# zju3dv/PVO

Measured on AMD Instinct MI355X. Metric: VO keyframe updates/sec (8-keyframe window, 512x384, 36 edges; 6 graph updates + edge rebuild per keyframe), higher is better.
Workload: dtype f16 (volume, lookup, update operator) / f32 (BA assembly) / f64 (pose solve); 1 GPU; S-B: BASELINE.json configs[1] window (8 keyframes, 48x64 maps, E=36, itrs=2), synthetic; edges=36, parallelism=independent window per GPU

## Files before the change

include/pvo_hip.h:

```cpp
#ifndef PVO_HIP_H
#define PVO_HIP_H

#include <stddef.h>
#include <stdint.h>

#ifdef __cplusplus
extern "C" {
#endif

enum { PVO_F32 = 0, PVO_F16 = 1, PVO_BF16 = 2, PVO_F64 = 3 };

enum {
  PVO_OK = 0,
  PVO_EINVAL = 1,
  PVO_ELAUNCH = 2,
  PVO_EWORKSPACE = 3,
  PVO_EUNSUPPORTED = 4
};

const char* pvo_strerror(int code);
const char* pvo_last_hip_error(void);
#define PVO_ABI_VERSION 105
int pvo_version(void);
size_t pvo_graph_update_args_size(void);

enum {
  PVO_KNOB_BA_SOLVER = 0,
  PVO_KNOB_HEADS_GATHER_FLAT = 1,
  PVO_KNOB_NO_RIDERS = 2,
  PVO_KNOB_POST_SEPARATE = 3,
  PVO_KNOB_COUNT = 4
};
int pvo_debug_config(int knob, int value);
int pvo_knob(int knob);


int pvo_corr_index_forward(const void* volume, const float* coords, void* corr,
                           int N, int h1, int w1, int h2, int w2,
                           int radius, int dtype, void* stream);

int pvo_corr_index_backward(const float* coords, const void* corr_grad, void* volume_grad,
                            int N, int h1, int w1, int h2, int w2,
                            int radius, int dtype, void* stream);

int pvo_corr_pyramid_lookup(const void* const* volumes_host, const float* coords, void* out,
                            int N, int h1, int w1, int h2, int w2,
                            int num_levels, int radius, int dtype, int out_channels_last,
                            const int* slots, int num_slots, void* stream);

int pvo_altcorr_forward(const void* fmap1, const void* fmap2, const float* coords, void* corr,
                        int B, int S, int H1, int W1, int H2, int W2, int C,
                        int radius, int dtype, void* stream);

int pvo_altcorr_backward(const void* fmap1, const void* fmap2, const float* coords,
                         const void* corr_grad, void* fmap1_grad, void* fmap2_grad,
                         int B, int S, int H1, int W1, int H2, int W2, int C,
                         int radius, int dtype, void* stream);


int pvo_corr_build(const void* fmap1, const void* fmap2, void* const* levels_host,
                   int N, int C, int H, int W, int num_levels, int dtype, int channels_last,
                   const int* out_slots, void* stream);

int pvo_corr_build_tiled(const void* fmap1, const void* fmap2, void* const* levels_host,
                         int N, int C, int H, int W, int dtype, const int* out_slots, void* stream);
int pvo_corr_pyramid_lookup_tiled(const void* const* volumes_host, const float* coords, void* out,
                                  int N, int h1, int w1, int h2, int w2, int num_levels, int dtype,
                                  int out_channels_last, const int* slots, int num_slots, void* stream);

int pvo_corr_lookup_encode_tiled(const void* const* volumes_host, const float* coords,
                                 const void* enc_weight, const float* enc_bias, void* out,
                                 int N, int h1, int w1, int dtype,
                                 const int* slots, int num_slots, void* stream);



int pvo_gru_glo_chunks(int HW);
int pvo_gru_glo_fused(const void* net, const void* w_weight, const float* w_bias, float* glo_part,
                      int E, int HW, int dtype, void* stream);
int pvo_gate_context(const float* glo_part, const float* wg_t, const float* g_bias, float* g,
                     int E, int chunks, void* stream);
int pvo_conv3x3_c128(const void* x, const void* w_taps, const float* bias, void* y,
                     int E, int H, int W, int Cout, int relu, int ystride, int yoff, int dtype, void* stream);
int pvo_conv3x3(const void* x, const void* w_taps, const float* bias, void* y,
                int E, int H, int W, int Cin, int Cout, int relu, int ystride, int yoff, int dtype, void* stream);
int pvo_gru_conv_gates(const void* net, const void* cf, int cf_channels, const void* w_taps, const float* g,
                       const void* P_zr, const int* p_slots, void* Z, void* RN, int E, int H, int W, int dtype, void* stream);
int pvo_gru_conv_candidate(const void* RN, const void* cf, int cf_channels, const void* w_taps, const float* g,
                           const void* P_q, const int* p_slots, const void* Z, const void* net, void* net_out,
                           int E, int H, int W, int dtype, void* stream);
int pvo_conv3x3_heads(const void* x, const void* w1_taps, const float* bias1, const void* w2_frags, float* z,
                      int E, int H, int W, int dtype, void* stream);
int pvo_heads_gather(const float* z, const float* bias2, void* y, int E, int H, int W, int dtype, void* stream);
int pvo_heads_out(const void* h1, const float* bias1, const void* w2, const float* bias2, void* y,
                  int E, int H, int W, int dtype, void* stream);
int pvo_conv7x7_c8(const void* x, const void* w_taps, const float* bias, void* y,
                   int E, int H, int W, int dtype, void* stream);
int pvo_flow_encoder(const void* x, const void* w7_taps, const float* bias7, const void* w3_taps, const float* bias3,
                     void* y, int E, int H, int W, int ystride, int yoff, int dtype, void* stream);
int pvo_corr_encode(const void* corr, const void* enc_weight, const float* enc_bias, void* y, long long rows,
                    int dtype, void* stream);
int pvo_segment_mean(const void* x, const int* seg_ptr, const int* seg_idx, const float* in_bias, void* out,
                     int K, int HW, int C, int dtype, void* stream);
int pvo_eta_head(const void* x, const void* w_taps, const float* bias, const int64_t* frame, const int* pos,
                 float* damping, float* eta, int R, int H, int W, float EP, float eta_scale, int dtype, void* stream);
int pvo_conv1x1_c128(const void* x, const void* w, const float* bias, void* y, long long rows, int Cout, int relu,
                     int dtype, void* stream);

int pvo_bias_norm_act(const void* x, const void* bias, const void* residual, void* y, long long planes, int C, int HW,
                      int norm, float eps, int relu_inner, int relu_outer, int dtype, void* stream);
int pvo_bias_norm_act_slices(int HW);
int pvo_bias_norm_act_split(const void* x, const void* bias, const void* residual, void* y, long long planes, int C, int HW,
                            int norm, float eps, int relu_inner, int relu_outer, int dtype, float* ws, size_t ws_floats, void* stream);
int pvo_conv1x1_planes(const void* x, const void* w, const void* bias, void* y, int N, int Cin, int Cout, int Hin, int Win, int stride,
                       int dtype, void* stream);
int pvo_frame_normalise(const void* img, void* out, int H, int W, const float* mean3, const float* std3, int in_kind, int dtype, void* stream);

int pvo_graph_motion(const float* target, const float* coords1, const float* delta_dy, const float* raw_mask,
                     void* motn, int E, int H, int W, int dtype, void* stream);
int pvo_segment_hist(const int* segm, const float* raw_mask, const void* heads, int* tot, int* dyn,
                     int E, int HW, int max_segments, float dy_thresh, int dtype, void* stream);
int pvo_graph_post(const float* coords1, const void* heads, float* raw_mask, float* target, float* delta_dy,
                   float* weight, float* target_ba, float* weight_ba, float* full_flow,
                   int E, int H, int W, float dy_thresh, const int* segm, const int* vote_tot, const int* vote_dyn,
                   int max_segments, float vote_thresh, int dtype, void* stream);


enum {
  PVO_OP_CONV128_WIDE = 1,
  PVO_OP_SINGLE_STREAM = 2,
  PVO_OP_ENC_SIDE_STREAM = 4
};

typedef struct pvo_update_weights {
  int dtype;
  int flags;
  const void* enc0_w;   const float* enc0_b;
  const void* cenc2_w;  const float* cenc2_b;
  const void* fenc0_w;  const float* fenc0_b;
  const void* fenc2_w;  const float* fenc2_b;
  const void* glo_w;    const float* glo_b;
  const float* gate_wt; const float* gate_b;
  const void* zr_w;     const void* q_w;
  const void* zr_inp_w; const void* q_inp_w;
  const void* heads1_w; const float* heads1_b;
  const void* heads2_w; const float* heads2_b;
  const void* agg1_w;   const float* agg1_b;
  const void* agg2_w;   const float* agg2_b;
  const void* eta_w;    const float* eta_b;
  const void* up_w;     const float* up_b;
} pvo_update_weights;

typedef struct pvo_operator_args {
  int E, H, W;
  const void* levels[4]; const int* slots; int num_slots;
  const float* coords;
  const void* corr;
  const void* motion;
  const void* net;
  void* net_out;
  const void* inp;
  const void* P_zr; const void* P_q;
  int static_by_slot;
  const int* seg_ptr; const int* seg_idx; int K;
  void* heads;
  const int64_t* eta_frame; const int* eta_pos; int R; float* damping; float EP; float eta_scale;
  float* eta;
  void* upmask;
} pvo_operator_args;

size_t pvo_operator_workspace_bytes(int E, int K, int H, int W);
int pvo_update_operator(const pvo_update_weights* weights, const pvo_operator_args* args,
                        void* workspace, size_t workspace_bytes, void* stream);

typedef struct pvo_graph_update_args {
  pvo_operator_args op;
  int nframes;
  float* poses; float* disps; const float* intrinsics;
  const int64_t* ii; const int64_t* jj;
  float* target; float* delta_dy; float* raw_mask;
  float* weight; float* full_flow;
  const int* segm; int max_segments; float vote_thresh;
  float dy_thresh;
  int n_in;
  float* target_ba; float* weight_ba;
  const int64_t* ii_ba; const int64_t* jj_ba;
  int t0, t1, itrs, motion_only; float lm, ep;
  void* sys; void* ba_ws; size_t ba_ws_bytes;
  int clamp_frames; float disp_min;
  int want_upmask;
  int context_ahead, context_ready;
} pvo_graph_update_args;

size_t pvo_graph_update_workspace_bytes(int E, int K, int R, int H, int W, int max_segments);
int pvo_side_stream(void** stream_out);

int pvo_proximity_select(const float* dist, int ni, int nj, int t0, int t1, int rad, int nms, double thresh,
                         const long long* have_i, const long long* have_j, int n_have,
                         long long* out_i, long long* out_j, int max_out, int* n_out);
enum { PVO_STAGE_LOOKUP = 0, PVO_STAGE_GATES = 1, PVO_STAGE_CANDIDATE = 2, PVO_STAGE_BA = 3, PVO_STAGE_UPDATE = 4,
       PVO_STAGE_EMPTY = 5  };
int pvo_probe_arm(int stage, int capacity);
int pvo_probe_arm_every(int stage, int capacity, int every);
int pvo_probe_read(float* ms_host, int max_n);
int pvo_graph_update(const pvo_update_weights* weights, const pvo_graph_update_args* args,
                     void* workspace, size_t workspace_bytes, void* stream);


int pvo_frame_distance(const float* poses, const float* disps, const float* intrinsics,
                       const int64_t* ii, const int64_t* jj, float* dist,
                       int M, int ht, int wd, float beta, void* stream);
int pvo_frame_distance_bidirectional(const float* poses, const float* disps, const float* intrinsics,
                                     const int64_t* ii, const int64_t* jj, float* dist,
                                     int M, int ht, int wd, float beta, void* stream);

int pvo_projmap(const float* poses, const float* disps, const float* intrinsics,
                const int64_t* ii, const int64_t* jj, float* coords, float* valid,
                int E, int ht, int wd, void* stream);

int pvo_iproj(const float* poses, const float* disps, const float* intrinsics,
              float* points, int N, int ht, int wd, void* stream);

int pvo_depth_filter(const float* poses, const float* disps, const float* intrinsics,
                     const int64_t* ix, const float* thresh, float* counter,
                     int N, int nframes, int ht, int wd, void* stream);

int pvo_reproject(const float* poses, const float* disps, const float* intrinsics,
                  const int64_t* ii, const int64_t* jj, float* coords, float* valid,
                  int E, int ht, int wd, void* stream);
int pvo_reproject_motion(const float* poses, const float* disps, const float* intrinsics,
                         const int64_t* ii, const int64_t* jj, float* coords, float* valid,
                         const float* target, const float* delta_dy, const float* raw_mask, void* motn,
                         int E, int ht, int wd, int dtype, void* stream);


int pvo_se3_unary(int op, const void* x, void* y, long long n, int dtype, void* stream);
int pvo_se3_binary(int op, const void* a, long long rep_a, const void* b, long long rep_b, void* y, long long n,
                   int dtype, void* stream);
int pvo_se3_unary_vjp(int op, const void* x, const void* gy, void* gx, long long n, int dtype, void* stream);
int pvo_se3_binary_vjp(int op, const void* a, long long rep_a, const void* b, long long rep_b, const void* gy,
                       void* ga, void* gb, long long n, int dtype, void* stream);

int pvo_proj_transform(const void* poses, const void* depths, const void* intr, const int64_t* ii, const int64_t* jj,
                       int B, int P, int N, int ht, int wd, int nx, void* x1, void* valid, void* Ji, void* Jj, void* Jz,
                       int dtype, void* stream);
int pvo_proj_transform_vjp(const void* poses, const void* depths, const void* intr, const int64_t* ii, const int64_t* jj,
                           int B, int P, int N, int ht, int wd, int nx, const void* g_x1, const void* g_Ji, const void* g_Jj, const void* g_Jz,
                           void* gposes, void* gdepths, int dtype, void* stream);


size_t pvo_ba_workspace_bytes(int E, int P, int nframes, int HW);

int pvo_ba(float* poses, float* disps, const float* intrinsics,
           const float* targets, const float* weights, const float* eta,
           const int64_t* ii, const int64_t* jj,
           int E, int nframes, int ht, int wd, int K_eta,
           int t0, int t1, int iterations, float lm, float ep, int motion_only,
           float* dx_out, float* dz_out, int dz_rows, int* status_out,
           void* workspace, size_t workspace_bytes, void* stream);

int pvo_ba_plan(const int64_t* ii, const int64_t* jj, int E, int nframes, int HW,
                int K_eta, int t0, int t1, void* workspace, size_t workspace_bytes,
                void* stream);
int pvo_ba_last_partition(void* workspace, size_t workspace_bytes, int E, int P, int nframes, int HW, int* out, void* stream);
int pvo_ba_local(const float* poses, const float* disps, const float* intrinsics,
                 const float* targets, const float* weights, const float* eta,
                 const int64_t* ii, const int64_t* jj,
                 int E, int nframes, int ht, int wd, int K_eta, int t0, int t1,
                 int motion_only, void* sys,
                 void* workspace, size_t workspace_bytes, void* stream);
int pvo_ba_finish(float* poses, float* disps, void* sys,
                  const int64_t* ii, const int64_t* jj,
                  int E, int nframes, int ht, int wd, int t0, int t1,
                  float lm, float ep, int motion_only, int clamp_frames, float disp_min,
                  float* dx_out, float* dz_out, int dz_rows, int* status_out,
                  void* workspace, size_t workspace_bytes, void* stream);
size_t pvo_ba_packed_elems(const int* first_host, int P);
int pvo_ba_pack(void* sys, const int* first_s, void* msg, int P, void* stream);
int pvo_ba_finish_packed(float* poses, float* disps, const void* msg, const int* first_s,
                         const int64_t* ii, const int64_t* jj,
                         int E, int nframes, int ht, int wd, int t0, int t1,
                         float lm, float ep, int motion_only, int clamp_frames, float disp_min,
                         float* dx_out, float* dz_out, int dz_rows, int* status_out,
                         void* workspace, size_t workspace_bytes, void* stream);

typedef struct pvo_ba_riders {
  const void* cx; const void* cw; const float* cbias; void* cy; long long crows; int cCout; int cdtype;
  const void* gnet; const void* gw; const float* gbias; float* gpart; int gE; int gHW; int gdtype;
  const float* xpart; const float* xwt; const float* xbias; float* xg; int xE; int xchunks;
} pvo_ba_riders;
int pvo_ba_finish_riders(float* poses, float* disps, void* sys,
                         const int64_t* ii, const int64_t* jj,
                         int E, int nframes, int ht, int wd, int t0, int t1,
                         float lm, float ep, int motion_only, int clamp_frames, float disp_min,
                         float* dx_out, float* dz_out, int dz_rows, int* status_out,
                         void* workspace, size_t workspace_bytes,
                         const pvo_ba_riders* riders, void* stream);
int pvo_ba_finish_conv1x1(float* poses, float* disps, void* sys,
                          const int64_t* ii, const int64_t* jj,
                          int E, int nframes, int ht, int wd, int t0, int t1,
                          float lm, float ep, int motion_only, int clamp_frames, float disp_min,
                          float* dx_out, float* dz_out, int dz_rows, int* status_out,
                          void* workspace, size_t workspace_bytes,
                          const void* cx, const void* cw, const float* cbias, void* cy, long long crows, int cCout, int cdtype,
                          void* stream);


size_t pvo_ba_train_workspace_bytes(int B, int P, int N, int M, int HW, int dtype);
size_t pvo_ba_train_vjp_scratch_bytes(int B, int P, int N, int M, int HW, int dtype);
int pvo_ba_train(const void* poses, const void* disps, const void* intr, const void* target, const void* weight, const void* eta,
                 const int64_t* ii, const int64_t* jj, const int* kx, const int* kk, const int* kptr, const int* kedge,
                 int B, int P, int N, int M, int ht, int wd, int fixedp, void* poses_out, void* disps_out, void* dx_out,
                 void* workspace, size_t workspace_bytes, int dtype, void* stream);
int pvo_ba_train_vjp(const void* poses, const void* disps, const void* intr, const void* target, const void* weight,
                     const int64_t* ii, const int64_t* jj, const int* kx, const int* kk, const int* kptr, const int* kedge,
                     int B, int P, int N, int M, int ht, int wd, int fixedp, const void* g_poses_out, const void* g_disps_out,
                     void* g_target, void* g_weight, void* g_eta, void* g_poses, void* g_disps,
                     const void* workspace, size_t workspace_bytes, void* scratch, size_t scratch_bytes, int dtype, void* stream);

#ifdef __cplusplus
}
#endif
#endif
```

pvo_amd/_lib.py:

```python
import ctypes
import os

_HERE = os.path.dirname(os.path.abspath(__file__))
LIB_PATH = os.path.join(_HERE, "libpvo_hip.so")

PVO_F32, PVO_F16, PVO_BF16, PVO_F64 = 0, 1, 2, 3
PVO_ABI_VERSION = 105

_c = ctypes
_vp, _i, _f, _sz = _c.c_void_p, _c.c_int, _c.c_float, _c.c_size_t

SIGNATURES = {
    "pvo_strerror": (_c.c_char_p, [_i]),
    "pvo_version": (_i, []),
    "pvo_graph_update_args_size": (_sz, []),
    "pvo_last_hip_error": (_c.c_char_p, []),
    "pvo_debug_config": (_i, [_i, _i]),
    "pvo_knob": (_i, [_i]),
    "pvo_corr_index_forward": (_i, [_vp, _vp, _vp, _i, _i, _i, _i, _i, _i, _i, _vp]),
    "pvo_corr_index_backward": (_i, [_vp, _vp, _vp, _i, _i, _i, _i, _i, _i, _i, _vp]),
    "pvo_corr_pyramid_lookup": (_i, [_vp, _vp, _vp, _i, _i, _i, _i, _i, _i, _i, _i, _i, _vp, _i, _vp]),
    "pvo_altcorr_forward": (_i, [_vp, _vp, _vp, _vp, _i, _i, _i, _i, _i, _i, _i, _i, _i, _vp]),
    "pvo_altcorr_backward": (_i, [_vp, _vp, _vp, _vp, _vp, _vp, _i, _i, _i, _i, _i, _i, _i, _i, _i, _vp]),
    "pvo_corr_build": (_i, [_vp, _vp, _vp, _i, _i, _i, _i, _i, _i, _i, _vp, _vp]),
    "pvo_gru_glo_chunks": (_i, [_i]),
    "pvo_gru_glo_fused": (_i, [_vp, _vp, _vp, _vp, _i, _i, _i, _vp]),
    "pvo_gate_context": (_i, [_vp, _vp, _vp, _vp, _i, _i, _vp]),
    "pvo_gru_conv_gates": (_i, [_vp, _vp, _i, _vp, _vp, _vp, _vp, _vp, _vp, _i, _i, _i, _i, _vp]),
    "pvo_gru_conv_candidate": (_i, [_vp, _vp, _i, _vp, _vp, _vp, _vp, _vp, _vp, _vp, _i, _i, _i, _i, _vp]),
    "pvo_conv3x3": (_i, [_vp, _vp, _vp, _vp, _i, _i, _i, _i, _i, _i, _i, _i, _i, _vp]),
    "pvo_conv3x3_c128": (_i, [_vp, _vp, _vp, _vp, _i, _i, _i, _i, _i, _i, _i, _i, _vp]),
    "pvo_conv7x7_c8": (_i, [_vp, _vp, _vp, _vp, _i, _i, _i, _i, _vp]),
    "pvo_flow_encoder": (_i, [_vp, _vp, _vp, _vp, _vp, _vp, _i, _i, _i, _i, _i, _i, _vp]),
    "pvo_corr_encode": (_i, [_vp, _vp, _vp, _vp, _c.c_longlong, _i, _vp]),
    "pvo_eta_head": (_i, [_vp, _vp, _vp, _vp, _vp, _vp, _vp, _i, _i, _i, _f, _f, _i, _vp]),
    "pvo_conv1x1_c128": (_i, [_vp, _vp, _vp, _vp, _c.c_longlong, _i, _i, _i, _vp]),
    "pvo_corr_build_tiled": (_i, [_vp, _vp, _vp, _i, _i, _i, _i, _i, _vp, _vp]),
    "pvo_corr_lookup_encode_tiled": (_i, [_vp, _vp, _vp, _vp, _vp, _i, _i, _i, _i, _vp, _i, _vp]),
    "pvo_corr_pyramid_lookup_tiled": (_i, [_vp, _vp, _vp, _i, _i, _i, _i, _i, _i, _i, _i, _vp, _i, _vp]),
    "pvo_heads_out": (_i, [_vp, _vp, _vp, _vp, _vp, _i, _i, _i, _i, _vp]),
    "pvo_conv3x3_heads": (_i, [_vp, _vp, _vp, _vp, _vp, _i, _i, _i, _i, _vp]),
    "pvo_heads_gather": (_i, [_vp, _vp, _vp, _i, _i, _i, _i, _vp]),
    "pvo_segment_mean": (_i, [_vp, _vp, _vp, _vp, _vp, _i, _i, _i, _i, _vp]),
    "pvo_graph_motion": (_i, [_vp, _vp, _vp, _vp, _vp, _i, _i, _i, _i, _vp]),
    "pvo_reproject_motion": (_i, [_vp, _vp, _vp, _vp, _vp, _vp, _vp, _vp, _vp, _vp, _vp, _i, _i, _i, _i, _vp]),
    "pvo_bias_norm_act": (_i, [_vp, _vp, _vp, _vp, _c.c_longlong, _i, _i, _i, _f, _i, _i, _i, _vp]),
    "pvo_bias_norm_act_slices": (_i, [_i]),
    "pvo_bias_norm_act_split": (_i, [_vp, _vp, _vp, _vp, _c.c_longlong, _i, _i, _i, _f, _i, _i, _i, _vp, _sz, _vp]),
    "pvo_conv1x1_planes": (_i, [_vp, _vp, _vp, _vp, _i, _i, _i, _i, _i, _i, _i, _vp]),
    "pvo_frame_normalise": (_i, [_vp, _vp, _i, _i, _c.POINTER(_f), _c.POINTER(_f), _i, _i, _vp]),
    "pvo_segment_hist": (_i, [_vp, _vp, _vp, _vp, _vp, _i, _i, _i, _f, _i, _vp]),
    "pvo_graph_post": (_i, [_vp, _vp, _vp, _vp, _vp, _vp, _vp, _vp, _vp, _i, _i, _i, _f, _vp, _vp, _vp, _i, _f, _i, _vp]),
    "pvo_operator_workspace_bytes": (_sz, [_i, _i, _i, _i]),
    "pvo_update_operator": (_i, [_vp, _vp, _vp, _sz, _vp]),
    "pvo_graph_update_workspace_bytes": (_sz, [_i, _i, _i, _i, _i, _i]),
    "pvo_graph_update": (_i, [_vp, _vp, _vp, _sz, _vp]),
    "pvo_se3_unary": (_i, [_i, _vp, _vp, _c.c_longlong, _i, _vp]),
    "pvo_se3_binary": (_i, [_i, _vp, _c.c_longlong, _vp, _c.c_longlong, _vp, _c.c_longlong, _i, _vp]),
    "pvo_se3_unary_vjp": (_i, [_i, _vp, _vp, _vp, _c.c_longlong, _i, _vp]),
    "pvo_se3_binary_vjp": (_i, [_i, _vp, _c.c_longlong, _vp, _c.c_longlong, _vp, _vp, _vp, _c.c_longlong, _i, _vp]),
    "pvo_proj_transform": (_i, [_vp, _vp, _vp, _vp, _vp, _i, _i, _i, _i, _i, _i, _vp, _vp, _vp, _vp, _vp, _i, _vp]),
    "pvo_proj_transform_vjp": (_i, [_vp, _vp, _vp, _vp, _vp, _i, _i, _i, _i, _i, _i, _vp, _vp, _vp, _vp, _vp, _vp, _i, _vp]),
    "pvo_side_stream": (_i, [_c.POINTER(_vp)]),
    "pvo_proximity_select": (_i, [_vp, _i, _i, _i, _i, _i, _i, _c.c_double, _vp, _vp, _i, _vp, _vp, _i, _c.POINTER(_i)]),
    "pvo_probe_arm": (_i, [_i, _i]),
    "pvo_probe_arm_every": (_i, [_i, _i, _i]),
    "pvo_probe_read": (_i, [_vp, _i]),
    "pvo_frame_distance": (_i, [_vp, _vp, _vp, _vp, _vp, _vp, _i, _i, _i, _f, _vp]),
    "pvo_frame_distance_bidirectional": (_i, [_vp, _vp, _vp, _vp, _vp, _vp, _i, _i, _i, _f, _vp]),
    "pvo_projmap": (_i, [_vp, _vp, _vp, _vp, _vp, _vp, _vp, _i, _i, _i, _vp]),
    "pvo_iproj": (_i, [_vp, _vp, _vp, _vp, _i, _i, _i, _vp]),
    "pvo_depth_filter": (_i, [_vp, _vp, _vp, _vp, _vp, _vp, _i, _i, _i, _i, _vp]),
    "pvo_reproject": (_i, [_vp, _vp, _vp, _vp, _vp, _vp, _vp, _i, _i, _i, _vp]),
    "pvo_ba_workspace_bytes": (_sz, [_i, _i, _i, _i]),
    "pvo_ba": (_i, [_vp, _vp, _vp, _vp, _vp, _vp, _vp, _vp, _i, _i, _i, _i, _i, _i, _i, _i,
                    _f, _f, _i, _vp, _vp, _i, _vp, _vp, _sz, _vp]),
    "pvo_ba_plan": (_i, [_vp, _vp, _i, _i, _i, _i, _i, _i, _vp, _sz, _vp]),
    "pvo_ba_last_partition": (_i, [_vp, _sz, _i, _i, _i, _i, ctypes.POINTER(ctypes.c_int), _vp]),
    "pvo_ba_packed_elems": (_sz, [ctypes.POINTER(ctypes.c_int), _i]),
    "pvo_ba_pack": (_i, [_vp, _vp, _vp, _i, _vp]),
    "pvo_ba_finish_packed": (_i, [_vp, _vp, _vp, _vp, _vp, _vp, _i, _i, _i, _i, _i, _i, _f, _f, _i, _i, _f,
                                  _vp, _vp, _i, _vp, _vp, _sz, _vp]),
    "pvo_ba_local": (_i, [_vp, _vp, _vp, _vp, _vp, _vp, _vp, _vp, _i, _i, _i, _i, _i, _i, _i,
                          _i, _vp, _vp, _sz, _vp]),
    "pvo_ba_finish": (_i, [_vp, _vp, _vp, _vp, _vp, _i, _i, _i, _i, _i, _i, _f, _f, _i, _i, _f,
                           _vp, _vp, _i, _vp, _vp, _sz, _vp]),
    "pvo_ba_finish_riders": (_i, [_vp, _vp, _vp, _vp, _vp, _i, _i, _i, _i, _i, _i, _f, _f, _i, _i, _f,
                                  _vp, _vp, _i, _vp, _vp, _sz, _vp, _vp]),
    "pvo_ba_finish_conv1x1": (_i, [_vp, _vp, _vp, _vp, _vp, _i, _i, _i, _i, _i, _i, _f, _f, _i, _i, _f,
                                   _vp, _vp, _i, _vp, _vp, _sz, _vp, _vp, _vp, _vp, _c.c_longlong, _i, _i, _vp]),
    "pvo_ba_train_workspace_bytes": (_sz, [_i, _i, _i, _i, _i, _i]),
    "pvo_ba_train_vjp_scratch_bytes": (_sz, [_i, _i, _i, _i, _i, _i]),
    "pvo_ba_train": (_i, [_vp, _vp, _vp, _vp, _vp, _vp, _vp, _vp, _vp, _vp, _vp, _vp, _i, _i, _i, _i, _i, _i, _i,
                          _vp, _vp, _vp, _vp, _sz, _i, _vp]),
    "pvo_ba_train_vjp": (_i, [_vp, _vp, _vp, _vp, _vp, _vp, _vp, _vp, _vp, _vp, _vp, _i, _i, _i, _i, _i, _i, _i,
                              _vp, _vp, _vp, _vp, _vp, _vp, _vp, _vp, _sz, _vp, _sz, _i, _vp]),
}



class UpdateWeights(_c.Structure):
    _fields_ = [("dtype", _i), ("flags", _i)] + [(n, _vp) for n in (
        "enc0_w", "enc0_b", "cenc2_w", "cenc2_b", "fenc0_w", "fenc0_b", "fenc2_w", "fenc2_b", "glo_w", "glo_b",
        "gate_wt", "gate_b", "zr_w", "q_w", "zr_inp_w", "q_inp_w", "heads1_w", "heads1_b", "heads2_w", "heads2_b",
        "agg1_w", "agg1_b", "agg2_w", "agg2_b", "eta_w", "eta_b", "up_w", "up_b")]


class OperatorArgs(_c.Structure):
    _fields_ = [("E", _i), ("H", _i), ("W", _i), ("levels", _vp * 4), ("slots", _vp), ("num_slots", _i),
                ("coords", _vp), ("corr", _vp), ("motion", _vp), ("net", _vp), ("net_out", _vp), ("inp", _vp),
                ("P_zr", _vp), ("P_q", _vp), ("static_by_slot", _i), ("seg_ptr", _vp), ("seg_idx", _vp), ("K", _i), ("heads", _vp),
                ("eta_frame", _vp), ("eta_pos", _vp), ("R", _i), ("damping", _vp), ("EP", _f), ("eta_scale", _f), ("eta", _vp),
                ("upmask", _vp)]


class GraphUpdateArgs(_c.Structure):
    _fields_ = [("op", OperatorArgs), ("nframes", _i), ("poses", _vp), ("disps", _vp), ("intrinsics", _vp),
                ("ii", _vp), ("jj", _vp), ("target", _vp), ("delta_dy", _vp), ("raw_mask", _vp), ("weight", _vp),
                ("full_flow", _vp), ("segm", _vp), ("max_segments", _i), ("vote_thresh", _f), ("dy_thresh", _f),
                ("n_in", _i), ("target_ba", _vp), ("weight_ba", _vp), ("ii_ba", _vp), ("jj_ba", _vp),
                ("t0", _i), ("t1", _i), ("itrs", _i), ("motion_only", _i), ("lm", _f), ("ep", _f),
                ("sys", _vp), ("ba_ws", _vp), ("ba_ws_bytes", _sz), ("clamp_frames", _i), ("disp_min", _f),
                ("want_upmask", _i), ("context_ahead", _i), ("context_ready", _i)]


PVO_OP_CONV128_WIDE, PVO_OP_SINGLE_STREAM, PVO_OP_ENC_SIDE_STREAM = 1, 2, 4
PVO_KNOB_BA_SOLVER, PVO_KNOB_HEADS_GATHER_FLAT, PVO_KNOB_NO_RIDERS, PVO_KNOB_POST_SEPARATE = 0, 1, 2, 3

_lib = None


class PvoHipError(RuntimeError):
    pass


def load():
    global _lib
    if _lib is not None:
        return _lib
    if not os.path.exists(LIB_PATH):
        raise PvoHipError(
            "libpvo_hip.so not found at %s - build it with `python -m pvo_amd.build` "
            "(there is no CPU fallback)" % LIB_PATH)
    import torch
    lib = ctypes.CDLL(LIB_PATH)
    for name, (res, args) in SIGNATURES.items():
        fn = getattr(lib, name)
        fn.restype = res
        fn.argtypes = args
    if lib.pvo_version() != PVO_ABI_VERSION or lib.pvo_graph_update_args_size() != ctypes.sizeof(GraphUpdateArgs):
        raise PvoHipError("libpvo_hip.so is ABI version %d with a %d-byte pvo_graph_update_args; this binding is written for version %d / %d bytes - "
                          "rebuild with `python -m pvo_amd.build`" % (lib.pvo_version(), lib.pvo_graph_update_args_size(), PVO_ABI_VERSION,
                                                                     ctypes.sizeof(GraphUpdateArgs)))
    _lib = lib
    return lib


PROBE_LIB_PATH = os.path.join(_HERE, "libpvo_probe.so")
PROBE_SIGNATURES = {
    "pvo_clock_probe": (_i, [_vp, _i, _vp]),
    "pvo_mem_probe": (_c.c_longlong, [_vp, _sz, _i, _i, _i, _vp, _vp]),
}
_probe_lib = None


def load_probe():
    global _probe_lib
    if _probe_lib is None:
        load()
        if not os.path.exists(PROBE_LIB_PATH):
            raise PvoHipError("libpvo_probe.so not found at %s - build it with `python -m pvo_amd.build`" % PROBE_LIB_PATH)
        lib = ctypes.CDLL(PROBE_LIB_PATH)
        for name, (res, args) in PROBE_SIGNATURES.items():
            fn = getattr(lib, name)
            fn.restype, fn.argtypes = res, args
        _probe_lib = lib
    return _probe_lib


def check(status, what):
    if status != 0:
        msg = load().pvo_strerror(status).decode()
        if status == 2:
            msg += " - " + load().pvo_last_hip_error().decode()
        raise PvoHipError("%s failed: %s (status %d)" % (what, msg, status))
```

pvo_amd/csrc/ba.hip:

```cpp
#include "se3.h"
#include "conv1x1_tile.h"
#include "glo_tile.h"
#include <stdlib.h>
#include <type_traits>

namespace {

constexpr float kMinDepth = 0.25f;

constexpr double kFix = 268435456.0, kInvFix = 1.0 / 268435456.0;
__device__ __forceinline__ void fix_add(long long* sys, long long idx, double v, int* meta) {
  if (!(fabs(v) < 3.0e10)) { meta[4] = 1; return; }
#ifdef PVO_BA_NO_ATOMICS
  if (idx >= 0) return;
#endif
  atomicAdd(reinterpret_cast<unsigned long long*>(sys + idx), static_cast<unsigned long long>(__double2ll_rn(v * kFix)));
}
constexpr int kDealEdges = 2;
constexpr int kPPT = 2;
constexpr int kChunkA = 256 * kPPT;
constexpr int kMaxSep = 12;
constexpr int kXchgDoubles = 2 + 36 * kMaxSep * kMaxSep + 12 * kMaxSep;


#if defined(PVO_BA_PROBE) && PVO_BA_PROBE == 3
__device__ unsigned long long* g_ba_wg_probe = nullptr;
#define BA_WG_PROBE(kern, slot)                                                                                         \
  do {                                                                                                                  \
    if (g_ba_wg_probe && threadIdx.x == 0 && blockIdx.z == 0) {                                                         \
      const unsigned wg_ = blockIdx.y * gridDim.x + blockIdx.x;                                                         \
      if (wg_ < 4096u) g_ba_wg_probe[((kern) * 4096u + wg_) * 8u + (slot)] = wall_clock64();                            \
    }                                                                                                                   \
  } while (0)
#else
#define BA_WG_PROBE(kern, slot)
#endif

struct Plan {
  int* kidx;
  int* kx;
  int* eptr;
  int* eidx;
  int* meta;
  int* env;
};

struct Ws {
  Plan plan;
  float *Eii, *Eij;
  float *Cii, *bz;
  float *Ei;
  float *Q, *w;
  float *dx;
  float *part;
  long long* sys;
  double* chol;
  double* xchg;
  double* ldiag;
  double* xvec;
  float* Mrg;
  float* spart;
  short* srow;
  int* sT;
  size_t bytes;
};
constexpr int kSchurStagePairs = 36;
__host__ __device__ __forceinline__ int schur_stage_frames(int P) { return (P > 0 && P <= 29) ? P + 8 : 0; }

__host__ size_t align_up(size_t x) { return (x + 255) & ~static_cast<size_t>(255); }

__host__ Ws carve(void* base, int E, int P, int F, int HW) {
  Ws w{};
  char* p = static_cast<char*>(base);
  size_t off = 0;
  auto take = [&](size_t bytes) { char* r = p ? p + off : nullptr; off += align_up(bytes); return r; };
  const int Kmax = (F < P + E) ? F : (P + E);
  const size_t n6 = static_cast<size_t>(6) * (P > 0 ? P : 0);
  w.plan.kidx = reinterpret_cast<int*>(take(sizeof(int) * (F + 1)));
  w.plan.kx = reinterpret_cast<int*>(take(sizeof(int) * (F + 1)));
  w.plan.eptr = reinterpret_cast<int*>(take(sizeof(int) * (F + 2)));
  w.plan.eidx = reinterpret_cast<int*>(take(sizeof(int) * (E + 1)));
  w.plan.meta = reinterpret_cast<int*>(take(sizeof(int) * 8));
  w.plan.env = reinterpret_cast<int*>(take(sizeof(int) * ((P > 0 ? P : 0) + 1)));
  w.Eii = reinterpret_cast<float*>(take(sizeof(float) * static_cast<size_t>(E) * 6 * HW));
  w.Eij = reinterpret_cast<float*>(take(sizeof(float) * static_cast<size_t>(E) * 6 * HW));
  w.Cii = reinterpret_cast<float*>(take(sizeof(float) * static_cast<size_t>(E) * HW));
  w.bz = reinterpret_cast<float*>(take(sizeof(float) * static_cast<size_t>(E) * HW));
  w.Ei = reinterpret_cast<float*>(take(sizeof(float) * static_cast<size_t>(P > 0 ? P : 0) * 6 * HW));
  w.Q = reinterpret_cast<float*>(take(sizeof(float) * static_cast<size_t>(Kmax) * HW));
  w.w = reinterpret_cast<float*>(take(sizeof(float) * static_cast<size_t>(Kmax) * HW));
  w.dx = reinterpret_cast<float*>(take(sizeof(float) * (n6 + 8)));
  w.part = reinterpret_cast<float*>(take(sizeof(float) * static_cast<size_t>(E) * ((HW + kChunkA - 1) / kChunkA) * 90 + 16));
  w.sys = reinterpret_cast<long long*>(take(sizeof(double) * (n6 * n6 + n6 + 8)));
  w.chol = reinterpret_cast<double*>(take(sizeof(double) * (n6 * n6 + n6 + 27 * (n6 / 6) + 32)));
  w.xchg = reinterpret_cast<double*>(take(sizeof(double) * kXchgDoubles));
  w.ldiag = reinterpret_cast<double*>(take(sizeof(double) * (n6 / 48 + 2) * (48 * 48 + 48)));
  w.xvec = reinterpret_cast<double*>(take(sizeof(double) * (n6 + 8)));
  w.Mrg = reinterpret_cast<float*>(take(sizeof(float) * static_cast<size_t>(E) * 6 * HW));
  {
    const size_t ks = static_cast<size_t>(schur_stage_frames(P));
    w.spart = reinterpret_cast<float*>(take(sizeof(float) * ks * ((HW + 255) / 256) * kSchurStagePairs * 256));
    w.srow = reinterpret_cast<short*>(take(sizeof(short) * ks * 128));
    w.sT = reinterpret_cast<int*>(take(sizeof(int) * (ks + 1)));
  }
  w.bytes = off;
  return w;
}

__global__ __launch_bounds__(256) void ba_plan_kernel(
    const int64_t* __restrict__ ii, const int64_t* __restrict__ jj, Plan pl,
    int E, int F, int t0, int t1, int K_eta, int motion_only) {
  __shared__ int seg[257];
  const int tid = threadIdx.x;
  for (int b = tid; b < t1 - t0; b += 256) pl.env[b] = 0x7fffffff;
  for (int f = tid; f < F; f += 256) pl.kidx[f] = (f >= t0 && f < t1) ? 1 : 0;
  __syncthreads();
  for (int e = tid; e < E; e += 256) {
    const long long f = ii[e];
    if (f >= 0 && f < F) pl.kidx[f] = 1;
  }
  __syncthreads();
  const int per = (F + 255) / 256;
  const int lo = min(tid * per, F), hi = min(lo + per, F);
  int cnt = 0;
  for (int f = lo; f < hi; ++f) cnt += pl.kidx[f];
  seg[tid + 1] = cnt;
  if (tid == 0) seg[0] = 0;
  __syncthreads();
  if (tid == 0) for (int i = 1; i <= 256; ++i) seg[i] += seg[i - 1];
  __syncthreads();
  int run = seg[tid];
  for (int f = lo; f < hi; ++f) {
    if (pl.kidx[f]) { pl.kx[run] = f; pl.kidx[f] = run; ++run; } else pl.kidx[f] = -1;
  }
  const int K = seg[256];
  __syncthreads();
  for (int k = tid; k < K; k += 256) {
    const int f = pl.kx[k];
    int c = 0;
    for (int e = 0; e < E; ++e) c += (ii[e] == f) ? 1 : 0;
    pl.eptr[k + 1] = c;
  }
  if (tid == 0) pl.eptr[0] = 0;
  __syncthreads();
  if (tid == 0) for (int k = 1; k <= K; ++k) pl.eptr[k] += pl.eptr[k - 1];
  __syncthreads();
  for (int k = tid; k < K; k += 256) {
    const int f = pl.kx[k];
    int o = pl.eptr[k];
    for (int e = 0; e < E; ++e) if (ii[e] == f) pl.eidx[o++] = e;
  }
  if (tid == 0) {
    pl.meta[0] = K;
    pl.meta[1] = 0;
    pl.meta[3] = 0;
    pl.meta[4] = 0;
    pl.meta[2] = (!motion_only && K_eta != K && K_eta != 1) ? 1 : 0;
  }
}

struct EdgeGeom { Pose G; float fx, fy, cx, cy; };

__device__ __forceinline__ void pixel_terms(const EdgeGeom& g, float u, float v, float disp,
                                            float tu, float tv, float wgu, float wgv,
                                            float (&h)[78], float (&vi)[6], float (&vj)[6],
                                            float (&eii)[6], float (&eij)[6], float& cii, float& bzz) {
  float Xi[4] = {(u - g.cx) / g.fx, (v - g.cy) / g.fy, 1.0f, disp};
  float Xj[4];
  act4(g.G, Xi, Xj);
  const float x = Xj[0], y = Xj[1], hh = Xj[3];
  const bool ok = !(Xj[2] < kMinDepth);
  const float d = ok ? 1.0f / Xj[2] : 0.0f;
  const float d2 = d * d;
  const float wu = ok ? static_cast<float>(0.001 * static_cast<double>(wgu)) : 0.0f;
  const float wv = ok ? static_cast<float>(0.001 * static_cast<double>(wgv)) : 0.0f;
  const float ru = tu - (g.fx * d * x + g.cx);
  const float rv = tv - (g.fy * d * y + g.cy);
  float J[12];
  float Jz;
  J[6] = g.fx * (hh * d); J[7] = 0.0f; J[8] = g.fx * (-x * hh * d2);
  J[9] = g.fx * (-x * y * d2); J[10] = g.fx * (1.0f + x * x * d2); J[11] = g.fx * (-y * d);
  Jz = g.fx * (g.G.t.x * d - g.G.t.z * (x * d2));
  adjT(g.G, &J[6], &J[0]);
#pragma unroll
  for (int n = 0; n < 6; ++n) J[n] = -J[n];
  {
    int l = 0;
#pragma unroll
    for (int n = 0; n < 12; ++n) {
      const float wj = wu * J[n];
#pragma unroll
      for (int m = 0; m <= n; ++m) { h[l] += wj * J[m]; ++l; }
    }
  }
#pragma unroll
  for (int n = 0; n < 6; ++n) {
    vi[n] += wu * ru * J[n];
    vj[n] += wu * ru * J[6 + n];
    eii[n] = wu * Jz * J[n];
    eij[n] = wu * Jz * J[6 + n];
  }
  cii = wu * Jz * Jz;
  bzz = wu * ru * Jz;
  J[6] = 0.0f; J[7] = g.fy * (hh * d); J[8] = g.fy * (-y * hh * d2);
  J[9] = g.fy * (-1.0f - y * y * d2); J[10] = g.fy * (x * y * d2); J[11] = g.fy * (x * d);
  Jz = g.fy * (g.G.t.y * d - g.G.t.z * (y * d2));
  adjT(g.G, &J[6], &J[0]);
#pragma unroll
  for (int n = 0; n < 6; ++n) J[n] = -J[n];
  {
    int l = 0;
#pragma unroll
    for (int n = 0; n < 12; ++n) {
      const float wj = wv * J[n];
#pragma unroll
      for (int m = 0; m <= n; ++m) { h[l] += wj * J[m]; ++l; }
    }
  }
#pragma unroll
  for (int n = 0; n < 6; ++n) {
    vi[n] += wv * rv * J[n];
    vj[n] += wv * rv * J[6 + n];
    eii[n] += wv * Jz * J[n];
    eij[n] += wv * Jz * J[6 + n];
  }
  cii += wv * Jz * Jz;
  bzz += wv * rv * Jz;
}

__device__ __forceinline__ void pose_block_scatter(int t, double val, int pi, int pj, int P, long long* __restrict__ sys, int* __restrict__ meta) {
  const bool iok = pi >= 0 && pi < P, jok = pj >= 0 && pj < P;
  const int n6 = 6 * P;
  if (t < 78) {
    int n = 0, base = 0;
    while (base + n + 1 <= t) { base += n + 1; ++n; }
    const int m = t - base;
    if (n < 6) {
      if (iok) {
        fix_add(sys, static_cast<long long>(6 * pi + n) * n6 + 6 * pi + m, val, meta);
        if (n != m) fix_add(sys, static_cast<long long>(6 * pi + m) * n6 + 6 * pi + n, val, meta);
      }
    } else if (m < 6) {
      if (iok && jok) {
        if (pi > pj) fix_add(sys, static_cast<long long>(6 * pi + m) * n6 + 6 * pj + (n - 6), val, meta);
        else fix_add(sys, static_cast<long long>(6 * pj + (n - 6)) * n6 + 6 * pi + m, val, meta);
      }
    } else {
      if (jok) {
        fix_add(sys, static_cast<long long>(6 * pj + n - 6) * n6 + 6 * pj + m - 6, val, meta);
        if (n != m) fix_add(sys, static_cast<long long>(6 * pj + m - 6) * n6 + 6 * pj + n - 6, val, meta);
      }
    }
  } else if (t < 84) {
    if (iok) fix_add(sys, static_cast<long long>(n6) * n6 + 6 * pi + (t - 78), val, meta);
  } else {
    if (jok) fix_add(sys, static_cast<long long>(n6) * n6 + 6 * pj + (t - 84), val, meta);
  }
}

__device__ __forceinline__ void pose_block_targets(int t, int pi, int pj, int P, long long idx[2]) {
  const bool iok = pi >= 0 && pi < P, jok = pj >= 0 && pj < P;
  const long long n6 = 6 * P;
  idx[0] = idx[1] = -1;
  if (t < 78) {
    int n = 0, base = 0;
    while (base + n + 1 <= t) { base += n + 1; ++n; }
    const int m = t - base;
    if (n < 6) {
      if (iok) { idx[0] = (6 * pi + n) * n6 + 6 * pi + m; if (n != m) idx[1] = (6 * pi + m) * n6 + 6 * pi + n; }
    } else if (m < 6) {
      if (iok && jok) idx[0] = (pi > pj) ? (6 * pi + m) * n6 + 6 * pj + (n - 6) : (6 * pj + (n - 6)) * n6 + 6 * pi + m;
    } else {
      if (jok) { idx[0] = (6 * pj + n - 6) * n6 + 6 * pj + m - 6; if (n != m) idx[1] = (6 * pj + m - 6) * n6 + 6 * pj + n - 6; }
    }
  } else if (t < 84) {
    if (iok) idx[0] = n6 * n6 + 6 * pi + (t - 78);
  } else {
    if (jok) idx[0] = n6 * n6 + 6 * pj + (t - 84);
  }
}

__global__ __launch_bounds__(256) void ba_assemble_kernel(
    const float* __restrict__ poses, const float* __restrict__ disps, const float* __restrict__ intr,
    const float* __restrict__ targets, const float* __restrict__ weights,
    const int64_t* __restrict__ ii, const int64_t* __restrict__ jj,
    float* __restrict__ Eii, float* __restrict__ Eij, float* __restrict__ Cii, float* __restrict__ bz,
    long long* __restrict__ sys, int* __restrict__ meta, int HW, int wd, int t0, int P, int motion_only, float* __restrict__ part) {
  __shared__ float red[4][90];
  BA_WG_PROBE(0, 0);
  const int e = blockIdx.y;
  const int ix = static_cast<int>(ii[e]), jx = static_cast<int>(jj[e]);
  EdgeGeom g;
  g.G = rel_pose(load_pose(poses + 7 * static_cast<long long>(ix)), load_pose(poses + 7 * static_cast<long long>(jx)));
  g.fx = intr[0]; g.fy = intr[1]; g.cx = intr[2]; g.cy = intr[3];

  float h[78], vi[6], vj[6];
#pragma unroll
  for (int l = 0; l < 78; ++l) h[l] = 0.0f;
#pragma unroll
  for (int n = 0; n < 6; ++n) { vi[n] = 0.0f; vj[n] = 0.0f; }

  const float* __restrict__ d_i = disps + static_cast<long long>(ix) * HW;
  const float* __restrict__ tg = targets + static_cast<long long>(e) * 2 * HW;
// ... 1981 lines not shown
        }
        double v = a[j];
#pragma unroll
        for (int k = 0; k < j; ++k) v -= a[k] * L[j * (j + 1) / 2 + k];
        v *= rs;
        if (tid < 8 && j > tid) v = 0.0;
        a[j] = v;
      }
#pragma unroll
      for (int j = 0; j < 8; ++j) pan[tid * 8 + (j ^ sw)] = a[j];
      if (tid < 8) {
        double r = L[0];
#pragma unroll
        for (int j = 1; j < 8; ++j) r = (tid == j) ? L[j * (j + 1) / 2 + j] : r;
        rdg[c0 + tid] = r;
      }
      if (tid == 0 && !ok) fail = 1;
    }
    DENSE_STEP_PROBE(9);
    __syncthreads();
    DENSE_STEP_PROBE(10);
    {
      const int u0 = first_slot(h == 0 ? tc : tc + 1);
      auto pair = [&](auto kc) {
        constexpr int K = decltype(kc)::value;
        constexpr int K1 = K + 1 < SLOTS ? K + 1 : K;
        const bool on0 = K >= u0 && K < nsl, on1 = K + 1 < SLOTS && K + 1 >= u0 && K + 1 < nsl;
        const int ta0 = on0 ? 16 * tti[K] + lc - c0 : 0, tb0 = on0 ? 16 * ttj[K] + lc - c0 : 0;
        const int ta1 = on1 ? 16 * tti[K1] + lc - c0 : 0, tb1 = on1 ? 16 * ttj[K1] + lc - c0 : 0;
        double a00 = pan[dense_swz(ta0, lr)], b00 = pan[dense_swz(tb0, lr)], a01 = pan[dense_swz(ta0, 4 + lr)], b01 = pan[dense_swz(tb0, 4 + lr)];
        double a10 = pan[dense_swz(ta1, lr)], b10 = pan[dense_swz(tb1, lr)], a11 = pan[dense_swz(ta1, 4 + lr)], b11 = pan[dense_swz(tb1, 4 + lr)];
        if (!on0) { a00 = 0.0; a01 = 0.0; }
        if (!on1) { a10 = 0.0; a11 = 0.0; }
        C[K] = __builtin_amdgcn_mfma_f64_16x16x4f64(-a00, b00, C[K], 0, 0, 0);
        if (K + 1 < SLOTS) C[K1] = __builtin_amdgcn_mfma_f64_16x16x4f64(-a10, b10, C[K1], 0, 0, 0);
        C[K] = __builtin_amdgcn_mfma_f64_16x16x4f64(-a01, b01, C[K], 0, 0, 0);
        if (K + 1 < SLOTS) C[K1] = __builtin_amdgcn_mfma_f64_16x16x4f64(-a11, b11, C[K1], 0, 0, 0);
      };
      switch (u0 >> 1) {
#define PVO_DENSE_PAIR(K) case K / 2: if (K < SLOTS) { if (K >= nsl) break; pair(std::integral_constant<int, (K < SLOTS ? K : 0)>{}); } [[fallthrough]];
        PVO_DENSE_PAIR(0) PVO_DENSE_PAIR(2) PVO_DENSE_PAIR(4) PVO_DENSE_PAIR(6) PVO_DENSE_PAIR(8) PVO_DENSE_PAIR(10) PVO_DENSE_PAIR(12)
        PVO_DENSE_PAIR(14) PVO_DENSE_PAIR(16)
#undef PVO_DENSE_PAIR
        default: break;
      }
    }
    DENSE_STEP_PROBE(11);
    if (kb8 + 1 < nb) extract(kb8 + 1);
    DENSE_STEP_PROBE(12);
    DENSE_STEP_PROBE(13);
    __syncthreads();
    DENSE_STEP_PROBE(14);
  }
  BA_PROBE(2);

  if (wave == 0) {
    double z[3];
#pragma unroll
    for (int m = 0; m < 3; ++m) {
      const int c = lane + 64 * m;
      z[m] = c < n ? Lp[8 * dense_panel_off(c >> 3, N) + dense_swz(n - 8 * (c >> 3), c & 7)] : 0.0;
    }
    for (int kb8 = nb - 1; kb8 >= 0; --kb8) {
      const int c0 = 8 * kb8, m0 = c0 >> 6, l0 = c0 & 63;
      const int nv = (n - c0 < 8) ? n - c0 : 8;
      const double* pan = Lp + 8 * dense_panel_off(kb8, N);
      double Lk[28], rdv[8];
#pragma unroll
      for (int j = 0; j < 8; ++j) {
        rdv[j] = rdg[c0 + j];
#pragma unroll
        for (int i = j + 1; i < 8; ++i) Lk[i * (i - 1) / 2 + j] = pan[dense_swz(i, j)];
      }
      const double zsel = m0 == 0 ? z[0] : (m0 == 1 ? z[1] : z[2]);
      double x[8];
#pragma unroll
      for (int j = 0; j < 8; ++j) {
        const int lo = __builtin_amdgcn_readlane(static_cast<int>(__double_as_longlong(zsel) & 0xffffffffLL), l0 + j);
        const int hi = __builtin_amdgcn_readlane(static_cast<int>(__double_as_longlong(zsel) >> 32), l0 + j);
        x[j] = __longlong_as_double((static_cast<long long>(hi) << 32) | static_cast<unsigned int>(lo));
      }
#pragma unroll
      for (int j = 7; j >= 0; --j) {
        double v = x[j];
#pragma unroll
        for (int i = 7; i > j; --i) v -= Lk[i * (i - 1) / 2 + j] * x[i];
        x[j] = (j < nv) ? v * rdv[j] : 0.0;
      }
#pragma unroll
      for (int m = 0; m < 3; ++m) {
        const int c = lane + 64 * m;
        if (c < c0) {
          const double* pc = Lp + 8 * dense_panel_off(c >> 3, N);
          double v = z[m];
#pragma unroll
          for (int i = 0; i < 8; ++i) v -= pc[dense_swz(c0 + i - 8 * (c >> 3), c & 7)] * x[i];
          z[m] = v;
        } else if (c < c0 + 8) {
          double v = x[0];
#pragma unroll
          for (int j = 1; j < 8; ++j) v = (c - c0 == j) ? x[j] : v;
          z[m] = v;
        }
      }
    }
#pragma unroll
    for (int m = 0; m < 3; ++m) {
      const int c = lane + 64 * m;
      if (c < n) xs[c] = z[m];
    }
  }
  __syncthreads();
  BA_PROBE(4);
  solve_epilogue([&](int i) { return xs[i]; }, fail | meta[4] | meta[2], true, 0, P, t0, poses, dx_ws, dx_out, meta, status_out, true,
                 [] { BA_PROBE(5); });
}

constexpr int kNB = 48;
__global__ __launch_bounds__(256) void dense_panel_kernel(double* __restrict__ A, double* __restrict__ Ldiag, int n, int kb, int* __restrict__ meta) {
  __shared__ double Lk[kNB][kNB + 1];
  __shared__ double Xs[kNB][kNB + 1];
  __shared__ double rinv[kNB], ldg[kNB];
  const int tid = threadIdx.x;
  const int c0 = kNB * kb, nc = (n - c0 < kNB) ? n - c0 : kNB;
  const int rb = kb + blockIdx.x, r0 = kNB * rb;
  for (int t = tid; t < kNB * kNB; t += 256) {
    const int r = t / kNB, c = t - r * kNB;
    Lk[r][c] = (r < nc && c <= r) ? A[static_cast<size_t>(c0 + r) * n + c0 + c] : 0.0;
    const int rr = r0 + r;
    Xs[r][c] = (rr <= n && c < nc) ? A[static_cast<size_t>(rr) * n + c0 + c] : 0.0;
  }
  __syncthreads();
  bool ok = true;
  for (int j0 = 0; j0 < nc; j0 += 8) {
    const int nv = (nc - j0 < 8) ? nc - j0 : 8;
    double L[36], av[8];
    if (tid < 2 * kNB) {
      const bool isx = tid >= kNB;
      const int t = isx ? tid - kNB : tid;
      if (isx || (t >= j0 && t < nc)) {
        double (*Row)[kNB + 1] = isx ? Xs : Lk;
#pragma unroll
        for (int i = 0; i < 8; ++i) {
#pragma unroll
          for (int j = 0; j <= i; ++j) L[i * (i + 1) / 2 + j] = Lk[j0 + i][j0 + j];
        }
#pragma unroll
        for (int j = 0; j < 8; ++j) av[j] = Row[t][j0 + j];
      }
    }
    __syncthreads();
    if (tid < 2 * kNB) {
      const bool isx = tid >= kNB;
      const int t = isx ? tid - kNB : tid;
      if (isx || (t >= j0 && t < nc)) {
        double (*Row)[kNB + 1] = isx ? Xs : Lk;
#pragma unroll
        for (int j = 0; j < 8; ++j) {
          double d = L[j * (j + 1) / 2 + j];
#pragma unroll
          for (int k = 0; k < j; ++k) d -= L[j * (j + 1) / 2 + k] * L[j * (j + 1) / 2 + k];
          const bool real = j < nv;
          ok = ok && (!real || d > 0.0);
          const double rs = (real && ok) ? rsqrt_nr(d) : 0.0;
          if (!isx && t == j0 + j) { rinv[j0 + j] = rs; ldg[j0 + j] = d * rs; }
          L[j * (j + 1) / 2 + j] = rs;
#pragma unroll
          for (int i = j + 1; i < 8; ++i) {
            double v = L[i * (i + 1) / 2 + j];
#pragma unroll
            for (int k = 0; k < j; ++k) v -= L[i * (i + 1) / 2 + k] * L[j * (j + 1) / 2 + k];
            L[i * (i + 1) / 2 + j] = v * rs;
          }
          double v = av[j];
#pragma unroll
          for (int k = 0; k < j; ++k) v -= av[k] * L[j * (j + 1) / 2 + k];
          av[j] = v * rs;
        }
#pragma unroll
        for (int j = 0; j < 8; ++j) if (j < nv && (isx || j0 + j <= t)) Row[t][j0 + j] = av[j];
      }
    }
    __syncthreads();
    const int c1 = j0 + 8;
    if (c1 < nc) {
      const int ty = tid >> 4, tx = tid & 15;
      for (int r = c1 + ty; r < nc + kNB; r += 16) {
        const bool isx = r >= nc;
        double (*Row)[kNB + 1] = isx ? Xs : Lk;
        const int rr = isx ? r - nc : r;
        double a8[8];
#pragma unroll
        for (int k = 0; k < 8; ++k) a8[k] = Row[rr][j0 + k];
        const int cend = isx ? nc - 1 : rr;
        for (int c = c1 + tx; c <= cend; c += 16) {
          double v = Row[rr][c];
#pragma unroll
          for (int k = 0; k < 8; ++k) v -= a8[k] * Lk[c][j0 + k];
          Row[rr][c] = v;
        }
      }
    }
    __syncthreads();
  }
  if (tid == kNB && !ok) meta[4] = 1;
  if (tid >= nc && tid < kNB) { rinv[tid] = 0.0; ldg[tid] = 0.0; }
  __syncthreads();
  for (int t = tid; t < kNB * kNB; t += 256) {
    const int r = t / kNB, c = t - r * kNB;
    const int rr = r0 + r;
    if (rr <= n && c < nc && (rb > kb || r >= nc)) A[static_cast<size_t>(rr) * n + c0 + c] = Xs[r][c];
  }
  if (blockIdx.x == 0) {
    double* Ld = Ldiag + static_cast<size_t>(kb) * (kNB * kNB + kNB);
    for (int t = tid; t < kNB * kNB; t += 256) {
      const int r = t / kNB, c = t - r * kNB;
      Ld[t] = (r < nc && c < r) ? Lk[r][c] : ((r == c && r < nc) ? ldg[r] : 0.0);
    }
    if (tid < kNB) Ld[kNB * kNB + tid] = rinv[tid];
  }
}

__global__ __launch_bounds__(256) void dense_update_kernel(double* __restrict__ A, int n, int kb, int nrb) {
  __shared__ double Li[kNB][kNB + 1], Lj[kNB][kNB + 1];
  const int m = nrb - kb - 1;
  int p = blockIdx.x, jj = 0;
  while (p >= m - jj) { p -= m - jj; ++jj; }
  const int bj = kb + 1 + jj, bi = bj + p;
  const int tid = threadIdx.x;
  const int c0 = kNB * kb, nc = (n - c0 < kNB) ? n - c0 : kNB;
  for (int t = tid; t < kNB * kNB; t += 256) {
    const int r = t / kNB, c = t - r * kNB;
    const int ri = kNB * bi + r, rj = kNB * bj + r;
    Li[r][c] = (ri <= n && c < nc) ? A[static_cast<size_t>(ri) * n + c0 + c] : 0.0;
    Lj[r][c] = (rj < n && c < nc) ? A[static_cast<size_t>(rj) * n + c0 + c] : 0.0;
  }
  __syncthreads();
  const int ty = tid >> 4, tx = tid & 15;
  double acc[3][3] = {{0, 0, 0}, {0, 0, 0}, {0, 0, 0}};
#pragma unroll 4
  for (int k = 0; k < kNB; ++k) {
    double a[3], b[3];
#pragma unroll
    for (int u = 0; u < 3; ++u) { a[u] = Li[3 * ty + u][k]; b[u] = Lj[3 * tx + u][k]; }
#pragma unroll
    for (int u = 0; u < 3; ++u)
#pragma unroll
      for (int v = 0; v < 3; ++v) acc[u][v] += a[u] * b[v];
  }
#pragma unroll
  for (int u = 0; u < 3; ++u) {
    const int rr = kNB * bi + 3 * ty + u;
    if (rr > n) continue;
#pragma unroll
    for (int v = 0; v < 3; ++v) {
      const int cc = kNB * bj + 3 * tx + v;
      if (cc < n && (bi > bj || cc <= rr)) A[static_cast<size_t>(rr) * n + cc] -= acc[u][v];
    }
  }
}

__global__ __launch_bounds__(256) void dense_back_kernel(const double* __restrict__ A, const double* __restrict__ Ldiag, double* __restrict__ yrow,
                                                         double* __restrict__ xvec, int n, int kb) {
  __shared__ double Lk[kNB][kNB + 1];
  __shared__ double s[kNB], xk[kNB], rinv[kNB];
  const int tid = threadIdx.x, lane = tid & 63;
  const int c0 = kNB * kb, nc = (n - c0 < kNB) ? n - c0 : kNB;
  const double* Ld = Ldiag + static_cast<size_t>(kb) * (kNB * kNB + kNB);
  for (int t = tid; t < kNB * kNB; t += 256) Lk[t / kNB][t % kNB] = Ld[t];
  if (tid < kNB) { rinv[tid] = Ld[kNB * kNB + tid]; s[tid] = tid < nc ? yrow[c0 + tid] : 0.0; }
  __syncthreads();
  if (tid < 64) {
    for (int j = nc - 1; j >= 0; --j) {
      if (lane == j) xk[j] = s[j] * rinv[j];
      const double xj = xk[j];
      if (lane < j) s[lane] -= Lk[j][lane] * xj;
    }
  }
  __syncthreads();
  const int bj = blockIdx.x;
  if (bj == kb) {
    if (tid < nc) xvec[c0 + tid] = xk[tid];
    return;
  }
  if (tid < kNB) {
    const int col = kNB * bj + tid;
    double v = yrow[col];
    for (int r = 0; r < nc; ++r) v -= A[static_cast<size_t>(c0 + r) * n + col] * xk[r];
    yrow[col] = v;
  }
}

__global__ __launch_bounds__(256) void dense_finish_kernel(const double* __restrict__ xvec, float* __restrict__ poses, float* __restrict__ dx_ws,
                                                           float* __restrict__ dx_out, int* __restrict__ meta, int* __restrict__ status_out,
                                                           int P, int t0, Riders riders) {
  extern __shared__ __attribute__((aligned(16))) unsigned char smem[];
  if (blockIdx.x > 0) {
    ride(smem, riders, blockIdx.x - 1);
    return;
  }
  solve_epilogue([&](int i) { return xvec[i]; }, meta[4] | meta[2], true, 0, P, t0, poses, dx_ws, dx_out, meta, status_out, true, [] {});
}

__device__ __forceinline__ void ba_backsub_body(
    const Plan& pl, const int64_t* __restrict__ jj, const float* __restrict__ Ei, const float* __restrict__ Eij,
    const float* __restrict__ Q, const float* __restrict__ w, const float* __restrict__ dx,
    float* __restrict__ disps, float* __restrict__ dz_out, int dz_rows, int HW, int t0, int P,
    int clamp_frames, float disp_min) {
  const int k = blockIdx.y;
  const int x = blockIdx.x * 256 + threadIdx.x;
  __shared__ int s_edge[256], s_pose[256];
  __shared__ float s_dx[256][6];
  const bool live = k < pl.meta[0] && !pl.meta[2];
  const int e0 = live ? pl.eptr[k] : 0, deg = live ? pl.eptr[k + 1] - e0 : 0;
  const bool in_lds = deg <= 255;
  constexpr int lo = 1;
  if (live && in_lds && static_cast<int>(threadIdx.x) <= deg) {
    const int r = static_cast<int>(threadIdx.x) - 1;
    int e = 0, p;
    if (r < 0) p = pl.kx[k] - t0;
    else { e = pl.eidx[e0 + r]; p = static_cast<int>(jj[e]) - t0; }
    const bool ok = p >= 0 && p < P && p >= lo;
    s_edge[threadIdx.x] = e; s_pose[threadIdx.x] = ok ? p : -1;
#pragma unroll
    for (int n = 0; n < 6; ++n) s_dx[threadIdx.x][n] = ok ? dx[6 * p + n] : 0.0f;
  }
  BA_WG_PROBE(2, 0);
  __syncthreads();
  BA_WG_PROBE(2, 1);
  if (x >= HW) return;
  if (k < clamp_frames && pl.kidx[k] < 0) {
    const float v = disps[static_cast<long long>(k) * HW + x];
    if (v < disp_min) disps[static_cast<long long>(k) * HW + x] = disp_min;
  }
  if (!live) return;
  float acc = 0.0f;
  if (in_lds) {
    for (int q = 0; q <= deg; ++q) {
      const int p = s_pose[q];
      if (p < 0) continue;
      const float* base = (q == 0) ? Ei + static_cast<long long>(p) * 6 * HW : Eij + static_cast<long long>(s_edge[q]) * 6 * HW;
      float sacc = 0.0f;
#pragma unroll
      for (int n = 0; n < 6; ++n) sacc += base[static_cast<long long>(n) * HW + x] * s_dx[q][n];
      acc += sacc;
    }
  } else {
    for (int r = -1; r < deg; ++r) {
      const RowRef R = row_of(r, k, pl, Ei, Eij, jj, HW, t0, P);
      if (R.pose < lo) continue;
      float sacc = 0.0f;
#pragma unroll
      for (int n = 0; n < 6; ++n) sacc += R.base[static_cast<long long>(n) * HW + x] * dx[6 * R.pose + n];
      acc += sacc;
    }
  }
  const float dz = Q[static_cast<long long>(k) * HW + x] * (w[static_cast<long long>(k) * HW + x] - acc);
  float d = disps[static_cast<long long>(pl.kx[k]) * HW + x] + dz;
  if (pl.kx[k] < clamp_frames && d < disp_min) d = disp_min;
  disps[static_cast<long long>(pl.kx[k]) * HW + x] = d;
  if (dz_out && k < dz_rows) dz_out[static_cast<long long>(k) * HW + x] = dz;
  BA_WG_PROBE(2, 2);
}

__global__ __launch_bounds__(256) void ba_backsub_kernel(
    Plan pl, const int64_t* __restrict__ jj, const float* __restrict__ Ei, const float* __restrict__ Eij,
    const float* __restrict__ Q, const float* __restrict__ w, const float* __restrict__ dx,
    float* __restrict__ disps, float* __restrict__ dz_out, int dz_rows, int HW, int t0, int P,
    int clamp_frames, float disp_min) {
  ba_backsub_body(pl, jj, Ei, Eij, Q, w, dx, disps, dz_out, dz_rows, HW, t0, P, clamp_frames, disp_min);
}

int check_common(int E, int F, int ht, int wd, int t0, int t1) {
  if (E < 0 || F <= 0 || ht <= 0 || wd <= 0 || t0 < 0 || t1 < t0 || t1 > F) return PVO_EINVAL;
  if (E > 65535) return PVO_EUNSUPPORTED;
  return PVO_OK;
}

}

#if defined(PVO_BA_PROBE) && PVO_BA_PROBE == 3
extern "C" int pvo_debug_ba_wg_probe(void* buf) { return hipMemcpyToSymbol(HIP_SYMBOL(g_ba_wg_probe), &buf, sizeof(buf)) == hipSuccess ? 0 : 1; }
#endif
#ifdef PVO_BA_PROBE
extern "C" int pvo_debug_ba_probe(void* buf) { return hipMemcpyToSymbol(HIP_SYMBOL(g_ba_probe), &buf, sizeof(buf)) == hipSuccess ? 0 : 1; }
#endif



extern "C" size_t pvo_ba_workspace_bytes(int E, int P, int nframes, int HW) {
  if (E < 0 || P < 0 || nframes < 0 || HW < 0) return 0;
  return carve(nullptr, E, P, nframes, HW).bytes + 256;
}

static inline void* ws_base(void* workspace) {
  return reinterpret_cast<void*>((reinterpret_cast<uintptr_t>(workspace) + 255) & ~static_cast<uintptr_t>(255));
}

extern "C" int pvo_ba_plan(const int64_t* ii, const int64_t* jj, int E, int nframes, int HW,
                           int K_eta, int t0, int t1, void* workspace, size_t workspace_bytes,
                           void* stream) {
  if (E < 0 || nframes <= 0 || t0 < 0 || t1 < t0 || t1 > nframes || !workspace) return PVO_EINVAL;
  if (E > 0 && (!ii || !jj)) return PVO_EINVAL;
  const int P = t1 - t0;
  if (workspace_bytes < pvo_ba_workspace_bytes(E, P, nframes, HW)) return PVO_EWORKSPACE;
  Ws w = carve(ws_base(workspace), E, P, nframes, HW);
  hipLaunchKernelGGL(ba_plan_kernel, dim3(1), dim3(256), 0, pvo_stream(stream),
                     ii, jj, w.plan, E, nframes, t0, t1, K_eta, K_eta < 0 ? 1 : 0);
  PVO_CHECK_LAUNCH();
  return PVO_OK;
}

extern "C" int pvo_ba_local(const float* poses, const float* disps, const float* intrinsics,
                            const float* targets, const float* weights, const float* eta,
                            const int64_t* ii, const int64_t* jj,
                            int E, int nframes, int ht, int wd, int K_eta, int t0, int t1,
                            int motion_only, void* sys_,
                            void* workspace, size_t workspace_bytes, void* stream) {
  long long* sys = static_cast<long long*>(sys_);
  int rc = check_common(E, nframes, ht, wd, t0, t1);
  if (rc != PVO_OK) return rc;
  const int P = t1 - t0, HW = ht * wd;
  if (!poses || !disps || !intrinsics || !sys || !workspace) return PVO_EINVAL;
  if (E > 0 && (!targets || !weights || !ii || !jj)) return PVO_EINVAL;
  if (!motion_only && !eta) return PVO_EINVAL;
  if (P > 5400 || nframes >= (1 << 28)) return PVO_EUNSUPPORTED;
  if (workspace_bytes < pvo_ba_workspace_bytes(E, P, nframes, HW)) return PVO_EWORKSPACE;
  Ws w = carve(ws_base(workspace), E, P, nframes, HW);
  hipStream_t st = pvo_stream(stream);
  const size_t n6 = static_cast<size_t>(6) * P;
  const bool clean = (motion_only & 2) != 0;
  motion_only &= 1;
  if (!clean && hipMemsetAsync(sys, 0, sizeof(long long) * (n6 * n6 + n6), st) != hipSuccess) return PVO_ELAUNCH;
  if (E == 0) return PVO_OK;
  const bool two_stage = !motion_only;
  const int chunksA = (HW + kChunkA - 1) / kChunkA;
  hipLaunchKernelGGL(ba_assemble_kernel, dim3((HW + kChunkA - 1) / kChunkA, E), dim3(256), 0, st,
                     poses, disps, intrinsics, targets, weights, ii, jj, w.Eii, w.Eij, w.Cii, w.bz,
                     sys, w.plan.meta, HW, wd, t0, P, motion_only, two_stage ? w.part : nullptr);
  PVO_CHECK_LAUNCH();
  if (!motion_only) {
    const int Kmax = (nframes < P + E) ? nframes : (P + E);
    const int frames_opt = (nframes < P + 1) ? nframes : (P + 1);
    const long long wg256 = static_cast<long long>((HW + 255) / 256) * frames_opt;
    const bool dense_window = P <= kDenseMaxPoses && wg256 > 192;
    const int pix = (wg256 <= 192 || dense_window) ? 256 : (wg256 <= 1024 ? 512 : 1024);
    const int gx = (HW + pix - 1) / pix;
    const int deal_rows = two_stage ? (E + kDealEdges * gx - 1) / (kDealEdges * gx) : 0;
    const int Kgrid = (K_eta > 1 && K_eta <= Kmax) ? K_eta : Kmax;
    const dim3 sgrid(gx, Kgrid + deal_rows, dense_window ? 1 : 4);
    const int depth_done = (pix != 256 || dense_window) ? 1 : 0;
    constexpr int kSchurRowsLds = 110 * 1024;
    const size_t sdyn = dense_window ? kSchurRowsLds : 0;
    const int lds_floats = static_cast<int>(sdyn / sizeof(float));
    if (dense_window && !(pvo_allow_lds<ba_schur_mfma_kernel<true, 256>>(kSchurRowsLds) && pvo_allow_lds<ba_schur_mfma_kernel<false, 256>>(kSchurRowsLds)))
      return PVO_ELAUNCH;
    if (depth_done) {
      hipLaunchKernelGGL(ba_depth_kernel, dim3((HW + 255) / 256, Kgrid), dim3(256), 0, st, w.plan, eta, K_eta, w.Eii, w.Cii, w.bz, w.Ei, w.Q, w.w, HW, t0, P);
      PVO_CHECK_LAUNCH();
    }
    const bool stage2 = dense_window && Kgrid <= schur_stage_frames(P);
#define PVO_SCHUR_LAUNCH(V, PX) hipLaunchKernelGGL((ba_schur_mfma_kernel<V, PX>), sgrid, dim3(256), (PX == 256 ? sdyn : 0), st, w.plan, jj, eta, K_eta, w.Eii, w.Cii, w.bz, w.Ei, \
                                                   w.Eij, w.Q, w.w, sys, HW, t0, P, two_stage ? w.part : nullptr, ii, E, chunksA, deal_rows, w.Mrg, depth_done, (PX == 256 ? lds_floats : 0), \
                                                   (stage2 && PX == 256) ? w.spart : nullptr, w.srow, stage2 ? w.sT : nullptr)
    if ((HW & 3) == 0) { if (pix == 256) PVO_SCHUR_LAUNCH(true, 256); else if (pix == 512) PVO_SCHUR_LAUNCH(true, 512); else PVO_SCHUR_LAUNCH(true, 1024); }
    else { if (pix == 256) PVO_SCHUR_LAUNCH(false, 256); else if (pix == 512) PVO_SCHUR_LAUNCH(false, 512); else PVO_SCHUR_LAUNCH(false, 1024); }
#undef PVO_SCHUR_LAUNCH
    PVO_CHECK_LAUNCH();
    if (stage2) {
      hipLaunchKernelGGL(ba_schur_reduce_kernel, dim3(kSchurStagePairs, Kgrid), dim3(256), 0, st, w.plan, w.spart, w.srow, w.sT, sys, gx, 6 * P);
      PVO_CHECK_LAUNCH();
    }
  }
  return PVO_OK;
}

extern "C" int pvo_ba_finish(float* poses, float* disps, void* sys_,
                             const int64_t* ii, const int64_t* jj,
                             int E, int nframes, int ht, int wd, int t0, int t1,
                             float lm, float ep, int motion_only, int clamp_frames, float disp_min,
                             float* dx_out, float* dz_out, int dz_rows, int* status_out,
                             void* workspace, size_t workspace_bytes, void* stream) {
  return pvo_ba_finish_riders(poses, disps, sys_, ii, jj, E, nframes, ht, wd, t0, t1, lm, ep, motion_only, clamp_frames, disp_min,
                              dx_out, dz_out, dz_rows, status_out, workspace, workspace_bytes, nullptr, stream);
}

extern "C" int pvo_ba_finish_conv1x1(float* poses, float* disps, void* sys_,
                                     const int64_t* ii, const int64_t* jj,
                                     int E, int nframes, int ht, int wd, int t0, int t1,
                                     float lm, float ep, int motion_only, int clamp_frames, float disp_min,
                                     float* dx_out, float* dz_out, int dz_rows, int* status_out,
                                     void* workspace, size_t workspace_bytes,
                                     const void* cx, const void* cw, const float* cbias, void* cy, long long crows, int cCout, int cdtype,
                                     void* stream) {
  pvo_ba_riders r{};
  r.cx = cx; r.cw = cw; r.cbias = cbias; r.cy = cy; r.crows = crows; r.cCout = cCout; r.cdtype = cdtype;
  return pvo_ba_finish_riders(poses, disps, sys_, ii, jj, E, nframes, ht, wd, t0, t1, lm, ep, motion_only, clamp_frames, disp_min,
                              dx_out, dz_out, dz_rows, status_out, workspace, workspace_bytes, cy ? &r : nullptr, stream);
}

static int ba_finish_impl(float* poses, float* disps, void* sys_, const long long* msg, const int* first_s,
                          const int64_t* ii, const int64_t* jj,
                          int E, int nframes, int ht, int wd, int t0, int t1,
                          float lm, float ep, int motion_only, int clamp_frames, float disp_min,
                          float* dx_out, float* dz_out, int dz_rows, int* status_out,
                          void* workspace, size_t workspace_bytes,
                          const pvo_ba_riders* jobs, void* stream);

extern "C" int pvo_ba_finish_riders(float* poses, float* disps, void* sys_,
                                    const int64_t* ii, const int64_t* jj,
                                    int E, int nframes, int ht, int wd, int t0, int t1,
                                    float lm, float ep, int motion_only, int clamp_frames, float disp_min,
                                    float* dx_out, float* dz_out, int dz_rows, int* status_out,
                                    void* workspace, size_t workspace_bytes,
                                    const pvo_ba_riders* jobs, void* stream) {
  if (!sys_) return PVO_EINVAL;
  return ba_finish_impl(poses, disps, sys_, nullptr, nullptr, ii, jj, E, nframes, ht, wd, t0, t1, lm, ep, motion_only, clamp_frames, disp_min,
                        dx_out, dz_out, dz_rows, status_out, workspace, workspace_bytes, jobs, stream);
}

extern "C" size_t pvo_ba_packed_elems(const int* first_host, int P) {
  if (!first_host || P < 0) return 0;
  size_t blocks = 0;
  for (int b = 0; b < P; ++b) {
    const int f = first_host[b] < b ? (first_host[b] < 0 ? 0 : first_host[b]) : b;
    blocks += static_cast<size_t>(b - f + 1) * 36;
  }
  return blocks + static_cast<size_t>(6) * P;
}

extern "C" int pvo_ba_pack(void* sys_, const int* first_s, void* msg, int P, void* stream) {
  if (!sys_ || !first_s || !msg || P < 0) return PVO_EINVAL;
  if (P > kMaxEnvBlocks) return PVO_EUNSUPPORTED;
  if (P == 0) return PVO_OK;
  const int n6 = 6 * P;
  hipLaunchKernelGGL(ba_pack_kernel, dim3((n6 * n6 + n6 + 2047) / 2048), dim3(256), 0, pvo_stream(stream),
                     static_cast<long long*>(sys_), first_s, static_cast<long long*>(msg), n6);
  PVO_CHECK_LAUNCH();
  return PVO_OK;
}

extern "C" int pvo_ba_finish_packed(float* poses, float* disps, const void* msg, const int* first_s,
                                    const int64_t* ii, const int64_t* jj,
                                    int E, int nframes, int ht, int wd, int t0, int t1,
                                    float lm, float ep, int motion_only, int clamp_frames, float disp_min,
                                    float* dx_out, float* dz_out, int dz_rows, int* status_out,
                                    void* workspace, size_t workspace_bytes, void* stream) {
  if (!msg || !first_s) return PVO_EINVAL;
  return ba_finish_impl(poses, disps, nullptr, static_cast<const long long*>(msg), first_s, ii, jj, E, nframes, ht, wd, t0, t1, lm, ep, motion_only,
                        clamp_frames, disp_min, dx_out, dz_out, dz_rows, status_out, workspace, workspace_bytes, nullptr, stream);
}

enum SolveKind { kSolveStatus, kSolveDense, kSolveEnvelope, kSolveChain, kSolveBlocks };
struct SolveForm { SolveKind kind; int chol; };
static SolveForm solve_form(int P, int E, bool packed, int knob) {
  if (P == 0) return {kSolveStatus, 0};
  if (knob >= 1 && knob <= 3) return {kSolveChain, knob - 1};
  if (knob == 4) return {kSolveEnvelope, 2};
  if (knob == 6 && !packed) return {kSolveBlocks, 0};
  if (P <= kDenseMaxPoses) return {kSolveDense, 0};
  if (knob != 5 && !packed && static_cast<long long>(E) > 8LL * P) return {kSolveBlocks, 0};
  return {kSolveEnvelope, 2};
}

static int ba_finish_impl(float* poses, float* disps, void* sys_, const long long* msg, const int* first_s,
                          const int64_t* ii, const int64_t* jj,
                          int E, int nframes, int ht, int wd, int t0, int t1,
                          float lm, float ep, int motion_only, int clamp_frames, float disp_min,
                          float* dx_out, float* dz_out, int dz_rows, int* status_out,
                          void* workspace, size_t workspace_bytes,
                          const pvo_ba_riders* jobs, void* stream) {
  Riders rider{};
  size_t rider_lds = 0;
  if (jobs && jobs->cy && jobs->crows > 0) {
    if (!jobs->cx || !jobs->cw || jobs->cCout <= 0 || jobs->cCout % 192) return PVO_EINVAL;
    if (jobs->cdtype != PVO_F16 && jobs->cdtype != PVO_BF16) return PVO_EUNSUPPORTED;
    if (pvo_misaligned16(jobs->cx, jobs->cw, jobs->cy)) return PVO_EINVAL;
    if (jobs->crows > (1LL << 24)) return PVO_EUNSUPPORTED;
    rider.cx = static_cast<const uint16_t*>(jobs->cx); rider.cw = static_cast<const uint16_t*>(jobs->cw); rider.cbias = jobs->cbias;
    rider.cy = static_cast<uint16_t*>(jobs->cy); rider.crows = jobs->crows; rider.cCout = jobs->cCout; rider.cdtype = jobs->cdtype;
    rider.crow_blocks = static_cast<int>((jobs->crows + 63) / 64);
    rider.cblocks = rider.crow_blocks * (jobs->cCout / 192);
    rider_lds = c1t::kTileBytes;
  }
  if (jobs && jobs->gpart && jobs->gE > 0 && jobs->gHW > 0) {
    if (!jobs->gnet || !jobs->gw || jobs->gE > 65535) return PVO_EINVAL;
    if (jobs->gdtype != PVO_F16 && jobs->gdtype != PVO_BF16) return PVO_EUNSUPPORTED;
    if (pvo_misaligned16(jobs->gnet, jobs->gw)) return PVO_EINVAL;
    rider.gnet = static_cast<const uint16_t*>(jobs->gnet); rider.gw = static_cast<const uint16_t*>(jobs->gw); rider.gbias = jobs->gbias;
    rider.gpart = jobs->gpart; rider.gHW = jobs->gHW; rider.gchunks = (jobs->gHW + 255) / 256; rider.gdtype = jobs->gdtype;
    rider.gblocks = jobs->gE * rider.gchunks;
    if (rider_lds < static_cast<size_t>(glt::kTileBytes)) rider_lds = glt::kTileBytes;
  }
  if (jobs && jobs->xg && jobs->xE > 0) {
    if (!jobs->xpart || !jobs->xwt || !jobs->xbias || jobs->xchunks <= 0) return PVO_EINVAL;
    rider.xpart = jobs->xpart; rider.xwt = jobs->xwt; rider.xbias = jobs->xbias; rider.xg = jobs->xg;
    rider.xchunks = jobs->xchunks; rider.xblocks = jobs->xE;
    if (rider_lds < 512) rider_lds = 512;
  }
  const int rider_blocks = rider.cblocks + rider.gblocks + rider.xblocks;
  int rc = check_common(E, nframes, ht, wd, t0, t1);
  if (rc != PVO_OK) return rc;
  if (clamp_frames < 0 || clamp_frames > nframes) return PVO_EINVAL;
  const int P = t1 - t0, HW = ht * wd;
  long long* sys = static_cast<long long*>(sys_);
  if (!poses || !disps || (!sys && !msg) || !workspace) return PVO_EINVAL;
  if (P > kMaxEnvBlocks) return PVO_EUNSUPPORTED;
  if (workspace_bytes < pvo_ba_workspace_bytes(E, P, nframes, HW)) return PVO_EWORKSPACE;
  Ws w = carve(ws_base(workspace), E, P, nframes, HW);
  hipStream_t st = pvo_stream(stream);
  const int n6 = 6 * P;
  const SolveForm form = solve_form(P, E, msg != nullptr, pvo_knob(PVO_KNOB_BA_SOLVER));
  if (msg && form.kind == kSolveStatus) return PVO_OK;
  constexpr size_t kSolveLdsMax = 142000;
  if (form.kind == kSolveDense) {
    const size_t dl = dense_lds_bytes(n6);
    const size_t lds = dl > rider_lds ? dl : rider_lds;
    const int Td = dense_N(n6) / 16;
    if (!pvo_allow_lds<ba_solve_dense_kernel<4>>(kSolveLdsMax) || !pvo_allow_lds<ba_solve_dense_kernel<14>>(kSolveLdsMax) ||
        !pvo_allow_lds<ba_solve_dense_kernel<17>>(kSolveLdsMax))
      return PVO_ELAUNCH;
    const auto kernel = Td <= 5 ? ba_solve_dense_kernel<4> : (Td <= 10 ? ba_solve_dense_kernel<14> : ba_solve_dense_kernel<17>);
    hipLaunchKernelGGL(kernel, dim3(1 + rider_blocks), dim3(256), lds, st, sys, msg, first_s, poses, w.dx, dx_out, w.plan.meta, status_out,
                       P, t0, lm, ep, rider);
  } else if (form.kind == kSolveEnvelope || form.kind == kSolveChain) {
    int* part = form.kind == kSolveEnvelope ? reinterpret_cast<int*>(w.xchg) : nullptr;
    if (msg) {
      hipLaunchKernelGGL(ba_env_packed_kernel, dim3(P), dim3(256), 0, st, msg, first_s, w.plan.env, n6);
      hipLaunchKernelGGL(ba_prepare_packed_kernel, dim3(P + 1), dim3(256), 0, st, msg, first_s, w.chol, w.plan.env, n6, lm, ep,
                         static_cast<long long>(kSolveLdsMax), part);
    } else {
      hipLaunchKernelGGL(ba_env_kernel, dim3((n6 * n6 + 2047) / 2048), dim3(256), 0, st, sys, w.plan.env, n6);
      hipLaunchKernelGGL(ba_prepare_kernel, dim3((n6 * n6 + n6 + 2047) / 2048), dim3(256), 0, st, sys, w.chol, w.plan.env, n6, lm, ep,
                         static_cast<long long>(kSolveLdsMax), part);
    }
    PVO_CHECK_LAUNCH();
    if (!part && hipMemsetAsync(w.xchg, 0, 16, st) != hipSuccess) return PVO_ELAUNCH;
    if (!pvo_allow_lds<ba_solve_twin_kernel>(kSolveLdsMax)) return PVO_ELAUNCH;
    hipLaunchKernelGGL(ba_solve_twin_kernel, dim3(2 + rider_blocks), dim3(256), kSolveLdsMax > rider_lds ? kSolveLdsMax : rider_lds, st,
                       w.chol, poses, w.dx, dx_out, w.plan.meta, status_out, P, t0, w.plan.env, static_cast<long long>(kSolveLdsMax), w.xchg,
                       form.chol, rider);
  } else {
    if (form.kind == kSolveBlocks) {
      hipLaunchKernelGGL(ba_prepare_kernel, dim3((n6 * n6 + n6 + 2047) / 2048), dim3(256), 0, st, sys, w.chol, w.plan.env, n6, lm, ep,
                         0LL , static_cast<int*>(nullptr));
      PVO_CHECK_LAUNCH();
      if (hipMemsetAsync(w.xchg, 0, 16, st) != hipSuccess) return PVO_ELAUNCH;
      const int nkb = (n6 + kNB - 1) / kNB, nrb = (n6 + 1 + kNB - 1) / kNB;
      for (int kb = 0; kb < nkb; ++kb) {
        hipLaunchKernelGGL(dense_panel_kernel, dim3(nrb - kb), dim3(256), 0, st, w.chol, w.ldiag, n6, kb, w.plan.meta);
        const int m = nrb - kb - 1;
        if (m > 0) hipLaunchKernelGGL(dense_update_kernel, dim3(m * (m + 1) / 2), dim3(256), 0, st, w.chol, n6, kb, nrb);
      }
      PVO_CHECK_LAUNCH();
      double* yrow = w.chol + static_cast<size_t>(n6) * n6;
      for (int kb = nkb - 1; kb >= 0; --kb)
        hipLaunchKernelGGL(dense_back_kernel, dim3(kb + 1), dim3(256), 0, st, w.chol, w.ldiag, yrow, w.xvec, n6, kb);
      PVO_CHECK_LAUNCH();
    }
    if (rider_lds > 48 * 1024 && !pvo_allow_lds<dense_finish_kernel>(kSolveLdsMax)) return PVO_ELAUNCH;
    hipLaunchKernelGGL(dense_finish_kernel, dim3(1 + rider_blocks), dim3(256), rider_lds, st, w.xvec, poses, w.dx, dx_out, w.plan.meta, status_out, P, t0, rider);
  }
  PVO_CHECK_LAUNCH();
  if (!motion_only && E + P > 0) {
    const int Kmax = (nframes < P + E) ? nframes : (P + E);
    hipLaunchKernelGGL(ba_backsub_kernel, dim3((HW + 255) / 256, Kmax > clamp_frames ? Kmax : clamp_frames), dim3(256), 0, st,
                       w.plan, jj, w.Ei, w.Eij, w.Q, w.w, w.dx, disps, dz_out, dz_rows, HW, t0, P, clamp_frames, disp_min);
    PVO_CHECK_LAUNCH();
  }
  return PVO_OK;
}

extern "C" int pvo_ba_last_partition(void* workspace, size_t workspace_bytes, int E, int P, int nframes, int HW, int* out, void* stream) {
  if (!workspace || !out || E < 0 || P < 0) return PVO_EINVAL;
  if (workspace_bytes < pvo_ba_workspace_bytes(E, P, nframes, HW)) return PVO_EWORKSPACE;
  out[0] = out[1] = 0;
  const SolveKind kind = solve_form(P, E, false, pvo_knob(PVO_KNOB_BA_SOLVER)).kind;
  if (kind == kSolveStatus || kind == kSolveDense) return PVO_OK;
  Ws w = carve(ws_base(workspace), E, P, nframes, HW);
  int host[4] = {0, 0, 0, 0};
  if (hipMemcpyAsync(host, w.xchg, sizeof(host), hipMemcpyDeviceToHost, pvo_stream(stream)) != hipSuccess) return PVO_ELAUNCH;
  if (hipStreamSynchronize(pvo_stream(stream)) != hipSuccess) return PVO_ELAUNCH;
  out[0] = host[2]; out[1] = host[3];
  return PVO_OK;
}

extern "C" int pvo_ba(float* poses, float* disps, const float* intrinsics,
                      const float* targets, const float* weights, const float* eta,
                      const int64_t* ii, const int64_t* jj,
                      int E, int nframes, int ht, int wd, int K_eta,
                      int t0, int t1, int iterations, float lm, float ep, int motion_only,
                      float* dx_out, float* dz_out, int dz_rows, int* status_out,
                      void* workspace, size_t workspace_bytes, void* stream) {
  int rc = check_common(E, nframes, ht, wd, t0, t1);
  if (rc != PVO_OK) return rc;
  if (iterations < 0) return PVO_EINVAL;
  const int P = t1 - t0, HW = ht * wd;
  if (!workspace) return PVO_EINVAL;
  if (workspace_bytes < pvo_ba_workspace_bytes(E, P, nframes, HW)) return PVO_EWORKSPACE;
  Ws w = carve(ws_base(workspace), E, P, nframes, HW);
  hipStream_t st = pvo_stream(stream);
  hipLaunchKernelGGL(ba_plan_kernel, dim3(1), dim3(256), 0, st, ii, jj, w.plan, E, nframes, t0, t1,
                     K_eta, motion_only);
  PVO_CHECK_LAUNCH();
  for (int it = 0; it < iterations; ++it) {
    rc = pvo_ba_local(poses, disps, intrinsics, targets, weights, eta, ii, jj, E, nframes, ht, wd, K_eta,
                      t0, t1, (motion_only ? 1 : 0) | (it > 0 ? 2 : 0), w.sys, workspace, workspace_bytes, stream);
    if (rc != PVO_OK) return rc;
    rc = pvo_ba_finish(poses, disps, w.sys, ii, jj, E, nframes, ht, wd, t0, t1, lm, ep, motion_only, 0, 0.0f,
                       dx_out, dz_out, dz_rows, status_out, workspace, workspace_bytes, stream);
    if (rc != PVO_OK) return rc;
  }
  return PVO_OK;
}
```

pvo_amd/csrc/common.h:

```cpp
#pragma once
#include <hip/hip_runtime.h>
#include <stdint.h>
#include <atomic>
#include <mutex>
#include "../../include/pvo_hip.h"

extern "C" void pvo_note_hip_error(int code);
#define PVO_CHECK_LAUNCH()                                   \
  do {                                                       \
    hipError_t _e = hipGetLastError();                       \
    if (_e != hipSuccess) { pvo_note_hip_error(static_cast<int>(_e)); return PVO_ELAUNCH; } \
  } while (0)

static inline hipStream_t pvo_stream(void* s) { return reinterpret_cast<hipStream_t>(s); }

struct pvo_half { _Float16 v; };
struct pvo_bf16 { uint16_t v; };

__device__ __forceinline__ float pvo_bf16_to_f32(uint16_t h) {
  return __uint_as_float(static_cast<uint32_t>(h) << 16);
}
__device__ __forceinline__ uint16_t pvo_f32_to_bf16(float f) {
  return __builtin_bit_cast(uint16_t, static_cast<__bf16>(f));
}

template <typename T> struct Elem;
template <> struct Elem<float> {
  using store_t = float;
  static __device__ __forceinline__ float to_f32(float x) { return x; }
  static __device__ __forceinline__ float from_f32(float x) { return x; }
};
template <> struct Elem<pvo_half> {
  using store_t = _Float16;
  static __device__ __forceinline__ float to_f32(_Float16 x) { return static_cast<float>(x); }
  static __device__ __forceinline__ _Float16 from_f32(float x) { return static_cast<_Float16>(x); }
};
template <> struct Elem<pvo_bf16> {
  using store_t = uint16_t;
  static __device__ __forceinline__ float to_f32(uint16_t x) { return pvo_bf16_to_f32(x); }
  static __device__ __forceinline__ uint16_t from_f32(float x) { return pvo_f32_to_bf16(x); }
};

__device__ __forceinline__ int pvo_floor_to_int(float x) {
  float f = floorf(x);
  f = fminf(fmaxf(f, -1073741824.0f), 1073741824.0f);
  return (f != f) ? 0 : static_cast<int>(f);
}

template <int CTRL>
__device__ __forceinline__ float pvo_dpp_move(float v) {
  return __int_as_float(__builtin_amdgcn_update_dpp(0, __float_as_int(v), CTRL, 0xf, 0xf, true));
}
template <int CTRL>
__device__ __forceinline__ float pvo_dpp_step(float v) { return v + pvo_dpp_move<CTRL>(v); }

__device__ __forceinline__ float pvo_wave_sum(float v) {
  v = pvo_dpp_step<0xB1>(v);
  v = pvo_dpp_step<0x4E>(v);
  v = pvo_dpp_step<0x141>(v);
  v = pvo_dpp_step<0x140>(v);
  const int b = __float_as_int(v);
  const float r0 = __int_as_float(__builtin_amdgcn_readlane(b, 0));
  const float r1 = __int_as_float(__builtin_amdgcn_readlane(b, 16));
  const float r2 = __int_as_float(__builtin_amdgcn_readlane(b, 32));
  const float r3 = __int_as_float(__builtin_amdgcn_readlane(b, 48));
  return (r0 + r1) + (r2 + r3);
}

template <typename... P>
static inline bool pvo_misaligned16(const P*... p) { return ((reinterpret_cast<uintptr_t>(p) | ...) & 15) != 0; }

template <typename T> struct pvo_dtype_code;
template <> struct pvo_dtype_code<float> { static constexpr int value = PVO_F32; };
template <> struct pvo_dtype_code<double> { static constexpr int value = PVO_F64; };
template <> struct pvo_dtype_code<pvo_half> { static constexpr int value = PVO_F16; };
template <> struct pvo_dtype_code<pvo_bf16> { static constexpr int value = PVO_BF16; };

template <typename... Ts, typename F>
static inline int pvo_dispatch(int dtype, F&& f, int otherwise = PVO_EUNSUPPORTED) {
  int rc = otherwise;
  (void)((dtype == pvo_dtype_code<Ts>::value && (rc = f(Ts{}), true)) || ...);
  return rc;
}
template <typename F>
static inline int pvo_dispatch16(int dtype, F&& f) { return pvo_dispatch<pvo_half, pvo_bf16>(dtype, f); }

template <auto Kernel>
static inline bool pvo_allow_lds(size_t bytes) {
  constexpr int kDevices = 64;
  static std::atomic<size_t> granted[kDevices];
  static std::mutex growing;
  int dev = 0;
  if (hipGetDevice(&dev) != hipSuccess) return false;
  std::atomic<size_t>* g = dev >= 0 && dev < kDevices ? &granted[dev] : nullptr;
  if (g && g->load(std::memory_order_acquire) >= bytes) return true;
  std::lock_guard<std::mutex> lock(growing);
  if (g && g->load(std::memory_order_relaxed) >= bytes) return true;
  if (hipFuncSetAttribute(reinterpret_cast<const void*>(Kernel), hipFuncAttributeMaxDynamicSharedMemorySize, static_cast<int>(bytes)) != hipSuccess)
    return false;
  if (g) g->store(bytes, std::memory_order_release);
  return true;
}
```

pvo_amd/csrc/geom.hip:

```cpp
#include "operand16.h"
#include "se3.h"

namespace {

constexpr float kMinDepthNative = 0.25f;
constexpr float kMinDepthPy = 0.2f;

struct Intr { float fx, fy, cx, cy; };
__device__ __forceinline__ Intr load_intr(const float* p) { return {p[0], p[1], p[2], p[3]}; }

__device__ __forceinline__ float pair_distance(const float* __restrict__ poses, const float* __restrict__ disps, const Intr K,
                                               int ix, int jx, int HW, int wd, float beta, int tid, float (*red)[4]) {
  const Pose G = rel_pose(load_pose(poses + 7 * static_cast<long long>(ix)), load_pose(poses + 7 * static_cast<long long>(jx)));
  const float* __restrict__ d_i = disps + static_cast<long long>(ix) * HW;

  float accum = 0.f, valid = 0.f, total = 0.f;
  for (int k = tid; k < HW; k += 256) {
    const int i = k / wd, j = k - i * wd;
    const float u = static_cast<float>(j), v = static_cast<float>(i);
    float Xi[4] = {(u - K.cx) / K.fx, (v - K.cy) / K.fy, 1.0f, d_i[k]};
    float Xj[4];
    act4(G, Xi, Xj);
    float du = K.fx * (Xj[0] / Xj[2]) + K.cx - u;
    float dv = K.fy * (Xj[1] / Xj[2]) + K.cy - v;
    float d = sqrtf(du * du + dv * dv);
    total += beta;
    if (Xj[2] > kMinDepthNative) { accum += beta * d; valid += beta; }
    Xj[0] = Xi[0] + Xi[3] * G.t.x;
    Xj[1] = Xi[1] + Xi[3] * G.t.y;
    Xj[2] = Xi[2] + Xi[3] * G.t.z;
    du = K.fx * (Xj[0] / Xj[2]) + K.cx - u;
    dv = K.fy * (Xj[1] / Xj[2]) + K.cy - v;
    d = sqrtf(du * du + dv * dv);
    total += (1.0f - beta);
    if (Xj[2] > kMinDepthNative) { accum += (1.0f - beta) * d; valid += (1.0f - beta); }
  }
  accum = pvo_wave_sum(accum); valid = pvo_wave_sum(valid); total = pvo_wave_sum(total);
  const int wave = tid >> 6;
  if ((tid & 63) == 0) { red[0][wave] = accum; red[1][wave] = valid; red[2][wave] = total; }
  __syncthreads();
  const float a = (red[0][0] + red[0][1]) + (red[0][2] + red[0][3]);
  const float va = (red[1][0] + red[1][1]) + (red[1][2] + red[1][3]);
  const float to = (red[2][0] + red[2][1]) + (red[2][2] + red[2][3]);
  return (static_cast<double>(va) / (static_cast<double>(to) + 1e-8) < 0.75) ? 1000.0f : a / va;
}

__global__ __launch_bounds__(256) void frame_distance_kernel(
    const float* __restrict__ poses, const float* __restrict__ disps, const float* __restrict__ intrinsics,
    const int64_t* __restrict__ ii, const int64_t* __restrict__ jj, float* __restrict__ dist,
    int HW, int wd, float beta) {
  const int m = blockIdx.x;
  __shared__ float red[3][4];
  const float d = pair_distance(poses, disps, load_intr(intrinsics), static_cast<int>(ii[m]), static_cast<int>(jj[m]), HW, wd, beta,
                                threadIdx.x, red);
  if (threadIdx.x == 0) dist[m] = d;
}

__global__ __launch_bounds__(512) void frame_distance_bidir_kernel(
    const float* __restrict__ poses, const float* __restrict__ disps, const float* __restrict__ intrinsics,
    const int64_t* __restrict__ ii, const int64_t* __restrict__ jj, float* __restrict__ dist,
    int HW, int wd, float beta) {
  const int m = blockIdx.x;
  const int g = threadIdx.x >> 8, tid = threadIdx.x & 255;
  __shared__ float red[2][3][4];
  __shared__ float both[2];
  const int a = static_cast<int>(ii[m]), b = static_cast<int>(jj[m]);
  const float d = pair_distance(poses, disps, load_intr(intrinsics), g ? b : a, g ? a : b, HW, wd, beta, tid, red[g]);
  if (tid == 0) both[g] = d;
  __syncthreads();
  if (threadIdx.x == 0) dist[m] = __fmul_rn(0.5f, __fadd_rn(both[0], both[1]));
}

__global__ __launch_bounds__(256) void projmap_kernel(
    const float* __restrict__ poses, const float* __restrict__ disps, const float* __restrict__ intrinsics,
    const int64_t* __restrict__ ii, const int64_t* __restrict__ jj,
    float* __restrict__ coords, float* __restrict__ valid, int HW, int wd) {
  const int e = blockIdx.y;
  const int k = blockIdx.x * 256 + threadIdx.x;
  if (k >= HW) return;
  const int ix = static_cast<int>(ii[e]), jx = static_cast<int>(jj[e]);
  const Intr K = load_intr(intrinsics);
  const Pose G = rel_pose(load_pose(poses + 7 * static_cast<long long>(ix)), load_pose(poses + 7 * static_cast<long long>(jx)));
  const int i = k / wd, j = k - i * wd;
  const float u = static_cast<float>(j), v = static_cast<float>(i);
  float Xi[4] = {(u - K.cx) / K.fx, (v - K.cy) / K.fy, 1.0f, disps[static_cast<long long>(ix) * HW + k]};
  float Xj[4];
  act4(G, Xi, Xj);
  float cu = u, cv = v;
  if (Xj[2] > 0.01f) {
    cu = K.fx * (Xj[0] / Xj[2]) + K.cx;
    cv = K.fy * (Xj[1] / Xj[2]) + K.cy;
  }
  float* c = coords + (static_cast<long long>(e) * HW + k) * 3;
  c[0] = cu; c[1] = cv; c[2] = 0.0f;
  valid[static_cast<long long>(e) * HW + k] = (Xj[2] > kMinDepthNative) ? 1.0f : 0.0f;
}

__global__ __launch_bounds__(256) void iproj_kernel(
    const float* __restrict__ poses, const float* __restrict__ disps, const float* __restrict__ intrinsics,
    float* __restrict__ points, int HW, int wd) {
  const int n = blockIdx.y;
  const int k = blockIdx.x * 256 + threadIdx.x;
  if (k >= HW) return;
  const Intr K = load_intr(intrinsics);
  const Pose G = load_pose(poses + 7 * static_cast<long long>(n));
  const int i = k / wd, j = k - i * wd;
  float Xi[4] = {(static_cast<float>(j) - K.cx) / K.fx, (static_cast<float>(i) - K.cy) / K.fy, 1.0f,
                 disps[static_cast<long long>(n) * HW + k]};
  float Xj[4];
  act4(G, Xi, Xj);
  float* p = points + (static_cast<long long>(n) * HW + k) * 3;
  p[0] = Xj[0] / Xj[3]; p[1] = Xj[1] / Xj[3]; p[2] = Xj[2] / Xj[3];
}

__global__ __launch_bounds__(256) void depth_filter_kernel(
    const float* __restrict__ poses, const float* __restrict__ disps, const float* __restrict__ intrinsics,
    const int64_t* __restrict__ inds, const float* __restrict__ thresh, float* __restrict__ counter,
    int nframes, int ht, int wd) {
  const int HW = ht * wd;
  const int b = blockIdx.z;
  const int k = blockIdx.x * 256 + threadIdx.x;
  if (k >= HW) return;
  const int ix = static_cast<int>(inds[b]);
  const Intr K = load_intr(intrinsics);
  const Pose Gi = load_pose(poses + 7 * static_cast<long long>(ix));
  const float t = thresh[b];
  const int i = k / wd, j = k - i * wd;
  const float di = disps[static_cast<long long>(ix) * HW + k];
  const float Xi[4] = {(static_cast<float>(j) - K.cx) / K.fx, (static_cast<float>(i) - K.cy) / K.fy, 1.0f, di};
  float votes = 0.f;
#pragma unroll
  for (int neigh = 0; neigh < 6; ++neigh) {
    const int jx = (neigh < 3) ? ix - neigh - 1 : ix + neigh;
    if (jx < 0 || jx >= nframes) continue;
    const Pose G = rel_pose(Gi, load_pose(poses + 7 * static_cast<long long>(jx)));
    float Xj[4];
    act4(G, Xi, Xj);
    const float uj = K.fx * (Xj[0] / Xj[2]) + K.cx;
    const float vj = K.fy * (Xj[1] / Xj[2]) + K.cy;
    const float dj = Xj[3] / Xj[2];
    const int u0 = pvo_floor_to_int(uj), v0 = pvo_floor_to_int(vj);
    if (u0 >= 0 && v0 >= 0 && u0 < wd - 1 && v0 < ht - 1) {
      const float* dm = disps + static_cast<long long>(jx) * HW;
      const float d00 = dm[v0 * wd + u0], d01 = dm[v0 * wd + u0 + 1];
      const float d10 = dm[(v0 + 1) * wd + u0], d11 = dm[(v0 + 1) * wd + u0 + 1];
      const double idj = 1.0 / static_cast<double>(dj);
      if (fabs(idj - 1.0 / static_cast<double>(d00)) < t) votes += 1.0f;
      else if (fabs(idj - 1.0 / static_cast<double>(d01)) < t) votes += 1.0f;
      else if (fabs(idj - 1.0 / static_cast<double>(d10)) < t) votes += 1.0f;
      else if (fabs(idj - 1.0 / static_cast<double>(d11)) < t) votes += 1.0f;
    }
  }
  counter[static_cast<long long>(b) * HW + k] = votes;
}

__global__ __launch_bounds__(256) void reproject_kernel(
    const float* __restrict__ poses, const float* __restrict__ disps, const float* __restrict__ intrinsics,
    const int64_t* __restrict__ ii, const int64_t* __restrict__ jj,
    float* __restrict__ coords, float* __restrict__ valid, int HW, int wd) {
  const int e = blockIdx.y;
  const int k = blockIdx.x * 256 + threadIdx.x;
  if (k >= HW) return;
  const int ix = static_cast<int>(ii[e]), jx = static_cast<int>(jj[e]);
  const Intr Ki = load_intr(intrinsics + 4 * static_cast<long long>(ix));
  const Intr Kj = load_intr(intrinsics + 4 * static_cast<long long>(jx));
  const Pose G = rel_pose(load_pose(poses + 7 * static_cast<long long>(ix)), load_pose(poses + 7 * static_cast<long long>(jx)));
  const int i = k / wd, j = k - i * wd;
  float X0[4] = {(static_cast<float>(j) - Ki.cx) / Ki.fx, (static_cast<float>(i) - Ki.cy) / Ki.fy, 1.0f,
                 disps[static_cast<long long>(ix) * HW + k]};
  float X1[4];
  act4(G, X0, X1);
  float Z = X1[2];
  Z = (Z < 0.5f * kMinDepthPy) ? 1.0f : Z;
  const float d = 1.0f / Z;
  float2 c;
  c.x = Kj.fx * (X1[0] * d) + Kj.cx;
  c.y = Kj.fy * (X1[1] * d) + Kj.cy;
  *reinterpret_cast<float2*>(coords + (static_cast<long long>(e) * HW + k) * 2) = c;
  valid[static_cast<long long>(e) * HW + k] = (X1[2] > kMinDepthPy && X0[2] > kMinDepthPy) ? 1.0f : 0.0f;
}

}

#define PVO_REQ(c) do { if (!(c)) return PVO_EINVAL; } while (0)

extern "C" int pvo_frame_distance(const float* poses, const float* disps, const float* intrinsics,
                                  const int64_t* ii, const int64_t* jj, float* dist,
                                  int M, int ht, int wd, float beta, void* stream) {
  PVO_REQ(M >= 0 && ht >= 0 && wd >= 0);
  if (M == 0) return PVO_OK;
  PVO_REQ(poses && disps && intrinsics && ii && jj && dist);
  hipLaunchKernelGGL(frame_distance_kernel, dim3(M), dim3(256), 0, pvo_stream(stream),
                     poses, disps, intrinsics, ii, jj, dist, ht * wd, wd, beta);
  PVO_CHECK_LAUNCH();
  return PVO_OK;
}

extern "C" int pvo_frame_distance_bidirectional(const float* poses, const float* disps, const float* intrinsics,
                                                const int64_t* ii, const int64_t* jj, float* dist,
                                                int M, int ht, int wd, float beta, void* stream) {
  PVO_REQ(M >= 0 && ht >= 0 && wd >= 0);
  if (M == 0) return PVO_OK;
  PVO_REQ(poses && disps && intrinsics && ii && jj && dist);
  hipLaunchKernelGGL(frame_distance_bidir_kernel, dim3(M), dim3(512), 0, pvo_stream(stream),
                     poses, disps, intrinsics, ii, jj, dist, ht * wd, wd, beta);
  PVO_CHECK_LAUNCH();
  return PVO_OK;
}

extern "C" int pvo_projmap(const float* poses, const float* disps, const float* intrinsics,
                           const int64_t* ii, const int64_t* jj, float* coords, float* valid,
                           int E, int ht, int wd, void* stream) {
  PVO_REQ(E >= 0 && ht >= 0 && wd >= 0);
  if (E == 0 || ht * wd == 0) return PVO_OK;
  PVO_REQ(poses && disps && intrinsics && ii && jj && coords && valid && E <= 65535);
  hipLaunchKernelGGL(projmap_kernel, dim3((ht * wd + 255) / 256, E), dim3(256), 0, pvo_stream(stream),
                     poses, disps, intrinsics, ii, jj, coords, valid, ht * wd, wd);
  PVO_CHECK_LAUNCH();
  return PVO_OK;
}

extern "C" int pvo_iproj(const float* poses, const float* disps, const float* intrinsics,
                         float* points, int N, int ht, int wd, void* stream) {
  PVO_REQ(N >= 0 && ht >= 0 && wd >= 0);
  if (N == 0 || ht * wd == 0) return PVO_OK;
  PVO_REQ(poses && disps && intrinsics && points && N <= 65535);
  hipLaunchKernelGGL(iproj_kernel, dim3((ht * wd + 255) / 256, N), dim3(256), 0, pvo_stream(stream),
                     poses, disps, intrinsics, points, ht * wd, wd);
  PVO_CHECK_LAUNCH();
  return PVO_OK;
}

extern "C" int pvo_depth_filter(const float* poses, const float* disps, const float* intrinsics,
                                const int64_t* ix, const float* thresh, float* counter,
                                int N, int nframes, int ht, int wd, void* stream) {
  PVO_REQ(N >= 0 && ht >= 0 && wd >= 0 && nframes >= 0);
  if (N == 0 || ht * wd == 0) return PVO_OK;
  PVO_REQ(poses && disps && intrinsics && ix && thresh && counter && N <= 65535);
  hipLaunchKernelGGL(depth_filter_kernel, dim3((ht * wd + 255) / 256, 1, N), dim3(256), 0, pvo_stream(stream),
                     poses, disps, intrinsics, ix, thresh, counter, nframes, ht, wd);
  PVO_CHECK_LAUNCH();
  return PVO_OK;
}


template <typename T>
__global__ __launch_bounds__(256) void reproject_motion_kernel(
    const float* __restrict__ poses, const float* __restrict__ disps, const float* __restrict__ intrinsics,
    const int64_t* __restrict__ ii, const int64_t* __restrict__ jj,
    float* __restrict__ coords, float* __restrict__ valid,
    const float2* __restrict__ target, const float2* __restrict__ delta_dy, const float2* __restrict__ raw_mask,
    uint16_t* __restrict__ motn, int HW, int wd) {
  const int e = blockIdx.y;
  const int k = blockIdx.x * 256 + threadIdx.x;
  if (k >= HW) return;
  const long long idx = static_cast<long long>(e) * HW + k;
  const float2 t = target[idx], dd = delta_dy[idx], m = raw_mask[idx];
  const int ix = static_cast<int>(ii[e]), jx = static_cast<int>(jj[e]);
  const Intr Ki = load_intr(intrinsics + 4 * static_cast<long long>(ix));
  const Intr Kj = load_intr(intrinsics + 4 * static_cast<long long>(jx));
  const Pose G = rel_pose(load_pose(poses + 7 * static_cast<long long>(ix)), load_pose(poses + 7 * static_cast<long long>(jx)));
  const int i = k / wd, j = k - i * wd;
  float X0[4] = {(static_cast<float>(j) - Ki.cx) / Ki.fx, (static_cast<float>(i) - Ki.cy) / Ki.fy, 1.0f,
                 disps[static_cast<long long>(ix) * HW + k]};
  float X1[4];
  act4(G, X0, X1);
  float Z = X1[2];
  Z = (Z < 0.5f * kMinDepthPy) ? 1.0f : Z;
  const float d = 1.0f / Z;
  float2 c;
  c.x = Kj.fx * (X1[0] * d) + Kj.cx;
  c.y = Kj.fy * (X1[1] * d) + Kj.cy;
  *reinterpret_cast<float2*>(coords + idx * 2) = c;
  valid[idx] = (X1[2] > kMinDepthPy && X0[2] > kMinDepthPy) ? 1.0f : 0.0f;
  const float x0 = static_cast<float>(j), y0 = static_cast<float>(i);
  const float f[8] = {t.x - x0, t.y - y0, t.x - x0 + dd.x, t.y - y0 + dd.y, t.x - c.x, t.y - c.y, m.x, m.y};
  uint32_t o[4];
#pragma unroll
  for (int q = 0; q < 4; ++q) {
    const float a = fminf(fmaxf(f[2 * q], -64.0f), 64.0f), b = fminf(fmaxf(f[2 * q + 1], -64.0f), 64.0f);
    o[q] = pvo_bits<T>(a) | (pvo_bits<T>(b) << 16);
  }
  *reinterpret_cast<uint4*>(motn + idx * 8) = make_uint4(o[0], o[1], o[2], o[3]);
}

extern "C" int pvo_reproject_motion(const float* poses, const float* disps, const float* intrinsics,
                                    const int64_t* ii, const int64_t* jj, float* coords, float* valid,
                                    const float* target, const float* delta_dy, const float* raw_mask, void* motn,
                                    int E, int ht, int wd, int dtype, void* stream) {
  PVO_REQ(E >= 0 && ht >= 0 && wd >= 0);
  if (E == 0 || ht * wd == 0) return PVO_OK;
  PVO_REQ(poses && disps && intrinsics && ii && jj && coords && valid && target && delta_dy && raw_mask && motn && E <= 65535);
  PVO_REQ(!pvo_misaligned16(motn) && !((reinterpret_cast<uintptr_t>(target) | reinterpret_cast<uintptr_t>(delta_dy) |
           reinterpret_cast<uintptr_t>(raw_mask) | reinterpret_cast<uintptr_t>(coords)) & 7));
  const dim3 grid((ht * wd + 255) / 256, E);
  auto f2 = [](const float* p) { return reinterpret_cast<const float2*>(p); };
  return pvo_dispatch16(dtype, [&](auto tag) -> int {
    using T = decltype(tag);
    hipLaunchKernelGGL(reproject_motion_kernel<T>, grid, dim3(256), 0, pvo_stream(stream), poses, disps, intrinsics, ii, jj, coords, valid,
                       f2(target), f2(delta_dy), f2(raw_mask), static_cast<uint16_t*>(motn), ht * wd, wd);
    PVO_CHECK_LAUNCH();
    return PVO_OK;
  });
}

extern "C" int pvo_reproject(const float* poses, const float* disps, const float* intrinsics,
                             const int64_t* ii, const int64_t* jj, float* coords, float* valid,
                             int E, int ht, int wd, void* stream) {
  PVO_REQ(E >= 0 && ht >= 0 && wd >= 0);
  if (E == 0 || ht * wd == 0) return PVO_OK;
  PVO_REQ(poses && disps && intrinsics && ii && jj && coords && valid && E <= 65535);
  hipLaunchKernelGGL(reproject_kernel, dim3((ht * wd + 255) / 256, E), dim3(256), 0, pvo_stream(stream),
                     poses, disps, intrinsics, ii, jj, coords, valid, ht * wd, wd);
  PVO_CHECK_LAUNCH();
  return PVO_OK;
}
```

pvo_amd/csrc/graph_glue.hip:

```cpp
#include "operand16.h"
#include "graph_post.h"

namespace {

template <typename T>
__global__ __launch_bounds__(256) void graph_motion_kernel(const float2* __restrict__ target, const float2* __restrict__ coords1,
                                                           const float2* __restrict__ delta_dy, const float2* __restrict__ raw_mask,
                                                           uint16_t* __restrict__ motn, int E, int HW, int W) {
  const int idx = blockIdx.x * 256 + threadIdx.x;
  if (idx >= E * HW) return;
  const int pix = idx % HW;
  const float x0 = static_cast<float>(pix % W), y0 = static_cast<float>(pix / W);
  const float2 t = target[idx], c1 = coords1[idx], d = delta_dy[idx], m = raw_mask[idx];
  float f[8] = {t.x - x0, t.y - y0, t.x - x0 + d.x, t.y - y0 + d.y, t.x - c1.x, t.y - c1.y, m.x, m.y};
  uint32_t o[4];
#pragma unroll
  for (int k = 0; k < 4; ++k) {
    const float a = fminf(fmaxf(f[2 * k], -64.0f), 64.0f), b = fminf(fmaxf(f[2 * k + 1], -64.0f), 64.0f);
    o[k] = pvo_bits<T>(a) | (pvo_bits<T>(b) << 16);
  }
  *reinterpret_cast<uint4*>(motn + static_cast<size_t>(idx) * 8) = make_uint4(o[0], o[1], o[2], o[3]);
}

template <typename T>
__global__ __launch_bounds__(256) void graph_post_kernel(GraphPostArgs g, const uint16_t* __restrict__ y8, int E, int HW, int W,
                                                         const int* __restrict__ segm, const int* __restrict__ vote_tot,
                                                         const int* __restrict__ vote_dyn, int S, float vote_thresh) {
  const int idx = blockIdx.x * 256 + threadIdx.x;
  if (idx >= E * HW) return;
  const int e = idx / HW, pix = idx - e * HW;
  const uint4 q = *reinterpret_cast<const uint4*>(y8 + static_cast<size_t>(idx) * 8);
  graph_post_pixel<T>(idx, e, pix, q, g, HW, W, segm, vote_tot, vote_dyn, S, vote_thresh);
}

}


extern "C" int pvo_graph_motion(const float* target, const float* coords1, const float* delta_dy, const float* raw_mask,
                                void* motn, int E, int H, int W, int dtype, void* stream) {
  if (E < 0 || H < 0 || W < 0) return PVO_EINVAL;
  const long long n = static_cast<long long>(E) * H * W;
  if (n == 0) return PVO_OK;
  if (!target || !coords1 || !delta_dy || !raw_mask || !motn || n >= (1LL << 31)) return PVO_EINVAL;
  if (pvo_misaligned16(motn) || ((reinterpret_cast<uintptr_t>(target) | reinterpret_cast<uintptr_t>(coords1) |
       reinterpret_cast<uintptr_t>(delta_dy) | reinterpret_cast<uintptr_t>(raw_mask)) & 7)) return PVO_EINVAL;
  hipStream_t st = pvo_stream(stream);
  const dim3 grid(static_cast<unsigned>((n + 255) / 256));
  auto f2 = [](const float* p) { return reinterpret_cast<const float2*>(p); };
  return pvo_dispatch16(dtype, [&](auto tag) -> int {
    using T = decltype(tag);
    hipLaunchKernelGGL(graph_motion_kernel<T>, grid, dim3(256), 0, st, f2(target), f2(coords1), f2(delta_dy), f2(raw_mask), static_cast<uint16_t*>(motn), E, H * W, W);
    PVO_CHECK_LAUNCH();
    return PVO_OK;
  });
}

extern "C" int pvo_graph_post(const float* coords1, const void* heads, float* raw_mask, float* target, float* delta_dy,
                              float* weight, float* target_ba, float* weight_ba, float* full_flow,
                              int E, int H, int W, float dy_thresh, const int* segm, const int* vote_tot, const int* vote_dyn,
                              int max_segments, float vote_thresh, int dtype, void* stream) {
  if (E < 0 || H < 0 || W < 0) return PVO_EINVAL;
  const long long n = static_cast<long long>(E) * H * W;
  if (n == 0) return PVO_OK;
  if (!coords1 || !heads || !raw_mask || !target || !delta_dy || !weight || !target_ba || !weight_ba || !full_flow || n >= (1LL << 31)) return PVO_EINVAL;
  if (pvo_misaligned16(heads)) return PVO_EINVAL;
  if (segm && (!vote_tot || !vote_dyn || max_segments <= 0)) return PVO_EINVAL;
  hipStream_t st = pvo_stream(stream);
  const dim3 grid(static_cast<unsigned>((n + 255) / 256));
  auto f2 = [](float* p) { return reinterpret_cast<float2*>(p); };
  const GraphPostArgs g = {reinterpret_cast<const float2*>(coords1), f2(raw_mask), f2(target), f2(delta_dy), f2(weight), target_ba, weight_ba, f2(full_flow), dy_thresh};
  return pvo_dispatch16(dtype, [&](auto tag) -> int {
    using T = decltype(tag);
    hipLaunchKernelGGL(graph_post_kernel<T>, grid, dim3(256), 0, st, g, static_cast<const uint16_t*>(heads), E, H * W, W, segm, vote_tot, vote_dyn, max_segments, vote_thresh);
    PVO_CHECK_LAUNCH();
    return PVO_OK;
  });
}
```

pvo_amd/csrc/se3.h:

```cpp
#pragma once
#include "common.h"

struct Quat { float x, y, z, w; };
struct Vec3 { float x, y, z; };
struct Pose { Vec3 t; Quat q; };

__device__ __forceinline__ Pose load_pose(const float* p) {
  Pose P; P.t = {p[0], p[1], p[2]}; P.q = {p[3], p[4], p[5], p[6]}; return P;
}

__device__ __forceinline__ Vec3 cross3(const Vec3 a, const Vec3 b) {
  return {a.y * b.z - a.z * b.y, a.z * b.x - a.x * b.z, a.x * b.y - a.y * b.x};
}

__device__ __forceinline__ Vec3 rotate(const Quat q, const Vec3 v) {
  const Vec3 qv = {q.x, q.y, q.z};
  Vec3 uv = cross3(qv, v);
  uv = {2.0f * uv.x, 2.0f * uv.y, 2.0f * uv.z};
  const Vec3 c = cross3(qv, uv);
  return {v.x + q.w * uv.x + c.x, v.y + q.w * uv.y + c.y, v.z + q.w * uv.z + c.z};
}

__device__ __forceinline__ Quat qconj(const Quat q) { return {-q.x, -q.y, -q.z, q.w}; }

__device__ __forceinline__ Quat qmul(const Quat a, const Quat b) {
  return {a.w * b.x + a.x * b.w + a.y * b.z - a.z * b.y,
          a.w * b.y + a.y * b.w + a.z * b.x - a.x * b.z,
          a.w * b.z + a.z * b.w + a.x * b.y - a.y * b.x,
          a.w * b.w - a.x * b.x - a.y * b.y - a.z * b.z};
}

__device__ __forceinline__ Pose rel_pose(const Pose Gi, const Pose Gj) {
  Pose G;
  G.q = qmul(Gj.q, qconj(Gi.q));
  const Vec3 r = rotate(G.q, Gi.t);
  G.t = {Gj.t.x - r.x, Gj.t.y - r.y, Gj.t.z - r.z};
  return G;
}

__device__ __forceinline__ void act4(const Pose G, const float X[4], float Y[4]) {
  const Vec3 r = rotate(G.q, {X[0], X[1], X[2]});
  Y[0] = r.x + X[3] * G.t.x;
  Y[1] = r.y + X[3] * G.t.y;
  Y[2] = r.z + X[3] * G.t.z;
  Y[3] = X[3];
}

__device__ __forceinline__ void adjT(const Pose G, const float X[6], float Y[6]) {
  const Quat qi = qconj(G.q);
  const Vec3 a = rotate(qi, {X[0], X[1], X[2]});
  const Vec3 b = rotate(qi, {X[3], X[4], X[5]});
  const Vec3 u = {G.t.z * X[1] - G.t.y * X[2], G.t.x * X[2] - G.t.z * X[0], G.t.y * X[0] - G.t.x * X[1]};
  const Vec3 v = rotate(qi, u);
  Y[0] = a.x; Y[1] = a.y; Y[2] = a.z;
  Y[3] = b.x + v.x; Y[4] = b.y + v.y; Y[5] = b.z + v.z;
}

__device__ __forceinline__ Quat exp_so3(const Vec3 phi) {
  const float th2 = phi.x * phi.x + phi.y * phi.y + phi.z * phi.z;
  const float th4 = th2 * th2;
  const float th = sqrtf(th2);
  float imag, real;
  if (th2 < 1e-8f) {
    imag = 0.5f - (1.0f / 48.0f) * th2 + (1.0f / 3840.0f) * th4;
    real = 1.0f - (1.0f / 8.0f) * th2 + (1.0f / 384.0f) * th4;
  } else {
    imag = sinf(0.5f * th) / th;
    real = cosf(0.5f * th);
  }
  return {imag * phi.x, imag * phi.y, imag * phi.z, real};
}

__device__ __forceinline__ Pose exp_se3(const float xi[6]) {
  Pose G;
  const Vec3 phi = {xi[3], xi[4], xi[5]};
  G.q = exp_so3(phi);
  Vec3 tau = {xi[0], xi[1], xi[2]};
  const float th2 = phi.x * phi.x + phi.y * phi.y + phi.z * phi.z;
  const float th = sqrtf(th2);
  G.t = tau;
  if (th > 1e-4f) {
    const float a = (1.0f - cosf(th)) / th2;
    tau = cross3(phi, tau);
    G.t = {G.t.x + a * tau.x, G.t.y + a * tau.y, G.t.z + a * tau.z};
    const float b = (th - sinf(th)) / (th * th2);
    tau = cross3(phi, tau);
    G.t = {G.t.x + b * tau.x, G.t.y + b * tau.y, G.t.z + b * tau.z};
  }
  return G;
}

__device__ __forceinline__ Pose retract(const float xi[6], const Pose T) {
  const Pose d = exp_se3(xi);
  Pose R;
  R.q = qmul(d.q, T.q);
  const Vec3 r = rotate(d.q, T.t);
  R.t = {r.x + d.t.x, r.y + d.t.y, r.z + d.t.z};
  return R;
}
```

pvo_amd/csrc/update_exec.hip:

```cpp
#include "common.h"
#include "graph_post.h"
#include <stdlib.h>

int pvo_segment_hist_ws(const int* segm, const float* raw_mask, const void* heads, int* tot, int* dyn,
                        int E, int HW, int S, float dy_thresh, int dtype, void* stream);

namespace {

struct SideCtx { hipStream_t side; hipEvent_t fork, join, mid; bool ok; };

constexpr unsigned g_event_flags = hipEventDisableTiming | hipEventDisableSystemFence;
SideCtx g_side_ctx[64] = {};
SideCtx* side_ctx() {
  SideCtx* ctx = g_side_ctx;
  int dev = 0;
  if (hipGetDevice(&dev) != hipSuccess || dev < 0 || dev >= 64) return nullptr;
  SideCtx& c = ctx[dev];
  if (!c.ok) {
    int least = 0, greatest = 0;
    if (hipDeviceGetStreamPriorityRange(&least, &greatest) != hipSuccess) return nullptr;
    if (hipStreamCreateWithPriority(&c.side, hipStreamNonBlocking, greatest) != hipSuccess) return nullptr;
    if (hipEventCreateWithFlags(&c.fork, g_event_flags) != hipSuccess) return nullptr;
    if (hipEventCreateWithFlags(&c.join, g_event_flags) != hipSuccess) return nullptr;
    if (hipEventCreateWithFlags(&c.mid, g_event_flags) != hipSuccess) return nullptr;
    c.ok = true;
  }
  return &c;
}

size_t al(size_t x) { return (x + 255) & ~static_cast<size_t>(255); }

struct ContextAhead { const void *ws, *weights, *glo_w, *gate_wt, *net; int E, H, W, dtype; bool valid; };
ContextAhead g_ctx_ahead[64] = {};
ContextAhead* ctx_ahead_slot() {
  int dev = 0;
  if (hipGetDevice(&dev) != hipSuccess || dev < 0 || dev >= 64) return nullptr;
  return &g_ctx_ahead[dev];
}

struct Probe { int stage; int cap; int limit; int n; int every; int seen; hipEvent_t* ev; };
Probe g_probe = {-1, 0, 0, 0, 1, 0, nullptr};

inline void probe_mark(int stage, int which, void* stream) {
  if (g_probe.stage != stage || g_probe.n >= g_probe.limit) return;
  if (g_probe.seen % g_probe.every == 0) {
    (void)hipEventRecord(g_probe.ev[2 * g_probe.n + which], pvo_stream(stream));
    if (which == 1) ++g_probe.n;
  }
  if (which == 1) ++g_probe.seen;
}

struct OpWs {
  char *c1, *f1, *CF, *Z, *RN, *h1, *a1, *am, *a2, *P_zr, *P_q;
  float *part, *g;
  size_t bytes;
};

OpWs carve_op(void* base, int E, int K, int H, int W, int chunks) {
  OpWs w{};
  char* p = static_cast<char*>(base);
  size_t off = 0;
  auto take = [&](size_t bytes) { char* r = p ? p + off : nullptr; off += al(bytes); return r; };
  const size_t px = static_cast<size_t>(E) * H * W, kpx = static_cast<size_t>(K) * H * W;
  w.c1 = take(px * 128 * 2); w.f1 = take(px * 128 * 2); w.CF = take(px * 192 * 2);
  w.Z = take(px * 128 * 2); w.RN = take(px * 128 * 2); w.h1 = take(px * 72 * 4);
  w.a1 = take(px * 128 * 2); w.am = take(kpx * 128 * 2); w.a2 = take(kpx * 128 * 2);
  w.P_zr = take(px * 256 * 2); w.P_q = take(px * 128 * 2);
  w.part = reinterpret_cast<float*>(take(static_cast<size_t>(E) * chunks * 128 * 4));
  w.g = reinterpret_cast<float*>(take(static_cast<size_t>(E) * 384 * 4));
  w.bytes = off;
  return w;
}

struct UpWs {
  float *coords, *valid, *eta;
  char *motion, *heads, *upmask;
  int *vote_tot, *vote_dyn;
  void* op;
  size_t bytes;
};

UpWs carve_up(void* base, int E, int K, int R, int H, int W, int S, size_t op_bytes) {
  UpWs w{};
  char* p = static_cast<char*>(base);
  size_t off = 0;
  auto take = [&](size_t bytes) { char* r = p ? p + off : nullptr; off += al(bytes); return r; };
  const size_t px = static_cast<size_t>(E) * H * W;
  w.coords = reinterpret_cast<float*>(take(px * 2 * 4));
  w.valid = reinterpret_cast<float*>(take(px * 4));
  w.eta = reinterpret_cast<float*>(take(static_cast<size_t>(R > 0 ? R : 1) * H * W * 4));
  w.motion = take(px * 8 * 2);
  w.heads = take(px * 8 * 2);
  w.upmask = take(static_cast<size_t>(K) * H * W * 576 * 2);
  w.vote_tot = reinterpret_cast<int*>(take(static_cast<size_t>(E) * (S > 0 ? S : 0) * 4 + 4));
  w.vote_dyn = reinterpret_cast<int*>(take(static_cast<size_t>(E) * (S > 0 ? S : 0) * 4 + 4));
  w.op = take(op_bytes);
  w.bytes = off;
  return w;
}

void* ws_base(void* workspace) {
  return reinterpret_cast<void*>((reinterpret_cast<uintptr_t>(workspace) + 255) & ~static_cast<uintptr_t>(255));
}


#define RUN(call)                    \
  do {                               \
    const int rc_ = (call);          \
    if (rc_ != PVO_OK) return rc_;   \
  } while (0)

struct MotionJob {
  const float *target, *coords, *delta_dy, *raw_mask; void* motion;
};

int run_trunk(const pvo_update_weights* w, const pvo_operator_args* a, OpWs& b, void* stream, const void** P_zr, const void** P_q,
              const MotionJob* mj, bool context_ready = false) {
  const int E = a->E, H = a->H, W = a->W, dt = w->dtype;
  const long long rows = static_cast<long long>(E) * H * W;
  hipStream_t st = pvo_stream(stream);
  SideCtx* sc = (w->flags & PVO_OP_ENC_SIDE_STREAM) && !(w->flags & PVO_OP_SINGLE_STREAM) ? side_ctx() : nullptr;
  void* s2 = sc ? static_cast<void*>(sc->side) : stream;
  void* s3 = stream;
  if (sc) {
    if (hipEventRecord(sc->fork, st) != hipSuccess) return PVO_ELAUNCH;
    if (hipStreamWaitEvent(sc->side, sc->fork, 0) != hipSuccess) return PVO_ELAUNCH;
  }
  if (a->levels[0]) {
    probe_mark(PVO_STAGE_EMPTY, 0, stream);
    probe_mark(PVO_STAGE_EMPTY, 1, stream);
    probe_mark(PVO_STAGE_LOOKUP, 0, stream);
    RUN(pvo_corr_lookup_encode_tiled(a->levels, a->coords, w->enc0_w, w->enc0_b, b.c1, E, H, W, dt, a->slots, a->num_slots, stream));
    probe_mark(PVO_STAGE_LOOKUP, 1, stream);
  } else {
    if (!a->corr) return PVO_EINVAL;
    RUN(pvo_corr_encode(a->corr, w->enc0_w, w->enc0_b, b.c1, rows, dt, stream));
  }
  if (mj) RUN(pvo_graph_motion(mj->target, mj->coords, mj->delta_dy, mj->raw_mask, mj->motion, E, H, W, dt, s2));
  RUN(pvo_conv7x7_c8(a->motion, w->fenc0_w, w->fenc0_b, b.f1, E, H, W, dt, s2));
  RUN(pvo_conv3x3_c128(b.f1, w->fenc2_w, w->fenc2_b, b.CF, E, H, W, 64, 1, 192, 128, dt, s2));
  if (sc && hipEventRecord(sc->join, sc->side) != hipSuccess) return PVO_ELAUNCH;
  if (w->flags & PVO_OP_CONV128_WIDE)
    RUN(pvo_conv3x3(b.c1, w->cenc2_w, w->cenc2_b, b.CF, E, H, W, 128, 128, 1, 192, 0, dt, stream));
  else
    RUN(pvo_conv3x3_c128(b.c1, w->cenc2_w, w->cenc2_b, b.CF, E, H, W, 128, 1, 192, 0, dt, stream));
  if (!context_ready) {
    RUN(pvo_gru_glo_fused(a->net, w->glo_w, w->glo_b, b.part, E, H * W, dt, s3));
    RUN(pvo_gate_context(b.part, w->gate_wt, w->gate_b, b.g, E, pvo_gru_glo_chunks(H * W), s3));
  }
  *P_zr = a->P_zr; *P_q = a->P_q;
  if (!a->P_zr || !a->P_q) {
    if (!a->inp) return PVO_EINVAL;
    RUN(pvo_conv3x3(a->inp, w->zr_inp_w, nullptr, b.P_zr, E, H, W, 128, 256, 0, 0, 0, dt, stream));
    RUN(pvo_conv3x3(a->inp, w->q_inp_w, nullptr, b.P_q, E, H, W, 128, 128, 0, 0, 0, dt, stream));
    *P_zr = b.P_zr; *P_q = b.P_q;
  }
  if (sc && hipStreamWaitEvent(st, sc->join, 0) != hipSuccess) return PVO_ELAUNCH;
  probe_mark(PVO_STAGE_GATES, 0, stream);
  const int* ps = (a->static_by_slot && a->P_zr && a->P_q) ? a->slots : nullptr;
  if (a->static_by_slot && !a->slots) return PVO_EINVAL;
  RUN(pvo_gru_conv_gates(a->net, b.CF, 192, w->zr_w, b.g, *P_zr, ps, b.Z, b.RN, E, H, W, dt, stream));
  probe_mark(PVO_STAGE_GATES, 1, stream);
  probe_mark(PVO_STAGE_CANDIDATE, 0, stream);
  RUN(pvo_gru_conv_candidate(b.RN, b.CF, 192, w->q_w, b.g, *P_q, ps, b.Z, a->net, a->net_out, E, H, W, dt, stream));
  probe_mark(PVO_STAGE_CANDIDATE, 1, stream);
  return PVO_OK;
}

int run_heads(const pvo_update_weights* w, const pvo_operator_args* a, OpWs& b, void* stream,
              const GraphPostArgs* post = nullptr, int* post_fused = nullptr) {
  const int E = a->E, H = a->H, W = a->W, dt = w->dtype;
  RUN(pvo_conv3x3_heads(a->net_out, w->heads1_w, w->heads1_b, w->heads2_w, reinterpret_cast<float*>(b.h1), E, H, W, dt, stream));
  RUN(pvo_internal_heads_gather_post(reinterpret_cast<const float*>(b.h1), w->heads2_b, a->heads, post, post_fused, E, H, W, dt, stream));
  return PVO_OK;
}

int run_upmask(const pvo_update_weights* w, const pvo_operator_args* a, OpWs& b, void* stream) {
  if (a->K <= 0 || !a->upmask) return PVO_OK;
  return pvo_conv1x1_c128(b.a2, w->up_w, w->up_b, a->upmask, static_cast<long long>(a->K) * a->H * a->W, 576, 0, w->dtype, stream);
}

int run_agg(const pvo_update_weights* w, const pvo_operator_args* a, OpWs& b, void* stream, SideCtx* mark = nullptr, bool with_upmask = true) {
  const int E = a->E, H = a->H, W = a->W, K = a->K, dt = w->dtype;
  if (K <= 0) return PVO_OK;
  if (w->flags & PVO_OP_CONV128_WIDE)
    RUN(pvo_conv3x3(a->net_out, w->agg1_w, nullptr, b.a1, E, H, W, 128, 128, 0, 0, 0, dt, stream));
  else
    RUN(pvo_conv3x3_c128(a->net_out, w->agg1_w, nullptr, b.a1, E, H, W, 128, 0, 0, 0, dt, stream));
  RUN(pvo_segment_mean(b.a1, a->seg_ptr, a->seg_idx, w->agg1_b, b.am, K, H * W, 128, dt, stream));
  RUN(pvo_conv3x3_c128(b.am, w->agg2_w, w->agg2_b, b.a2, K, H, W, 128, 1, 0, 0, dt, stream));
  if (a->eta)
    RUN(pvo_eta_head(b.a2, w->eta_w, w->eta_b, a->eta_frame, a->eta_pos, a->damping, a->eta, a->eta_frame ? a->R : K, H, W, a->EP, a->eta_scale, dt, stream));
  if (mark && hipEventRecord(mark->mid, pvo_stream(stream)) != hipSuccess) return PVO_ELAUNCH;
  if (with_upmask) RUN(run_upmask(w, a, b, stream));
  return PVO_OK;
}

int check_op(const pvo_update_weights* w, const pvo_operator_args* a) {
  if (!w || !a) return PVO_EINVAL;
  if (w->dtype != PVO_F16 && w->dtype != PVO_BF16) return PVO_EUNSUPPORTED;
  if (a->E < 0 || a->H <= 0 || a->W <= 0 || a->K < 0) return PVO_EINVAL;
  if (a->E > 0 && (!a->net || !a->net_out || !a->heads)) return PVO_EINVAL;
  if (a->K > 0 && (!a->seg_ptr || !a->seg_idx)) return PVO_EINVAL;
  return PVO_OK;
}

int run_operator(const pvo_update_weights* w, const pvo_operator_args* a, OpWs& b, void* stream, SideCtx** pending,
                 const MotionJob* mj = nullptr, bool upmask_on_side = true, bool context_ready = false,
                 const GraphPostArgs* post = nullptr, int* post_fused = nullptr) {
  const void *P_zr, *P_q;
  RUN(run_trunk(w, a, b, stream, &P_zr, &P_q, mj, context_ready));
  hipStream_t st = pvo_stream(stream);
  SideCtx* sc = (a->K > 0 && !(w->flags & PVO_OP_SINGLE_STREAM)) ? side_ctx() : nullptr;
  if (sc) {
    if (hipEventRecord(sc->fork, st) != hipSuccess) return PVO_ELAUNCH;
    if (hipStreamWaitEvent(sc->side, sc->fork, 0) != hipSuccess) return PVO_ELAUNCH;
    RUN(run_agg(w, a, b, sc->side, sc, upmask_on_side));
    if (hipEventRecord(sc->join, sc->side) != hipSuccess) return PVO_ELAUNCH;
    RUN(run_heads(w, a, b, stream, post, post_fused));
    *pending = sc;
  } else {
    RUN(run_heads(w, a, b, stream, post, post_fused));
    RUN(run_agg(w, a, b, stream, nullptr, upmask_on_side));
    *pending = nullptr;
  }
  return PVO_OK;
}

int join(SideCtx* sc, void* stream) {
  if (sc && hipStreamWaitEvent(pvo_stream(stream), sc->join, 0) != hipSuccess) return PVO_ELAUNCH;
  return PVO_OK;
}

__global__ __launch_bounds__(256) void clamp_min_kernel(float* __restrict__ x, long long n, float lo) {
  const long long i = static_cast<long long>(blockIdx.x) * 256 + threadIdx.x;
  if (i < n) { const float v = x[i]; x[i] = (v < lo) ? lo : v; }
}

}

extern "C" size_t pvo_operator_workspace_bytes(int E, int K, int H, int W) {
  if (E < 0 || K < 0 || H <= 0 || W <= 0) return 0;
  return carve_op(nullptr, E, K, H, W, pvo_gru_glo_chunks(H * W)).bytes + 256;
}

extern "C" int pvo_update_operator(const pvo_update_weights* w, const pvo_operator_args* a,
                                   void* workspace, size_t workspace_bytes, void* stream) {
  RUN(check_op(w, a));
  if (a->E == 0) return PVO_OK;
  if (!workspace || workspace_bytes < pvo_operator_workspace_bytes(a->E, a->K, a->H, a->W)) return PVO_EWORKSPACE;
  if (!a->motion) return PVO_EINVAL;
  OpWs b = carve_op(ws_base(workspace), a->E, a->K, a->H, a->W, pvo_gru_glo_chunks(a->H * a->W));
  if (ContextAhead* ca = ctx_ahead_slot()) ca->valid = false;
  SideCtx* pending = nullptr;
  RUN(run_operator(w, a, b, stream, &pending));
  return join(pending, stream);
}

extern "C" size_t pvo_graph_update_workspace_bytes(int E, int K, int R, int H, int W, int max_segments) {
  if (E < 0 || K < 0 || R < 0 || H <= 0 || W <= 0 || max_segments < 0) return 0;
  return carve_up(nullptr, E, K, R, H, W, max_segments, pvo_operator_workspace_bytes(E, K, H, W)).bytes + 256;
}

extern "C" int pvo_graph_update(const pvo_update_weights* w, const pvo_graph_update_args* u,
                                void* workspace, size_t workspace_bytes, void* stream) {
  if (!w || !u) return PVO_EINVAL;
  pvo_operator_args a = u->op;
  a.net_out = a.net_out ? a.net_out : const_cast<void*>(a.net);
  a.heads = reinterpret_cast<void*>(1);
  RUN(check_op(w, &a));
  const int E = a.E, H = a.H, W = a.W, K = a.K, R = a.R, dt = w->dtype, HW = H * W;
  if (E == 0) return PVO_OK;
  if (!a.levels[0]) return PVO_EUNSUPPORTED;
  if (!u->poses || !u->disps || !u->intrinsics || !u->ii || !u->jj || !u->target || !u->delta_dy || !u->raw_mask ||
      !u->weight || !u->full_flow || !u->target_ba || !u->weight_ba || !u->ii_ba || !u->jj_ba || !u->sys || !u->ba_ws)
    return PVO_EINVAL;
  if (K <= 0 || R <= 0 || !a.eta_frame || !a.eta_pos || !a.damping || u->n_in < 0) return PVO_EINVAL;
  const int S = u->segm ? u->max_segments : 0;
  if (u->segm && S <= 0) return PVO_EINVAL;
  if (!workspace || workspace_bytes < pvo_graph_update_workspace_bytes(E, K, R, H, W, S)) return PVO_EWORKSPACE;
  const size_t op_bytes = pvo_operator_workspace_bytes(E, K, H, W);
  UpWs s = carve_up(ws_base(workspace), E, K, R, H, W, S, op_bytes);
  OpWs b = carve_op(ws_base(s.op), E, K, H, W, pvo_gru_glo_chunks(HW));
  hipStream_t st = pvo_stream(stream);

  probe_mark(PVO_STAGE_UPDATE, 0, stream);
  RUN(pvo_reproject_motion(u->poses, u->disps, u->intrinsics, u->ii, u->jj, s.coords, s.valid, u->target, u->delta_dy, u->raw_mask,
                           s.motion, E, H, W, dt, stream));
  a.coords = s.coords; a.corr = nullptr; a.motion = s.motion; a.heads = s.heads;
  a.eta = u->op.eta ? u->op.eta : s.eta;
  if (u->want_upmask && !a.upmask) a.upmask = s.upmask;
  const bool ahead_off = pvo_knob(PVO_KNOB_NO_RIDERS) != 0;
  ContextAhead* ca = ctx_ahead_slot();
  const bool ctx_ready = ca && ca->valid && u->context_ready && !ahead_off && ca->ws == workspace && ca->weights == w &&
                         ca->glo_w == w->glo_w && ca->gate_wt == w->gate_wt && ca->net == a.net && ca->E == E && ca->H == H &&
                         ca->W == W && ca->dtype == dt;
  if (ca) ca->valid = false;
  SideCtx* pending = nullptr;
  float* const tba = u->target_ba + static_cast<size_t>(u->n_in) * 2 * HW;
  float* const wba = u->weight_ba + static_cast<size_t>(u->n_in) * 2 * HW;
  const GraphPostArgs gpa = {reinterpret_cast<const float2*>(s.coords), reinterpret_cast<float2*>(u->raw_mask), reinterpret_cast<float2*>(u->target),
                             reinterpret_cast<float2*>(u->delta_dy), reinterpret_cast<float2*>(u->weight), tba, wba,
                             reinterpret_cast<float2*>(u->full_flow), u->dy_thresh};
  const bool post_in_gather = !u->segm && pvo_knob(PVO_KNOB_POST_SEPARATE) == 0;
  int post_fused = 0;
  RUN(run_operator(w, &a, b, stream, &pending, nullptr, false, ctx_ready, post_in_gather ? &gpa : nullptr, &post_fused));
  if (u->segm)
    RUN(pvo_segment_hist_ws(u->segm, u->raw_mask, s.heads, s.vote_tot, s.vote_dyn, E, HW, S, u->dy_thresh, dt, stream));
  if (!post_fused)
    RUN(pvo_graph_post(s.coords, s.heads, u->raw_mask, u->target, u->delta_dy, u->weight, tba, wba,
                       u->full_flow, E, H, W, u->dy_thresh, u->segm, u->segm ? s.vote_tot : nullptr, u->segm ? s.vote_dyn : nullptr,
                       S, u->vote_thresh, dt, stream));
  const bool rider_off = pvo_knob(PVO_KNOB_NO_RIDERS) != 0;
  const bool rider_fits = static_cast<long long>(K) * HW <= (1LL << 24) &&
                          !pvo_misaligned16(b.a2, w->up_w, a.upmask);
  const bool mask_rides = u->itrs > 0 && a.K > 0 && a.upmask && !rider_off && rider_fits;
  const bool context_ahead = u->context_ahead && u->itrs >= 2 && !u->motion_only && !ahead_off;
  if (pending && hipStreamWaitEvent(st, pending->mid, 0) != hipSuccess) return PVO_ELAUNCH;
  if (!mask_rides) RUN(run_upmask(w, &a, b, stream));
  const int Eb = u->n_in + E;
  probe_mark(PVO_STAGE_BA, 0, stream);
  for (int it = 0; it < u->itrs; ++it) {
    const bool last = it + 1 == u->itrs;
    RUN(pvo_ba_local(u->poses, u->disps, u->intrinsics, u->target_ba, u->weight_ba, a.eta, u->ii_ba, u->jj_ba, Eb, u->nframes,
                     H, W, R, u->t0, u->t1, (u->motion_only ? 1 : 0) | 2, u->sys, u->ba_ws, u->ba_ws_bytes, stream));
    pvo_ba_riders jobs{};
    if (mask_rides && it == 0) {
      jobs.cx = b.a2; jobs.cw = w->up_w; jobs.cbias = w->up_b; jobs.cy = a.upmask;
      jobs.crows = static_cast<long long>(K) * HW; jobs.cCout = 576; jobs.cdtype = dt;
    }
    if (context_ahead && it == 0) {
      jobs.gnet = a.net_out; jobs.gw = w->glo_w; jobs.gbias = w->glo_b; jobs.gpart = b.part; jobs.gE = E; jobs.gHW = HW; jobs.gdtype = dt;
    }
    if (context_ahead && it == 1) {
      jobs.xpart = b.part; jobs.xwt = w->gate_wt; jobs.xbias = w->gate_b; jobs.xg = b.g; jobs.xE = E; jobs.xchunks = pvo_gru_glo_chunks(HW);
    }
    RUN(pvo_ba_finish_riders(u->poses, u->disps, u->sys, u->ii_ba, u->jj_ba, Eb, u->nframes, H, W, u->t0, u->t1, u->lm, u->ep,
                             u->motion_only, last && !u->motion_only ? u->clamp_frames : 0, u->disp_min,
                             nullptr, nullptr, 0, nullptr, u->ba_ws, u->ba_ws_bytes, &jobs, stream));
  }
  probe_mark(PVO_STAGE_BA, 1, stream);
  if (u->clamp_frames > 0 && (u->itrs == 0 || u->motion_only)) {
    const long long n = static_cast<long long>(u->clamp_frames) * HW;
    hipLaunchKernelGGL(clamp_min_kernel, dim3(static_cast<unsigned>((n + 255) / 256)), dim3(256), 0, st, u->disps, n, u->disp_min);
    PVO_CHECK_LAUNCH();
  }
  if (ca && context_ahead)
    *ca = ContextAhead{workspace, w, w->glo_w, w->gate_wt, a.net_out, E, H, W, dt, true};
  probe_mark(PVO_STAGE_UPDATE, 1, stream);
  return PVO_OK;
}

extern "C" int pvo_side_stream(void** stream_out) {
  if (!stream_out) return PVO_EINVAL;
  SideCtx* sc = side_ctx();
  if (!sc) return PVO_ELAUNCH;
  *stream_out = static_cast<void*>(sc->side);
  return PVO_OK;
}

extern "C" int pvo_probe_arm_every(int stage, int capacity, int every) {
  if (capacity < 0 || every < 1) return PVO_EINVAL;
  if (capacity > g_probe.cap) {
    hipEvent_t* ev = static_cast<hipEvent_t*>(realloc(g_probe.ev, sizeof(hipEvent_t) * 2 * capacity));
    if (!ev) return PVO_EINVAL;
    for (int i = 2 * g_probe.cap; i < 2 * capacity; ++i)
      if (hipEventCreate(&ev[i]) != hipSuccess) return PVO_ELAUNCH;
    g_probe.ev = ev; g_probe.cap = capacity;
  }
  g_probe.n = 0; g_probe.seen = 0; g_probe.limit = capacity; g_probe.every = every;
  g_probe.stage = capacity > 0 ? stage : -1;
  return PVO_OK;
}

extern "C" int pvo_probe_arm(int stage, int capacity) { return pvo_probe_arm_every(stage, capacity, 1); }

extern "C" int pvo_probe_read(float* ms_host, int max_n) {
  const int n = g_probe.n < max_n ? g_probe.n : max_n;
  for (int i = 0; i < n; ++i) {
    if (hipEventSynchronize(g_probe.ev[2 * i + 1]) != hipSuccess) return -1;
    if (hipEventElapsedTime(&ms_host[i], g_probe.ev[2 * i], g_probe.ev[2 * i + 1]) != hipSuccess) return -1;
  }
  g_probe.stage = -1;
  return n;
}
```

pvo_amd/factor_graph.py:

```python
import contextlib

import itertools
import torch

from .modules.corr import CorrBlock, CorrVolumePool


def coords_grid(ht, wd, device):
    y, x = torch.meshgrid(torch.arange(ht, device=device).float(), torch.arange(wd, device=device).float(),
                          indexing="ij")
    return torch.stack([x, y], dim=-1)


class _EdgeRows:

    def __init__(self, capacity):
        self.capacity = capacity
        self.buf = [None, None]
        self.cur = 0

    def _fits(self, rows):
        b = self.buf[self.cur]
        return b is not None and b.dtype == rows.dtype and b.device == rows.device and tuple(b.shape[1:]) == tuple(rows.shape[1:])

# ... 360 lines not shown
        jmax = max(self._jj_h + self._ii_h) if sharded is not None else max(self._jj_h)
        chunks = []
        for i in range(0, jmax + 1, 8):
            sel = [k for k, a in enumerate(self._ii_h) if i <= a < i + 8]
            if sel:
                chunks.append((torch.tensor(sel, device=self.device), sorted({self._ii_h[k] for k in sel})))
        src_l = sorted(set(self._ii_h))
        src = torch.tensor(src_l, device=self.device)
        if sharded is not None:
            rows_l = sorted(set(range(1, t)) | set(src_l))
            row_of_src = torch.tensor([rows_l.index(f) for f in src_l], device=self.device)
        for _ in range(steps):
            coords1, _ = self.video.reproject(self.ii, self.jj)
            cam = self.target_cam - self.coords0
            motn = torch.cat([cam, cam + self.delta_dy, self.target_cam - coords1, self.raw_mask], dim=-1)
            motn = motn.permute(0, 1, 4, 2, 3).clamp(-64.0, 64.0)
            for v, srcs in chunks:
                iis, jjs = self.ii[v], self.jj[v]
                corr1 = corr_op(coords1[:, v], iis, jjs)
                with torch.autocast("cuda", dtype=torch.float16, enabled=self._autocast and self.device.type == "cuda"):
                    net, delta, weight, damping, _, delta_m = self.update_op(
                        self.net[:, v], self.video.inps[iis][None], corr1, motn[:, v], iis, jjs, False)
                self.net[:, v] = net.to(self.net.dtype)
                self.target_cam[:, v] = coords1[:, v] + delta[..., 0:2].float()
                self.damping[torch.tensor(srcs, device=self.device)] = damping[0].float()
                raw = self.raw_mask[:, v] + delta_m.float()
                self.raw_mask[:, v] = raw
                bin_mask = (torch.sigmoid(raw) >= self.dy_thresh).float()
                self.delta_dy[:, v] = delta[..., 2:4].float() * (1 - bin_mask)
                self.weight[:, v] = torch.sigmoid(weight.float() + (1 - bin_mask) * 10)
            eta = self.damping[src].contiguous() + EP
            target = self.target_cam.view(-1, ht, wd, 2).permute(0, 3, 1, 2).contiguous()
            weight = self.weight.view(-1, ht, wd, 2).permute(0, 3, 1, 2).contiguous()
            if sharded is None:
                self.video.ba(target, weight, eta, self.ii, self.jj, 1, t, itrs=itrs, lm=1e-5, ep=1e-2, motion_only=False)
            else:
                eta_rows = torch.ones(len(rows_l), ht, wd, dtype=eta.dtype, device=self.device)
                eta_rows[row_of_src] = eta
                sharded.ba(self.video.poses, self.video.disps, self.video.intrinsics[0], target, weight, eta_rows,
                           self.ii.contiguous(), self.jj.contiguous(), 1, t, itrs=itrs, lm=1e-5, ep=1e-2,
                           plan_key=(id(self), self._version, t))
                self.video.disps.clamp_(min=0.001)
            self.video.dirty[:t] = True

    def add_neighborhood_factors(self, t0, t1, r=3):
        ii, jj = [], []
        for i in range(t0, t1):
            for j in range(t0, t1):
                if i != j and abs(i - j) <= r:
                    ii.append(i); jj.append(j)
        self.add_factors(ii, jj)

    def _agg_segments_host(self):
        frames = sorted(set(self._ii_h))
        pos = {f: k for k, f in enumerate(frames)}
        buckets = [[] for _ in frames]
        for e, i in enumerate(self._ii_h):
            buckets[pos[i]].append(e)
        ptr, idx = [0], []
        for b in buckets:
            idx += b
            ptr.append(len(idx))
        return ptr, idx, len(frames)

    def _agg_segments(self):
        from .droid_backends import to_device_async
        ptr, idx, n = self._agg_segments_host()
        both = to_device_async(ptr + idx, torch.int32, self.device)
        return both[:len(ptr)], both[len(ptr):], n

    def prefetch_proximity(self, t0, t1, t, beta):
        if self.device.type != "cuda" or t - t0 <= 0 or t - t1 <= 0:
            return
        import numpy as np
        nj = t - t1
        ii, jj = np.repeat(np.arange(t0, t), nj), np.tile(np.arange(t1, t), t - t0)
        d = self.video.distance(ii, jj, beta=beta).float().reshape(-1)
        st = self.__dict__.get("_prox_stage")
        if st is None or st[0].numel() < d.numel():
            st = self.__dict__["_prox_stage"] = (torch.empty(max(4096, d.numel()), dtype=torch.float32).pin_memory(), torch.cuda.Event())
        st[0][:d.numel()].copy_(d, non_blocking=True)
        st[1].record()
        self._prox_prefetch = {"key": (t0, t1, t, float(beta)), "host": st[0], "ready": st[1]}

    def add_proximity_factors(self, t0=0, t1=0, rad=2, nms=2, beta=0.25, thresh=16.0, remove=False):
        t = self.video.counter
        ix, jx = list(range(t0, t)), list(range(t1, t))
        if not ix or not jx:
            return
        import numpy as np
        ni, nj = len(ix), len(jx)
        ii, jj = np.repeat(np.arange(t0, t), nj), np.tile(np.arange(t1, t), ni)
        pf = self.__dict__.pop("_prox_prefetch", None)
        if pf is not None and pf["key"] == (t0, t1, t, float(beta)):
            pf["ready"].synchronize()
            D32 = pf["host"][:ni * nj].numpy().reshape(ni, nj)
        else:
            D32 = self.video.distance(ii, jj, beta=beta).float().cpu().numpy().reshape(ni, nj)
        if self.native_select:
            from . import droid_backends as db
            have_i = np.array(list(self._ii_h) + self.ii_bad.tolist() + list(self._ii_inac_h), dtype=np.int64)
            have_j = np.array(list(self._jj_h) + self.jj_bad.tolist() + list(self._jj_inac_h), dtype=np.int64)
            ei, ej = db.proximity_select(D32, t0, t1, rad, nms, thresh, have_i, have_j)
            if ei:
                self.add_factors(ei, ej, remove)
            return
        D = D32.astype(np.float64)
        I = np.arange(t0, t)[:, None]
        J = np.arange(t1, t)[None, :]
        D = np.where((I - rad < J) | ~(D <= 100), np.inf, D)
        offsets = [(di, dj) for di in range(-nms, nms + 1) for dj in range(-nms, nms + 1)]

        def suppress_many(hi, hj):
            r = np.maximum(np.minimum(np.abs(hi - hj) - 2, nms), 0)
            for di, dj in offsets:
                m = (abs(di) + abs(dj) <= r)
                a, b = hi[m] + di - t0, hj[m] + dj - t1
                ok = (a >= 0) & (a < ni) & (b >= 0) & (b < nj)
                D[a[ok], b[ok]] = np.inf

        diamonds = [np.add.outer(np.abs(np.arange(-r, r + 1)), np.abs(np.arange(-r, r + 1))) <= r for r in range(nms + 1)]

        def suppress_one(i, j):
            r = max(min(abs(i - j) - 2, nms), 0)
            a0, b0 = i - r - t0, j - r - t1
            a1, b1 = a0 + 2 * r + 1, b0 + 2 * r + 1
            ca0, cb0, ca1, cb1 = max(a0, 0), max(b0, 0), min(a1, ni), min(b1, nj)
            if ca0 < ca1 and cb0 < cb1:
                D[ca0:ca1, cb0:cb1][diamonds[r][ca0 - a0:ca1 - a0, cb0 - b0:cb1 - b0]] = np.inf

        have_i = np.array(list(self._ii_h) + self.ii_bad.tolist() + list(self._ii_inac_h), dtype=np.int64)
        have_j = np.array(list(self._jj_h) + self.jj_bad.tolist() + list(self._jj_inac_h), dtype=np.int64)
        far = np.abs(have_i - have_j) > 2
        if far.any():
            suppress_many(have_i[far], have_j[far])
        es = []
        for i in range(t0, t):
            for j in range(i + 1, min(i + rad + 1, t)):
                es += [(i, j), (j, i)]
        flat = D.ravel()
        order = np.argsort(flat, kind="stable")
        order = order[:int(np.count_nonzero(flat <= thresh))]
        for k in order.tolist():
            if not flat[k] <= thresh:
                continue
            i, j = int(ii[k]), int(jj[k])
            es += [(i, j), (j, i)]
            suppress_one(i, j)
        if es:
            self.add_factors([e[0] for e in es], [e[1] for e in es], remove)

    def _segment_vote(self, bin_mask):
        E = bin_mask.shape[1]
        S = self.video.max_segments
        seg = self.segm[0, :, 0].long().clamp_(0, S - 1)
        dyn = ((bin_mask[0, ..., 0] == 0) | (bin_mask[0, ..., 1] == 0))
        key = (torch.arange(E, device=seg.device).view(E, 1, 1) * S + seg).reshape(-1)
        tot = torch.bincount(key, minlength=E * S).float()
        dcn = torch.bincount(key, weights=dyn.reshape(-1).float(), minlength=E * S)
        forced = (dcn / tot.clamp(min=1) > self.video.thresh) & (torch.arange(E * S, device=seg.device) % S != 0)
        keep = ~forced[key].view(1, E, *seg.shape[1:])
        return bin_mask & keep.unsqueeze(-1)

    def _op_dtype(self):
        dt = next(self.update_op.parameters()).dtype
        return dt if dt in (torch.float16, torch.bfloat16) else torch.float16

    def _fused_ok(self):
        return self.fused_glue and self._static_ok()

    def _static_ok(self):
        if self.device.type != "cuda" or self.corr_impl != "volume":
            return False
        if self.corr is not None and not getattr(self.corr, "tiled", False):
            return False
        if self.corr is None and not (self.video.fmaps.dtype in (torch.float16, torch.bfloat16)):
            return False
        op = self.update_op
        if not hasattr(op, "packed_weights") or getattr(op, "training", True) or not getattr(op, "fused_gru", False) \
                or getattr(op, "use_aff_bri", False):
            return False
        if self.corr is None:
            from . import droid_backends as db
            return db.tiled_supported(self.ht, self.wd, self.video.fmaps.dtype)
        return True

    def _ba_plan(self, ii, jj, t0, t1, motion_only, n_in, R):
        from . import droid_backends as db
        v = self.video
        F, ht, wd = v.disps.shape
        P = t1 - t0
        key = (self._version, t0, t1, n_in, bool(motion_only), int(ii.shape[0]), int(R))
        st = self.__dict__.get("_ba_state")
        if st is None or st["key"] != key:
            need = db.ba_workspace_bytes(int(ii.shape[0]), P, F, ht * wd)
            ws = st["ws"] if st is not None and st["ws"].numel() >= need else \
                torch.empty(need + (need >> 2), dtype=torch.uint8, device=self.device)
            n6 = 6 * P
            sysb = st["sys"] if st is not None and st["sys"].numel() >= n6 * n6 + n6 else \
                torch.zeros(max(n6 * n6 + n6, 1), dtype=torch.int64, device=self.device)
            db.ba_plan(ii, jj, F, ht * wd, -1 if motion_only else int(R), t0, t1, ws)
            st = self.__dict__["_ba_state"] = {"key": key, "ws": ws, "sys": sysb, "ii": ii, "jj": jj}
        return st

    @torch.no_grad()
    def _update_fused(self, t0, t1, itrs, use_inactive, EP, motion_only, eta_scale=0.2, lm=1e-4, ep=0.1, sharded=None,
                      segm_vote=True):
        from . import droid_backends as db
        from ._lib import GraphUpdateArgs
        from .droid_backends import to_device_packed
        v = self.video
        ht, wd = self.ht, self.wd
        E = len(self._ii_h)
        dt = self._op_dtype()
        if t0 is None:
            t0 = max(1, min(self._ii_h) + 1)
        if t1 is None:
            t1 = max(max(self._ii_h), max(self._jj_h)) + 1
        vote = bool(segm_vote and v.segm_filter)
        S = (v.segments_bound() if hasattr(v, "segments_bound") else v.max_segments) if vote else 0
        key = (self._version, t0, t1, bool(use_inactive), bool(motion_only), E, float(eta_scale), float(lm), float(ep), sharded is not None,
               vote, S)
        st = self._cache.get("fused")
        if st is None or st["key"] != key:
            src = sorted(set(self._ii_h))
            m_l = [(i >= t0 - 3) and (j >= t0 - 3) for i, j in zip(self._ii_inac_h, self._jj_inac_h)] if use_inactive else []
            n_in = sum(m_l)
            rows = sorted(set(src) | {i for i, k in zip(self._ii_inac_h, m_l) if k} | set(range(t0, t1)))
            where = {f: k for k, f in enumerate(src)}
            seg_ptr, seg_idx, nseg = self._agg_segments_host()
            parts = [(rows, torch.long), ([where.get(f, -1) for f in rows], torch.int32), (seg_ptr, torch.int32),
                     (seg_idx, torch.int32), (self.corr.slots, torch.int32), ([k for k, f in enumerate(m_l) if f], torch.long)]
            if self._index_dirty:
                parts += [(self._ii_h, torch.long), (self._jj_h, torch.long), (self._age_h, torch.long)]
            up = to_device_packed(parts, self.device)
            frames_t, pos_t, seg, slots_t, m = up[0], up[1], (up[2], up[3], nseg), up[4], up[5]
            if self._index_dirty:
                self._ii_dev, self._jj_dev, self._age_dev = up[6], up[7], up[8]
                self._age_lag, self._index_dirty = 0, False
            self._cache["agg"] = seg
            self.corr._slots_t = slots_t
            target_ba = torch.empty(n_in + E, 2, ht, wd, device=self.device)
            weight_ba = torch.empty(n_in + E, 2, ht, wd, device=self.device)
            if n_in:
                ii_ba, jj_ba = torch.cat([self.ii_inac[m], self.ii]), torch.cat([self.jj_inac[m], self.jj])
                target_ba[:n_in] = self.target_cam_inac[0, m].permute(0, 3, 1, 2)
                weight_ba[:n_in] = self.weight_inac[0, m].permute(0, 3, 1, 2)
            else:
                ii_ba, jj_ba = self.ii.contiguous(), self.jj.contiguous()
            if sharded is None:
                ba = self._ba_plan(ii_ba, jj_ba, t0, t1, motion_only, n_in, len(rows))
            else:
                ba = {"ii": ii_ba.contiguous(), "jj": jj_ba.contiguous(), "sys": None, "ws": None}
            st = self._cache["fused"] = dict(
                key=key, n_in=n_in, target_ba=target_ba, weight_ba=weight_ba, ii_ba=ba["ii"], jj_ba=ba["jj"], frames=frames_t,
                pos=pos_t, seg=seg, ba=ba, R=len(rows), S=S, ii=self.ii.contiguous(), jj=self.jj.contiguous(),
                slots=self.corr.slots_tensor(),
                segm=self.segm[0, :, 0].to(torch.int32).contiguous() if vote else None,
                full_flow=torch.empty(1, E, ht, wd, 2, device=self.device),
                eta=torch.empty(len(rows), ht, wd, device=self.device) if sharded is not None else None,
                ws=db.graph_update_workspace(E, seg[2], len(rows), ht, wd, S, self.device), args=GraphUpdateArgs())
            a = st["args"]
            db._fill_operator_args(a.op, E, ht, wd, self.corr.levels, st["slots"], self.corr.capacity, None, None, None, None, None,
                                   None, None, None, seg, None, (frames_t, pos_t, self.damping, EP, eta_scale), st["eta"], None)
            a.nframes = v.disps.shape[0]
            a.poses, a.disps, a.intrinsics = v.poses.data_ptr(), v.disps.data_ptr(), v.intrinsics.data_ptr()
            a.ii, a.jj = st["ii"].data_ptr(), st["jj"].data_ptr()
            a.segm = st["segm"].data_ptr() if st["segm"] is not None else None
            a.max_segments, a.vote_thresh, a.dy_thresh = S, float(v.thresh), float(self.dy_thresh)
            a.n_in, a.target_ba, a.weight_ba = n_in, target_ba.data_ptr(), weight_ba.data_ptr()
            a.ii_ba, a.jj_ba = st["ii_ba"].data_ptr(), st["jj_ba"].data_ptr()
            a.t0, a.t1, a.motion_only, a.lm, a.ep = t0, t1, 1 if motion_only else 0, float(lm), float(ep)
            if sharded is None:
                a.sys, a.ba_ws, a.ba_ws_bytes = ba["sys"].data_ptr(), ba["ws"].data_ptr(), ba["ws"].numel()
            else:
                dummy = st["dummy"] = torch.zeros(64, dtype=torch.int64, device=self.device)
                a.sys, a.ba_ws, a.ba_ws_bytes = dummy.data_ptr(), dummy.data_ptr(), dummy.numel() * 8
            a.clamp_frames, a.disp_min = v.disps.shape[0], 0.001
            a.want_upmask = 1 if self.want_upmask else 0
        a = st["args"]
        for n in ("target_cam", "delta_dy", "raw_mask", "weight"):
            t = getattr(self, n)
            if not t.is_contiguous() or t.dtype != torch.float32:
                setattr(self, n, t.float().contiguous())
        net = self.net[0]
        if net.dtype != dt or not net.is_contiguous(memory_format=torch.channels_last):
            net = net.to(dt).contiguous(memory_format=torch.channels_last)
            self.net = net[None]
        a.op.net = a.op.net_out = net.data_ptr()
        a.op.P_zr, a.op.P_q = self.P_zr.data_ptr(), self.P_q.data_ptr()
        a.op.static_by_slot = 1 if self._static_by_slot else 0
        a.op.EP = float(EP)
        a.target, a.delta_dy, a.raw_mask = self.target_cam.data_ptr(), self.delta_dy.data_ptr(), self.raw_mask.data_ptr()
        if tuple(self.weight.shape) != (1, E, ht, wd, 2):
            self.weight = torch.empty(1, E, ht, wd, 2, device=self.device)
        self.full_flow = st["full_flow"]
        a.weight, a.full_flow = self.weight.data_ptr(), self.full_flow.data_ptr()
        a.itrs = int(itrs) if sharded is None else 0
        a.clamp_frames = v.disps.shape[0] if sharded is None else 0
        weights = self.update_op.packed_weights(dt)
        token = (net.data_ptr(), net._version, st.setdefault("serial", next(_CACHE_SERIAL)), weights.serial)
        a.context_ahead = 1
        a.context_ready = 1 if getattr(self, "_ctx_token", None) == token else 0
        db.graph_update(weights, a, st["ws"])
        self._ctx_token = token
        if sharded is not None:
            sharded.ba(v.poses, v.disps, v.intrinsics[0], st["target_ba"], st["weight_ba"], st["eta"], st["ii_ba"], st["jj_ba"],
                       t0, t1, itrs=itrs, lm=lm, ep=ep, motion_only=motion_only, plan_key=(id(self), self._version, t0, t1))
            v.disps.clamp_(min=0.001)
        self._age_lag += 1
        self._age_h = [x + 1 for x in self._age_h]

    @property
    def inp(self):
        if self._inp is None and self._static_by_slot and self._ii_h:
            return self._cached("inp", lambda: self._cl5(self.video.inps[self.ii][None]))
        return self._inp

    @inp.setter
    def inp(self, t):
        self._inp = t

    @property
    def segm(self):
        if self._segm is None and self._ii_h and not getattr(self.video, "segm_filter", True):
            return self._cached("segm", lambda: self.video.segms[self.ii][None])
        return self._segm

    @segm.setter
    def segm(self, t):
        self._segm = t

    @property
    def age(self):
        if self._index_dirty:
            self._sync_edge_index()
        if self._age_lag:
            self._age_dev += self._age_lag
            self._age_lag = 0
        return self._age_dev

    @age.setter
    def age(self, t):
        if self._index_dirty:
            self._sync_edge_index()
        self._age_dev, self._age_lag = t, 0

    @torch.no_grad()
    def update(self, t0=None, t1=None, itrs=2, use_inactive=False, EP=1e-7, motion_only=False):
        self._corr_sync()
        if self._fused_ok() and self.P_zr is not None:
            return self._update_fused(t0, t1, itrs, use_inactive, EP, motion_only)
        ht, wd = self.ht, self.wd
        coords1, _ = self.video.reproject(self.ii, self.jj)
        motn = torch.cat([self.target_cam - self.coords0, self.target_cam - self.coords0 + self.delta_dy,
                          self.target_cam - coords1, self.raw_mask], dim=-1)
        motn = motn.permute(0, 1, 4, 2, 3).clamp(-64.0, 64.0)
        if self.corr is None:
            corr = None
        elif getattr(self.corr, "supports_channels_last", False):
            corr = self.corr(coords1, channels_last=True)
        else:
            corr = self.corr(coords1)
        with torch.autocast("cuda", dtype=torch.float16, enabled=self._autocast and self.device.type == "cuda"):
            kw = {}
            if getattr(self.update_op, "agg", None) is not None and self.device.type == "cuda":
                kw["agg_segments"] = self._cached("agg", self._agg_segments)
            self.net, delta, weight, damping, upmask, delta_m = \
                self.update_op(self.net, self.inp, corr, motn, self.ii, self.jj, False, **kw)
        if t0 is None:
            t0 = max(1, min(self._ii_h) + 1)
        if t1 is None:
            t1 = max(max(self._ii_h), max(self._jj_h)) + 1
        self.target_cam = coords1 + delta[..., 0:2].float()
        self.raw_mask = self.raw_mask + delta_m.float()
        bin_mask = torch.sigmoid(self.raw_mask) >= self.dy_thresh
        if self.video.segm_filter:
            bin_mask = self._segment_vote(bin_mask)
        bin_mask = bin_mask.float()
        self.delta_dy = delta[..., 2:4].float() * (1 - bin_mask)
        self.weight = torch.sigmoid(weight.float() + (1 - bin_mask) * 10)
        src = sorted(set(self._ii_h))
        src_t = self._cached("src", lambda: torch.tensor(src, device=self.device))
        self.damping[src_t] = damping[0].float()
        m_l = [(i >= t0 - 3) and (j >= t0 - 3) for i, j in zip(self._ii_inac_h, self._jj_inac_h)] if use_inactive else []
        if any(m_l):
            m = self._cached(("inac", t0), lambda: torch.tensor(m_l, dtype=torch.bool, device=self.device))
            ii, jj = torch.cat([self.ii_inac[m], self.ii]), torch.cat([self.jj_inac[m], self.jj])
            target_cam = torch.cat([self.target_cam_inac[:, m], self.target_cam], 1)
            weight = torch.cat([self.weight_inac[:, m], self.weight], 1)
            src2 = sorted(set(src) | {i for i, k in zip(self._ii_inac_h, m_l) if k})
            src_t = self._cached(("src2", t0), lambda: torch.tensor(src2, device=self.device))
        else:
            ii, jj, target_cam, weight = self.ii, self.jj, self.target_cam, self.weight
        eta = 0.2 * self.damping[src_t] + EP
        target_cam = target_cam.view(-1, ht, wd, 2).permute(0, 3, 1, 2).contiguous()
        weight = weight.view(-1, ht, wd, 2).permute(0, 3, 1, 2).contiguous()
        self.video.ba(target_cam, weight, eta, ii, jj, t0, t1, itrs=itrs, lm=1e-4, ep=0.1, motion_only=motion_only)
        self.full_flow = coords1 + self.delta_dy - self.coords0
        self.age += 1
        self._age_h = [a + 1 for a in self._age_h]
```

Measured before the change: 245.4 keyframe updates/s.

## Fuse next update's reprojection into final BA backsubstitution kernel

The last BA iteration's back-substitution kernel now also computes the reprojection and motion features for the next graph update, using the freshly updated disparity and poses. A per-device record and a Python-side token of tensor pointers and versions let the next call skip its standalone reproject_motion launch when nothing changed in between. Shared SE3 math is split into a contract-off variant so the fused and standalone paths produce matching results. In exchange the back-substitution kernel does more work per pixel, and the bookkeeping adds risk of reusing stale coordinates if the invalidation checks miss a change.

```diff
diff --git a/include/pvo_hip.h b/include/pvo_hip.h
--- a/include/pvo_hip.h
+++ b/include/pvo_hip.h
@@ -20,7 +20,7 @@
 
 const char* pvo_strerror(int code);
 const char* pvo_last_hip_error(void);
-#define PVO_ABI_VERSION 105
+#define PVO_ABI_VERSION 106
 int pvo_version(void);
 size_t pvo_graph_update_args_size(void);
 
@@ -190,6 +190,7 @@
   int clamp_frames; float disp_min;
   int want_upmask;
   int context_ahead, context_ready;
+  int reproject_ahead, reproject_ready;
 } pvo_graph_update_args;
 
 size_t pvo_graph_update_workspace_bytes(int E, int K, int R, int H, int W, int max_segments);
diff --git a/pvo_amd/_lib.py b/pvo_amd/_lib.py
--- a/pvo_amd/_lib.py
+++ b/pvo_amd/_lib.py
@@ -5,7 +5,7 @@
 LIB_PATH = os.path.join(_HERE, "libpvo_hip.so")
 
 PVO_F32, PVO_F16, PVO_BF16, PVO_F64 = 0, 1, 2, 3
-PVO_ABI_VERSION = 105
+PVO_ABI_VERSION = 106
 
 _c = ctypes
 _vp, _i, _f, _sz = _c.c_void_p, _c.c_int, _c.c_float, _c.c_size_t
@@ -121,7 +121,7 @@
                 ("n_in", _i), ("target_ba", _vp), ("weight_ba", _vp), ("ii_ba", _vp), ("jj_ba", _vp),
                 ("t0", _i), ("t1", _i), ("itrs", _i), ("motion_only", _i), ("lm", _f), ("ep", _f),
                 ("sys", _vp), ("ba_ws", _vp), ("ba_ws_bytes", _sz), ("clamp_frames", _i), ("disp_min", _f),
-                ("want_upmask", _i), ("context_ahead", _i), ("context_ready", _i)]
+                ("want_upmask", _i), ("context_ahead", _i), ("context_ready", _i), ("reproject_ahead", _i), ("reproject_ready", _i)]
 
 
 PVO_OP_CONV128_WIDE, PVO_OP_SINGLE_STREAM, PVO_OP_ENC_SIDE_STREAM = 1, 2, 4
diff --git a/pvo_amd/csrc/ba.hip b/pvo_amd/csrc/ba.hip
--- a/pvo_amd/csrc/ba.hip
+++ b/pvo_amd/csrc/ba.hip
@@ -1,4 +1,5 @@
 #include "se3.h"
+#include "reproject_body.h"
 #include "conv1x1_tile.h"
 #include "glo_tile.h"
 #include <stdlib.h>
@@ -2586,20 +2587,22 @@
   solve_epilogue([&](int i) { return xvec[i]; }, meta[4] | meta[2], true, 0, P, t0, poses, dx_ws, dx_out, meta, status_out, true, [] {});
 }
 
+template <typename T>
 __device__ __forceinline__ void ba_backsub_body(
     const Plan& pl, const int64_t* __restrict__ jj, const float* __restrict__ Ei, const float* __restrict__ Eij,
     const float* __restrict__ Q, const float* __restrict__ w, const float* __restrict__ dx,
     float* __restrict__ disps, float* __restrict__ dz_out, int dz_rows, int HW, int t0, int P,
-    int clamp_frames, float disp_min) {
+    int clamp_frames, float disp_min, const ReprojAhead& ahead, int wd) {
   const int k = blockIdx.y;
   const int x = blockIdx.x * 256 + threadIdx.x;
   __shared__ int s_edge[256], s_pose[256];
   __shared__ float s_dx[256][6];
-  const bool live = k < pl.meta[0] && !pl.meta[2];
-  const int e0 = live ? pl.eptr[k] : 0, deg = live ? pl.eptr[k + 1] - e0 : 0;
+  const bool planned = k < pl.meta[0];
+  const bool live = planned && !pl.meta[2];
+  const int e0 = planned ? pl.eptr[k] : 0, deg = planned ? pl.eptr[k + 1] - e0 : 0;
   const bool in_lds = deg <= 255;
   constexpr int lo = 1;
-  if (live && in_lds && static_cast<int>(threadIdx.x) <= deg) {
+  if (planned && in_lds && static_cast<int>(threadIdx.x) <= deg) {
     const int r = static_cast<int>(threadIdx.x) - 1;
     int e = 0, p;
     if (r < 0) p = pl.kx[k] - t0;
@@ -2617,7 +2620,9 @@
     const float v = disps[static_cast<long long>(k) * HW + x];
     if (v < disp_min) disps[static_cast<long long>(k) * HW + x] = disp_min;
   }
-  if (!live) return;
+  if (!planned) return;
+  float d;
+  if (live) {
   float acc = 0.0f;
   if (in_lds) {
     for (int q = 0; q <= deg; ++q) {
@@ -2640,19 +2645,32 @@
     }
   }
   const float dz = Q[static_cast<long long>(k) * HW + x] * (w[static_cast<long long>(k) * HW + x] - acc);
-  float d = disps[static_cast<long long>(pl.kx[k]) * HW + x] + dz;
+  d = disps[static_cast<long long>(pl.kx[k]) * HW + x] + dz;
   if (pl.kx[k] < clamp_frames && d < disp_min) d = disp_min;
   disps[static_cast<long long>(pl.kx[k]) * HW + x] = d;
   if (dz_out && k < dz_rows) dz_out[static_cast<long long>(k) * HW + x] = dz;
   BA_WG_PROBE(2, 2);
-}
-
+  } else {
+    if constexpr (std::is_void<T>::value) return;
+    d = disps[static_cast<long long>(pl.kx[k]) * HW + x];
+  }
+  if constexpr (!std::is_void<T>::value) {
+    const int ix = pl.kx[k];
+    for (int q = 0; q < deg; ++q) {
+      const int e = in_lds ? s_edge[q + 1] : pl.eidx[e0 + q];
+      if (e < ahead.n_in) continue;
+      reproject_motion_pixel<T>(ahead.poses, ahead.intrinsics, ix, static_cast<int>(jj[e]), e - ahead.n_in, x, d, HW, wd, ahead.out);
+    }
+  }
+}
+
+template <typename T>
 __global__ __launch_bounds__(256) void ba_backsub_kernel(
     Plan pl, const int64_t* __restrict__ jj, const float* __restrict__ Ei, const float* __restrict__ Eij,
     const float* __restrict__ Q, const float* __restrict__ w, const float* __restrict__ dx,
     float* __restrict__ disps, float* __restrict__ dz_out, int dz_rows, int HW, int t0, int P,
-    int clamp_frames, float disp_min) {
-  ba_backsub_body(pl, jj, Ei, Eij, Q, w, dx, disps, dz_out, dz_rows, HW, t0, P, clamp_frames, disp_min);
+    int clamp_frames, float disp_min, const ReprojAhead ahead, int wd) {
+  ba_backsub_body<T>(pl, jj, Ei, Eij, Q, w, dx, disps, dz_out, dz_rows, HW, t0, P, clamp_frames, disp_min, ahead, wd);
 }
 
 int check_common(int E, int F, int ht, int wd, int t0, int t1) {
@@ -2789,7 +2807,7 @@
                           float lm, float ep, int motion_only, int clamp_frames, float disp_min,
                           float* dx_out, float* dz_out, int dz_rows, int* status_out,
                           void* workspace, size_t workspace_bytes,
-                          const pvo_ba_riders* jobs, void* stream);
+                          const pvo_ba_riders* jobs, const ReprojAhead* ahead, void* stream);
 
 extern "C" int pvo_ba_finish_riders(float* poses, float* disps, void* sys_,
                                     const int64_t* ii, const int64_t* jj,
@@ -2800,7 +2818,22 @@
                                     const pvo_ba_riders* jobs, void* stream) {
   if (!sys_) return PVO_EINVAL;
   return ba_finish_impl(poses, disps, sys_, nullptr, nullptr, ii, jj, E, nframes, ht, wd, t0, t1, lm, ep, motion_only, clamp_frames, disp_min,
-                        dx_out, dz_out, dz_rows, status_out, workspace, workspace_bytes, jobs, stream);
+                        dx_out, dz_out, dz_rows, status_out, workspace, workspace_bytes, jobs, nullptr, stream);
+}
+
+int pvo_internal_ba_finish_ahead(float* poses, float* disps, void* sys_, const int64_t* ii, const int64_t* jj,
+                                 int E, int nframes, int ht, int wd, int t0, int t1,
+                                 float lm, float ep, int motion_only, int clamp_frames, float disp_min,
+                                 void* workspace, size_t workspace_bytes,
+                                 const pvo_ba_riders* jobs, const ReprojAhead* ahead, int* rode, void* stream) {
+  if (!sys_ || !ahead || !rode) return PVO_EINVAL;
+  if (!ahead->intrinsics || !ahead->out.coords || !ahead->out.valid || !ahead->out.target || !ahead->out.delta_dy || !ahead->out.raw_mask ||
+      !ahead->out.motn || ahead->n_in < 0 || ahead->n_in > E)
+    return PVO_EINVAL;
+  if (ahead->dtype != PVO_F16 && ahead->dtype != PVO_BF16) return PVO_EUNSUPPORTED;
+  *rode = (!motion_only && E + (t1 - t0) > 0) ? 1 : 0;
+  return ba_finish_impl(poses, disps, sys_, nullptr, nullptr, ii, jj, E, nframes, ht, wd, t0, t1, lm, ep, motion_only, clamp_frames, disp_min,
+                        nullptr, nullptr, 0, nullptr, workspace, workspace_bytes, jobs, ahead, stream);
 }
 
 extern "C" size_t pvo_ba_packed_elems(const int* first_host, int P) {
@@ -2832,7 +2865,7 @@
                                     void* workspace, size_t workspace_bytes, void* stream) {
   if (!msg || !first_s) return PVO_EINVAL;
   return ba_finish_impl(poses, disps, nullptr, static_cast<const long long*>(msg), first_s, ii, jj, E, nframes, ht, wd, t0, t1, lm, ep, motion_only,
-                        clamp_frames, disp_min, dx_out, dz_out, dz_rows, status_out, workspace, workspace_bytes, nullptr, stream);
+                        clamp_frames, disp_min, dx_out, dz_out, dz_rows, status_out, workspace, workspace_bytes, nullptr, nullptr, stream);
 }
 
 enum SolveKind { kSolveStatus, kSolveDense, kSolveEnvelope, kSolveChain, kSolveBlocks };
@@ -2853,7 +2886,8 @@
                           float lm, float ep, int motion_only, int clamp_frames, float disp_min,
                           float* dx_out, float* dz_out, int dz_rows, int* status_out,
                           void* workspace, size_t workspace_bytes,
-                          const pvo_ba_riders* jobs, void* stream) {
+                          const pvo_ba_riders* jobs, const ReprojAhead* ahead, void* stream) {
+  pvo_internal_reproject_record_drop();
   Riders rider{};
   size_t rider_lds = 0;
   if (jobs && jobs->cy && jobs->crows > 0) {
@@ -2948,8 +2982,15 @@
   PVO_CHECK_LAUNCH();
   if (!motion_only && E + P > 0) {
     const int Kmax = (nframes < P + E) ? nframes : (P + E);
-    hipLaunchKernelGGL(ba_backsub_kernel, dim3((HW + 255) / 256, Kmax > clamp_frames ? Kmax : clamp_frames), dim3(256), 0, st,
-                       w.plan, jj, w.Ei, w.Eij, w.Q, w.w, w.dx, disps, dz_out, dz_rows, HW, t0, P, clamp_frames, disp_min);
+    const dim3 bgrid((HW + 255) / 256, Kmax > clamp_frames ? Kmax : clamp_frames);
+    ReprojAhead ra{};
+    if (ahead) { ra = *ahead; ra.poses = poses; }
+#define PVO_BACKSUB_LAUNCH(T) hipLaunchKernelGGL(ba_backsub_kernel<T>, bgrid, dim3(256), 0, st, w.plan, jj, w.Ei, w.Eij, w.Q, w.w, w.dx, disps, \
+                                                 dz_out, dz_rows, HW, t0, P, clamp_frames, disp_min, ra, wd)
+    if (!ahead) PVO_BACKSUB_LAUNCH(void);
+    else if (ahead->dtype == PVO_F16) PVO_BACKSUB_LAUNCH(pvo_half);
+    else PVO_BACKSUB_LAUNCH(pvo_bf16);
+#undef PVO_BACKSUB_LAUNCH
     PVO_CHECK_LAUNCH();
   }
   return PVO_OK;
diff --git a/pvo_amd/csrc/common.h b/pvo_amd/csrc/common.h
--- a/pvo_amd/csrc/common.h
+++ b/pvo_amd/csrc/common.h
@@ -11,6 +11,8 @@
     hipError_t _e = hipGetLastError();                       \
     if (_e != hipSuccess) { pvo_note_hip_error(static_cast<int>(_e)); return PVO_ELAUNCH; } \
   } while (0)
+
+void pvo_internal_reproject_record_drop() __attribute__((visibility("hidden")));
 
 static inline hipStream_t pvo_stream(void* s) { return reinterpret_cast<hipStream_t>(s); }
 
diff --git a/pvo_amd/csrc/geom.hip b/pvo_amd/csrc/geom.hip
--- a/pvo_amd/csrc/geom.hip
+++ b/pvo_amd/csrc/geom.hip
@@ -1,13 +1,8 @@
-#include "operand16.h"
-#include "se3.h"
+#include "reproject_body.h"
 
 namespace {
 
 constexpr float kMinDepthNative = 0.25f;
-constexpr float kMinDepthPy = 0.2f;
-
-struct Intr { float fx, fy, cx, cy; };
-__device__ __forceinline__ Intr load_intr(const float* p) { return {p[0], p[1], p[2], p[3]}; }
 
 __device__ __forceinline__ float pair_distance(const float* __restrict__ poses, const float* __restrict__ disps, const Intr K,
                                                int ix, int jx, int HW, int wd, float beta, int tid, float (*red)[4]) {
@@ -254,34 +249,9 @@
   const int e = blockIdx.y;
   const int k = blockIdx.x * 256 + threadIdx.x;
   if (k >= HW) return;
-  const long long idx = static_cast<long long>(e) * HW + k;
-  const float2 t = target[idx], dd = delta_dy[idx], m = raw_mask[idx];
   const int ix = static_cast<int>(ii[e]), jx = static_cast<int>(jj[e]);
-  const Intr Ki = load_intr(intrinsics + 4 * static_cast<long long>(ix));
-  const Intr Kj = load_intr(intrinsics + 4 * static_cast<long long>(jx));
-  const Pose G = rel_pose(load_pose(poses + 7 * static_cast<long long>(ix)), load_pose(poses + 7 * static_cast<long long>(jx)));
-  const int i = k / wd, j = k - i * wd;
-  float X0[4] = {(static_cast<float>(j) - Ki.cx) / Ki.fx, (static_cast<float>(i) - Ki.cy) / Ki.fy, 1.0f,
-                 disps[static_cast<long long>(ix) * HW + k]};
-  float X1[4];
-  act4(G, X0, X1);
-  float Z = X1[2];
-  Z = (Z < 0.5f * kMinDepthPy) ? 1.0f : Z;
-  const float d = 1.0f / Z;
-  float2 c;
-  c.x = Kj.fx * (X1[0] * d) + Kj.cx;
-  c.y = Kj.fy * (X1[1] * d) + Kj.cy;
-  *reinterpret_cast<float2*>(coords + idx * 2) = c;
-  valid[idx] = (X1[2] > kMinDepthPy && X0[2] > kMinDepthPy) ? 1.0f : 0.0f;
-  const float x0 = static_cast<float>(j), y0 = static_cast<float>(i);
-  const float f[8] = {t.x - x0, t.y - y0, t.x - x0 + dd.x, t.y - y0 + dd.y, t.x - c.x, t.y - c.y, m.x, m.y};
-  uint32_t o[4];
-#pragma unroll
-  for (int q = 0; q < 4; ++q) {
-    const float a = fminf(fmaxf(f[2 * q], -64.0f), 64.0f), b = fminf(fmaxf(f[2 * q + 1], -64.0f), 64.0f);
-    o[q] = pvo_bits<T>(a) | (pvo_bits<T>(b) << 16);
-  }
-  *reinterpret_cast<uint4*>(motn + idx * 8) = make_uint4(o[0], o[1], o[2], o[3]);
+  const ReprojMotionOut o = {coords, valid, target, delta_dy, raw_mask, motn};
+  reproject_motion_pixel<T>(poses, intrinsics, ix, jx, e, k, disps[static_cast<long long>(ix) * HW + k], HW, wd, o);
 }
 
 extern "C" int pvo_reproject_motion(const float* poses, const float* disps, const float* intrinsics,
diff --git a/pvo_amd/csrc/graph_glue.hip b/pvo_amd/csrc/graph_glue.hip
--- a/pvo_amd/csrc/graph_glue.hip
+++ b/pvo_amd/csrc/graph_glue.hip
@@ -65,6 +65,7 @@
   if (!coords1 || !heads || !raw_mask || !target || !delta_dy || !weight || !target_ba || !weight_ba || !full_flow || n >= (1LL << 31)) return PVO_EINVAL;
   if (pvo_misaligned16(heads)) return PVO_EINVAL;
   if (segm && (!vote_tot || !vote_dyn || max_segments <= 0)) return PVO_EINVAL;
+  pvo_internal_reproject_record_drop();
   hipStream_t st = pvo_stream(stream);
   const dim3 grid(static_cast<unsigned>((n + 255) / 256));
   auto f2 = [](float* p) { return reinterpret_cast<float2*>(p); };
diff --git a/pvo_amd/csrc/reproject_body.h b/pvo_amd/csrc/reproject_body.h
--- /dev/null
+++ b/pvo_amd/csrc/reproject_body.h
@@ -0,0 +1,54 @@
+#pragma once
+#include "operand16.h"
+#include "se3.h"
+
+constexpr float kMinDepthPy = 0.2f;
+
+struct Intr { float fx, fy, cx, cy; };
+__device__ __forceinline__ Intr load_intr(const float* p) { return {p[0], p[1], p[2], p[3]}; }
+
+struct ReprojMotionOut {
+  float* coords; float* valid;
+  const float2* target; const float2* delta_dy; const float2* raw_mask;
+  uint16_t* motn;
+};
+
+struct ReprojAhead { const float* poses; const float* intrinsics; ReprojMotionOut out; int n_in; int dtype; };
+
+int pvo_internal_ba_finish_ahead(float* poses, float* disps, void* sys, const int64_t* ii, const int64_t* jj,
+                                 int E, int nframes, int ht, int wd, int t0, int t1,
+                                 float lm, float ep, int motion_only, int clamp_frames, float disp_min,
+                                 void* workspace, size_t workspace_bytes,
+                                 const pvo_ba_riders* jobs, const ReprojAhead* ahead, int* rode, void* stream) __attribute__((visibility("hidden")));
+
+template <typename T>
+__device__ __forceinline__ void reproject_motion_pixel(const float* __restrict__ poses, const float* __restrict__ intrinsics,
+                                                       int ix, int jx, int e, int k, float disp, int HW, int wd, const ReprojMotionOut& o) {
+#pragma clang fp contract(off)
+  const long long idx = static_cast<long long>(e) * HW + k;
+  const float2 t = o.target[idx], dd = o.delta_dy[idx], m = o.raw_mask[idx];
+  const Intr Ki = load_intr(intrinsics + 4 * static_cast<long long>(ix));
+  const Intr Kj = load_intr(intrinsics + 4 * static_cast<long long>(jx));
+  const Pose G = Se3Exact::rel_pose(load_pose(poses + 7 * static_cast<long long>(ix)), load_pose(poses + 7 * static_cast<long long>(jx)));
+  const int i = k / wd, j = k - i * wd;
+  float X0[4] = {(static_cast<float>(j) - Ki.cx) / Ki.fx, (static_cast<float>(i) - Ki.cy) / Ki.fy, 1.0f, disp};
+  float X1[4];
+  Se3Exact::act4(G, X0, X1);
+  float Z = X1[2];
+  Z = (Z < 0.5f * kMinDepthPy) ? 1.0f : Z;
+  const float d = 1.0f / Z;
+  float2 c;
+  c.x = Kj.fx * (X1[0] * d) + Kj.cx;
+  c.y = Kj.fy * (X1[1] * d) + Kj.cy;
+  *reinterpret_cast<float2*>(o.coords + idx * 2) = c;
+  o.valid[idx] = (X1[2] > kMinDepthPy && X0[2] > kMinDepthPy) ? 1.0f : 0.0f;
+  const float x0 = static_cast<float>(j), y0 = static_cast<float>(i);
+  const float f[8] = {t.x - x0, t.y - y0, t.x - x0 + dd.x, t.y - y0 + dd.y, t.x - c.x, t.y - c.y, m.x, m.y};
+  uint32_t q4[4];
+#pragma unroll
+  for (int q = 0; q < 4; ++q) {
+    const float a = fminf(fmaxf(f[2 * q], -64.0f), 64.0f), b = fminf(fmaxf(f[2 * q + 1], -64.0f), 64.0f);
+    q4[q] = pvo_bits<T>(a) | (pvo_bits<T>(b) << 16);
+  }
+  *reinterpret_cast<uint4*>(o.motn + idx * 8) = make_uint4(q4[0], q4[1], q4[2], q4[3]);
+}
diff --git a/pvo_amd/csrc/se3.h b/pvo_amd/csrc/se3.h
--- a/pvo_amd/csrc/se3.h
+++ b/pvo_amd/csrc/se3.h
@@ -9,42 +9,20 @@
   Pose P; P.t = {p[0], p[1], p[2]}; P.q = {p[3], p[4], p[5], p[6]}; return P;
 }
 
-__device__ __forceinline__ Vec3 cross3(const Vec3 a, const Vec3 b) {
-  return {a.y * b.z - a.z * b.y, a.z * b.x - a.x * b.z, a.x * b.y - a.y * b.x};
-}
-
-__device__ __forceinline__ Vec3 rotate(const Quat q, const Vec3 v) {
-  const Vec3 qv = {q.x, q.y, q.z};
-  Vec3 uv = cross3(qv, v);
-  uv = {2.0f * uv.x, 2.0f * uv.y, 2.0f * uv.z};
-  const Vec3 c = cross3(qv, uv);
-  return {v.x + q.w * uv.x + c.x, v.y + q.w * uv.y + c.y, v.z + q.w * uv.z + c.z};
-}
-
 __device__ __forceinline__ Quat qconj(const Quat q) { return {-q.x, -q.y, -q.z, q.w}; }
 
-__device__ __forceinline__ Quat qmul(const Quat a, const Quat b) {
-  return {a.w * b.x + a.x * b.w + a.y * b.z - a.z * b.y,
-          a.w * b.y + a.y * b.w + a.z * b.x - a.x * b.z,
-          a.w * b.z + a.z * b.w + a.x * b.y - a.y * b.x,
-          a.w * b.w - a.x * b.x - a.y * b.y - a.z * b.z};
-}
-
-__device__ __forceinline__ Pose rel_pose(const Pose Gi, const Pose Gj) {
-  Pose G;
-  G.q = qmul(Gj.q, qconj(Gi.q));
-  const Vec3 r = rotate(G.q, Gi.t);
-  G.t = {Gj.t.x - r.x, Gj.t.y - r.y, Gj.t.z - r.z};
-  return G;
-}
-
-__device__ __forceinline__ void act4(const Pose G, const float X[4], float Y[4]) {
-  const Vec3 r = rotate(G.q, {X[0], X[1], X[2]});
-  Y[0] = r.x + X[3] * G.t.x;
-  Y[1] = r.y + X[3] * G.t.y;
-  Y[2] = r.z + X[3] * G.t.z;
-  Y[3] = X[3];
-}
+#define PVO_SE3_FN __device__ __forceinline__
+#define PVO_SE3_FP
+#include "se3_math.h"
+#undef PVO_SE3_FP
+#undef PVO_SE3_FN
+struct Se3Exact {
+#define PVO_SE3_FN static __device__ __forceinline__
+#define PVO_SE3_FP _Pragma("clang fp contract(off)")
+#include "se3_math.h"
+#undef PVO_SE3_FP
+#undef PVO_SE3_FN
+};
 
 __device__ __forceinline__ void adjT(const Pose G, const float X[6], float Y[6]) {
   const Quat qi = qconj(G.q);
diff --git a/pvo_amd/csrc/se3_math.h b/pvo_amd/csrc/se3_math.h
--- /dev/null
+++ b/pvo_amd/csrc/se3_math.h
@@ -0,0 +1,40 @@
+
+PVO_SE3_FN Vec3 cross3(const Vec3 a, const Vec3 b) {
+  PVO_SE3_FP
+  return {a.y * b.z - a.z * b.y, a.z * b.x - a.x * b.z, a.x * b.y - a.y * b.x};
+}
+
+PVO_SE3_FN Vec3 rotate(const Quat q, const Vec3 v) {
+  PVO_SE3_FP
+  const Vec3 qv = {q.x, q.y, q.z};
+  Vec3 uv = cross3(qv, v);
+  uv = {2.0f * uv.x, 2.0f * uv.y, 2.0f * uv.z};
+  const Vec3 c = cross3(qv, uv);
+  return {v.x + q.w * uv.x + c.x, v.y + q.w * uv.y + c.y, v.z + q.w * uv.z + c.z};
+}
+
+PVO_SE3_FN Quat qmul(const Quat a, const Quat b) {
+  PVO_SE3_FP
+  return {a.w * b.x + a.x * b.w + a.y * b.z - a.z * b.y,
+          a.w * b.y + a.y * b.w + a.z * b.x - a.x * b.z,
+          a.w * b.z + a.z * b.w + a.x * b.y - a.y * b.x,
+          a.w * b.w - a.x * b.x - a.y * b.y - a.z * b.z};
+}
+
+PVO_SE3_FN Pose rel_pose(const Pose Gi, const Pose Gj) {
+  PVO_SE3_FP
+  Pose G;
+  G.q = qmul(Gj.q, qconj(Gi.q));
+  const Vec3 r = rotate(G.q, Gi.t);
+  G.t = {Gj.t.x - r.x, Gj.t.y - r.y, Gj.t.z - r.z};
+  return G;
+}
+
+PVO_SE3_FN void act4(const Pose G, const float X[4], float Y[4]) {
+  PVO_SE3_FP
+  const Vec3 r = rotate(G.q, {X[0], X[1], X[2]});
+  Y[0] = r.x + X[3] * G.t.x;
+  Y[1] = r.y + X[3] * G.t.y;
+  Y[2] = r.z + X[3] * G.t.z;
+  Y[3] = X[3];
+}
diff --git a/pvo_amd/csrc/update_exec.hip b/pvo_amd/csrc/update_exec.hip
--- a/pvo_amd/csrc/update_exec.hip
+++ b/pvo_amd/csrc/update_exec.hip
@@ -1,5 +1,6 @@
 #include "common.h"
 #include "graph_post.h"
+#include "reproject_body.h"
 #include <stdlib.h>
 
 int pvo_segment_hist_ws(const int* segm, const float* raw_mask, const void* heads, int* tot, int* dyn,
@@ -36,6 +37,14 @@
   int dev = 0;
   if (hipGetDevice(&dev) != hipSuccess || dev < 0 || dev >= 64) return nullptr;
   return &g_ctx_ahead[dev];
+}
+
+struct ReprojRecord { const void *ws, *poses, *disps, *intrinsics, *ii, *jj, *target, *delta_dy, *raw_mask; int E, H, W, dtype; bool valid; };
+ReprojRecord g_reproj[64] = {};
+ReprojRecord* reproj_slot() {
+  int dev = 0;
+  if (hipGetDevice(&dev) != hipSuccess || dev < 0 || dev >= 64) return nullptr;
+  return &g_reproj[dev];
 }
 
 struct Probe { int stage; int cap; int limit; int n; int every; int seen; hipEvent_t* ev; };
@@ -237,6 +246,10 @@
   if (i < n) { const float v = x[i]; x[i] = (v < lo) ? lo : v; }
 }
 
+}
+
+void pvo_internal_reproject_record_drop() {
+  if (ReprojRecord* rr = reproj_slot()) rr->valid = false;
 }
 
 extern "C" size_t pvo_operator_workspace_bytes(int E, int K, int H, int W) {
@@ -285,12 +298,19 @@
   hipStream_t st = pvo_stream(stream);
 
   probe_mark(PVO_STAGE_UPDATE, 0, stream);
-  RUN(pvo_reproject_motion(u->poses, u->disps, u->intrinsics, u->ii, u->jj, s.coords, s.valid, u->target, u->delta_dy, u->raw_mask,
-                           s.motion, E, H, W, dt, stream));
+  const bool ahead_off = pvo_knob(PVO_KNOB_NO_RIDERS) != 0;
+  ReprojRecord* rr = reproj_slot();
+  const bool coords_ready = rr && rr->valid && u->reproject_ready && !ahead_off && rr->ws == workspace && rr->poses == u->poses &&
+                            rr->disps == u->disps && rr->intrinsics == u->intrinsics && rr->ii == u->ii && rr->jj == u->jj &&
+                            rr->target == u->target && rr->delta_dy == u->delta_dy && rr->raw_mask == u->raw_mask && rr->E == E &&
+                            rr->H == H && rr->W == W && rr->dtype == dt;
+  if (rr) rr->valid = false;
+  if (!coords_ready)
+    RUN(pvo_reproject_motion(u->poses, u->disps, u->intrinsics, u->ii, u->jj, s.coords, s.valid, u->target, u->delta_dy, u->raw_mask,
+                             s.motion, E, H, W, dt, stream));
   a.coords = s.coords; a.corr = nullptr; a.motion = s.motion; a.heads = s.heads;
   a.eta = u->op.eta ? u->op.eta : s.eta;
   if (u->want_upmask && !a.upmask) a.upmask = s.upmask;
-  const bool ahead_off = pvo_knob(PVO_KNOB_NO_RIDERS) != 0;
   ContextAhead* ca = ctx_ahead_slot();
   const bool ctx_ready = ca && ca->valid && u->context_ready && !ahead_off && ca->ws == workspace && ca->weights == w &&
                          ca->glo_w == w->glo_w && ca->gate_wt == w->gate_wt && ca->net == a.net && ca->E == E && ca->H == H &&
@@ -316,6 +336,10 @@
                           !pvo_misaligned16(b.a2, w->up_w, a.upmask);
   const bool mask_rides = u->itrs > 0 && a.K > 0 && a.upmask && !rider_off && rider_fits;
   const bool context_ahead = u->context_ahead && u->itrs >= 2 && !u->motion_only && !ahead_off;
+  const bool reproject_ahead = u->reproject_ahead && u->itrs >= 1 && !u->motion_only && !ahead_off && !pvo_misaligned16(s.motion) &&
+                               !((reinterpret_cast<uintptr_t>(u->target) | reinterpret_cast<uintptr_t>(u->delta_dy) |
+                                  reinterpret_cast<uintptr_t>(u->raw_mask)) & 7);
+  int reproject_rode = 0;
   if (pending && hipStreamWaitEvent(st, pending->mid, 0) != hipSuccess) return PVO_ELAUNCH;
   if (!mask_rides) RUN(run_upmask(w, &a, b, stream));
   const int Eb = u->n_in + E;
@@ -335,9 +359,18 @@
     if (context_ahead && it == 1) {
       jobs.xpart = b.part; jobs.xwt = w->gate_wt; jobs.xbias = w->gate_b; jobs.xg = b.g; jobs.xE = E; jobs.xchunks = pvo_gru_glo_chunks(HW);
     }
-    RUN(pvo_ba_finish_riders(u->poses, u->disps, u->sys, u->ii_ba, u->jj_ba, Eb, u->nframes, H, W, u->t0, u->t1, u->lm, u->ep,
-                             u->motion_only, last && !u->motion_only ? u->clamp_frames : 0, u->disp_min,
-                             nullptr, nullptr, 0, nullptr, u->ba_ws, u->ba_ws_bytes, &jobs, stream));
+    if (last && reproject_ahead) {
+      const ReprojAhead ra = {nullptr, u->intrinsics,
+                              {s.coords, s.valid, reinterpret_cast<const float2*>(u->target), reinterpret_cast<const float2*>(u->delta_dy),
+                               reinterpret_cast<const float2*>(u->raw_mask), reinterpret_cast<uint16_t*>(s.motion)}, u->n_in, dt};
+      RUN(pvo_internal_ba_finish_ahead(u->poses, u->disps, u->sys, u->ii_ba, u->jj_ba, Eb, u->nframes, H, W, u->t0, u->t1, u->lm, u->ep,
+                                       u->motion_only, u->clamp_frames, u->disp_min, u->ba_ws, u->ba_ws_bytes, &jobs, &ra, &reproject_rode,
+                                       stream));
+    } else {
+      RUN(pvo_ba_finish_riders(u->poses, u->disps, u->sys, u->ii_ba, u->jj_ba, Eb, u->nframes, H, W, u->t0, u->t1, u->lm, u->ep,
+                               u->motion_only, last && !u->motion_only ? u->clamp_frames : 0, u->disp_min,
+                               nullptr, nullptr, 0, nullptr, u->ba_ws, u->ba_ws_bytes, &jobs, stream));
+    }
   }
   probe_mark(PVO_STAGE_BA, 1, stream);
   if (u->clamp_frames > 0 && (u->itrs == 0 || u->motion_only)) {
@@ -347,6 +380,8 @@
   }
   if (ca && context_ahead)
     *ca = ContextAhead{workspace, w, w->glo_w, w->gate_wt, a.net_out, E, H, W, dt, true};
+  if (rr && reproject_rode)
+    *rr = ReprojRecord{workspace, u->poses, u->disps, u->intrinsics, u->ii, u->jj, u->target, u->delta_dy, u->raw_mask, E, H, W, dt, true};
   probe_mark(PVO_STAGE_UPDATE, 1, stream);
   return PVO_OK;
 }
diff --git a/pvo_amd/factor_graph.py b/pvo_amd/factor_graph.py
--- a/pvo_amd/factor_graph.py
+++ b/pvo_amd/factor_graph.py
@@ -686,8 +686,12 @@
         token = (net.data_ptr(), net._version, st.setdefault("serial", next(_CACHE_SERIAL)), weights.serial)
         a.context_ahead = 1
         a.context_ready = 1 if getattr(self, "_ctx_token", None) == token else 0
+        rtoken = (st["serial"],) + tuple(x for t in (v.poses, v.disps, v.intrinsics, self.target_cam, self.delta_dy, self.raw_mask)
+                                         for x in (t.data_ptr(), t._version))
+        a.reproject_ahead = 1
+        a.reproject_ready = 1 if getattr(self, "_reproj_token", None) == rtoken else 0
         db.graph_update(weights, a, st["ws"])
-        self._ctx_token = token
+        self._ctx_token, self._reproj_token = token, rtoken
         if sharded is not None:
             sharded.ba(v.poses, v.disps, v.intrinsics[0], st["target_ba"], st["weight_ba"], st["eta"], st["ii_ba"], st["jj_ba"],
                        t0, t1, itrs=itrs, lm=lm, ep=ep, motion_only=motion_only, plan_key=(id(self), self._version, t0, t1))
```

Result: no change. 245.4 keyframe updates/s (-0.0%).
